# junghoseong/aircombat-selfplay

Hardware: AMD Instinct MI355X
Metric: agent-steps/sec (higher is better)
Workload: dtype f32

## Files before the change

aircombat-selfplay_amd/csrc/aircombat.hip:

```cpp
#include <hip/hip_runtime.h>
#include <stdint.h>
#include <stdio.h>
#include <string.h>
#include <string>
#include <vector>
#include <cmath>
#include <algorithm>
#include <chrono>
#include "../../include/aircombat.h"
#include "../../include/aircombat_buffer.h"
#include "clk_stamps.hpp"
#include "f16_device.hpp"
#include "f16_split.hpp"

using f16::State;
using f16::Derived;
using f16::Tab;
using f16::clampf;

#define AC_F_FIELDS(X)                                                                                           \
  X(vx) X(vy) X(vz) X(q0) X(q1) X(q2) X(q3) X(wp) X(wq) X(wr) X(hv1x) X(hv1y) X(hv1z) X(hv2x) X(hv2y) X(hv2z)   \
  X(ha1x) X(ha1y) X(ha1z) X(wdx) X(wdy) X(wdz) X(aix) X(aiy) X(aiz) X(bax) X(bay) X(baz) X(da) X(de) X(dr)       \
  X(thr) X(pin_r) X(pin_p) X(pin_y) X(pi_r) X(pi_p) X(pi_y) X(tef) X(ail) X(elev) X(sbdeg) X(alpha) X(mach)      \
  X(qc) X(vg) X(ap) X(aq) X(ar) X(npx) X(npy) X(npz) X(n1) X(n2) X(n2norm) X(ff) X(tank0) X(tank1)
#define AC_TF_FIELDS(X) X(bloods) X(pre_posture) X(pre_altitude) X(pre_event) X(pre_shoot)
#define AC_TI_FIELDS(X)                                                                                  \
  X(status) X(die_flag) X(remaining) X(pre_remaining) X(shoot_action) X(last_missile) X(last_shoot_time) \
  X(lock_bits) X(lock_pos) X(cur_step)

enum {
#define X(n) FF_##n,
  AC_F_FIELDS(X) AC_TF_FIELDS(X)
#undef X
  NF
};
enum {
  FI_eng, FI_ticks,
#define X(n) FI_##n,
  AC_TI_FIELDS(X)
#undef X
  NI
};
enum { ND = 3 };
enum : int {
  SW_tef = 0, SW_pin_r, SW_pin_p, SW_pin_y,
  SW_pi_r, SW_pi_p, SW_pi_y, SW_ail,
  SW_elev, SW_sbdeg, SW_n1, SW_n2,
  SW_n2norm, SW_ff, SW_tank0, SW_tank1,
  SW_alpha, SW_mach, SW_qc, SW_vg,
  SW_ap, SW_aq, SW_ar, SW_npy,
  SW_npz, SW_npx, SW_eng, SW_ticks,
  SW_vx, SW_vy, SW_vz, SW_q0,
  SW_q1, SW_q2, SW_q3, SW_wp,
  SW_wq, SW_wr, SW_hv1x, SW_hv1y,
  SW_hv1z, SW_hv2x, SW_hv2y, SW_hv2z,
  SW_ha1x, SW_ha1y, SW_ha1z, SW_wdx,
  SW_wdy, SW_wdz, SW_aix, SW_aiy,
  SW_aiz, SW_bax, SW_bay, SW_baz,
  SW_da, SW_de, SW_dr, SW_thr,
  SW_pre_posture, SW_pre_altitude, SW_pre_event, SW_cur_step,
  SW_bloods, SW_status, SW_die_flag, SW_pre_shoot,
  SW_remaining, SW_pre_remaining, SW_shoot_action, SW_last_missile,
  SW_last_shoot_time, SW_lock_bits, SW_lock_pos, SW_pad,
  NSW
};
enum { NSG = NSW / 4, SG_TASK0 = 15 };
static_assert(NSW == 76 && SW_pre_posture == 4 * SG_TASK0, "19 groups: 15 flight, 4 task");
static const int kSlotF[NF] = {
#define X(n) SW_##n,
    AC_F_FIELDS(X) AC_TF_FIELDS(X)
#undef X
};
static const int kSlotI[NI] = {SW_eng, SW_ticks,
#define X(n) SW_##n,
                               AC_TI_FIELDS(X)
#undef X
};
enum { MF_px, MF_py, MF_pz, MF_vx, MF_vy, MF_vz, MF_theta, MF_psi, MF_t, MF_m, MF_dth, MF_dph, MF_dprev, NMF };
enum { MI_status, MI_recede, MI_order, NMI };
enum { MSL_INACTIVE = -1, MSL_LAUNCHED = 0, MSL_HIT = 1, MSL_MISS = 2 };

static const char* kStateNames[AC_STATE_LEN] = {
    "rx", "ry", "rz",
#define X(n) #n,
    AC_F_FIELDS(X) AC_TF_FIELDS(X) "eng", "ticks", AC_TI_FIELDS(X)
#undef X
    "x_rem_gun", "x_rem_9m", "x_rem_120b", "x_rem_chaff", "x_bits", "x_last_chaff", "x_orphan_hits", "x_mp_prev", "x_ref_set",
    "x_ch_status0", "x_ch_mult0", "x_ch_status1", "x_ch_mult1", "x_n_ch",
    "x_cg_AO", "x_cg_TA", "x_wez0", "x_wez1", "x_wez2", "x_wez3", "x_tail0", "x_tail1", "x_tail2", "x_tail3",
    "x_c0x", "x_c0y", "x_c0z", "x_c0t", "x_c1x", "x_c1y", "x_c1z", "x_c1t",
};

struct Task {
#define X(n) float n;
  AC_TF_FIELDS(X)
#undef X
#define X(n) int n;
  AC_TI_FIELDS(X)
#undef X
};

template <typename R>
struct MslT {
  R px, py, pz, vx, vy, vz, theta, psi, t, m, dth, dph, dprev;
  int status, recede, order;
  int dpos;
  int model;
};
using Msl = MslT<float>;
using MslD = MslT<double>;

struct DevCfg {
  int task, A, n_ego, substeps, max_steps, obs_dim, act_dim, msl_slots;
  int N;
  float altitude_limit, acc_x, acc_y, acc_z;
  float posture_scale, altitude_scale, event_scale, missile_posture_scale, shoot_penalty_scale;
  int posture_pot, altitude_pot, event_pot, shoot_pot;
  float alt_safe, alt_danger, alt_kv;
  float max_attack_angle, max_attack_distance;
  int min_attack_interval, use_artillery, lock_len;
  int rwr;
  int legacy_obs;
  int tobs;
  int num_missiles[AC_MAX_AGENTS];
  double P0x, P0y, P0z, sLat0, cLat0, sLon0, cLon0;
  float rm0, rn0, h0;
  unsigned long long chaff_seed;
};

struct DevPtrs {
  float* F; int* I; double* D;
  float* MF; int* MI;
  double* MD;
  float* H;
  int* man_step; float* man_h0;
  const float* tF; const int* tI; const double* tD;
  const float* tab;
  const float* actions;
  float* obs; float* rew; uint8_t* done; int* info;
  float* obs2; float* rew2; uint8_t* done2; int* info2;
  int* err;
};

__device__ __forceinline__ bool nonfinite_probe(float veci, float pqr, float h_sl_ft, float np_max) {
  return !(fabsf(veci + pqr + h_sl_ft + np_max) < INFINITY);
}
__device__ __forceinline__ float poison_if(bool bad, float reward) { return bad ? __int_as_float(0x7fc00001) : reward; }

#define AC_LANE_INDEX(n) const unsigned un_ = (unsigned)(n), uN_ = (unsigned)N
#define AC_AT(base, f) \
  (*(decltype(base))((char*)(base) + (size_t)((unsigned)(f) * (uN_ * (unsigned)sizeof(*(base))) + un_ * (unsigned)sizeof(*(base)))))
#define AC_GRP(S, g) (*reinterpret_cast<float4*>((char*)(S) + (size_t)((unsigned)(g) * (uN_ * 16u) + un_ * 16u)))
#define AC_WORD(S, w) (*reinterpret_cast<int*>((char*)(S) + (size_t)((unsigned)((w) >> 2) * (uN_ * 16u) + un_ * 16u + 4u * (unsigned)((w) & 3))))
__device__ __forceinline__ int state_word(const float* S, int w, int N, int n) { AC_LANE_INDEX(n); return AC_WORD(S, w); }
#define AC_FLIGHT_GROUPS(G)                                                                                                       \
  G(0, tef, pin_r, pin_p, pin_y) G(1, pi_r, pi_p, pi_y, ail) G(2, elev, sbdeg, n1, n2) G(3, n2norm, ff, tank0, tank1)               \
  G(4, alpha, mach, qc, vg) G(5, ap, aq, ar, npy) G(7, vx, vy, vz, q0) G(8, q1, q2, q3, wp) G(9, wq, wr, hv1x, hv1y)                \
  G(10, hv1z, hv2x, hv2y, hv2z) G(11, ha1x, ha1y, ha1z, wdx) G(12, wdy, wdz, aix, aiy) G(13, aiz, bax, bay, baz) G(14, da, de, dr, thr)
static_assert(SW_alpha == 16 && SW_npz == 24 && SW_vx == 28 && SW_ha1x == 44 && SW_da == 56, "AC_FLIGHT_GROUPS follows the SW_ order");
__device__ __forceinline__ void load_position(const double* D, int N, int n, State& s) {
  const double2 xy = *reinterpret_cast<const double2*>((const char*)D + (size_t)((unsigned)n * 16u));
  s.rx = xy.x; s.ry = xy.y;
  s.rz = D[2 * (size_t)N + n];
}
__device__ __forceinline__ void store_position(double* D, int N, int n, const State& s) {
  *reinterpret_cast<double2*>((char*)D + (size_t)((unsigned)n * 16u)) = make_double2(s.rx, s.ry);
  D[2 * (size_t)N + n] = s.rz;
}
constexpr bool ac_role_reads(int role, int g) {
  return role < 0 || (role == 0 ? g >= 4 : (role == 1 ? g <= 6 : (g >= 6 && g <= 10)));
}
template <int ROLE>
__device__ __forceinline__ void load_flight_role(const float* F, const int* I, const double* D, int N, int n, State& s) {
  (void)I;
  AC_LANE_INDEX(n);
#define G(g, a, b, c, d) if (ac_role_reads(ROLE, g)) { const float4 v = AC_GRP(F, g); s.a = v.x; s.b = v.y; s.c = v.z; s.d = v.w; }
  AC_FLIGHT_GROUPS(G)
#undef G
  if (ac_role_reads(ROLE, 6)) {
    const float4 v = AC_GRP(F, 6);
    s.npz = v.x; s.npx = v.y; s.eng = __float_as_int(v.z); s.ticks = __float_as_int(v.w);
  }
  if (ROLE != 1) load_position(D, N, n, s);
}
__device__ __forceinline__ void load_flight(const float* F, const int* I, const double* D, int N, int n, State& s) { load_flight_role<-1>(F, I, D, N, n, s); }
__device__ __forceinline__ void store_flight(float* F, int* I, double* D, int N, int n, const State& s) {
  (void)I;
  AC_LANE_INDEX(n);
#define G(g, a, b, c, d) AC_GRP(F, g) = make_float4(s.a, s.b, s.c, s.d);
  AC_FLIGHT_GROUPS(G)
#undef G
  AC_GRP(F, 6) = make_float4(s.npz, s.npx, __int_as_float(s.eng), __int_as_float(s.ticks));
  store_position(D, N, n, s);
}
__device__ __forceinline__ void load_task(const float* F, const int* I, int N, int n, Task& t) {
  (void)I;
  AC_LANE_INDEX(n);
  const float4 a = AC_GRP(F, SG_TASK0), b = AC_GRP(F, SG_TASK0 + 1), c = AC_GRP(F, SG_TASK0 + 2), d = AC_GRP(F, SG_TASK0 + 3);
  t.pre_posture = a.x; t.pre_altitude = a.y; t.pre_event = a.z; t.cur_step = __float_as_int(a.w);
  t.bloods = b.x; t.status = __float_as_int(b.y); t.die_flag = __float_as_int(b.z); t.pre_shoot = b.w;
  t.remaining = __float_as_int(c.x); t.pre_remaining = __float_as_int(c.y); t.shoot_action = __float_as_int(c.z); t.last_missile = __float_as_int(c.w);
  t.last_shoot_time = __float_as_int(d.x); t.lock_bits = __float_as_int(d.y); t.lock_pos = __float_as_int(d.z);
}
__device__ __forceinline__ void store_task_group0(float* F, int N, int n, const Task& t) {
  AC_LANE_INDEX(n);
  AC_GRP(F, SG_TASK0) = make_float4(t.pre_posture, t.pre_altitude, t.pre_event, __int_as_float(t.cur_step));
}
__device__ __forceinline__ void store_task_rare(float* F, int N, int n, const Task& t) {
  AC_LANE_INDEX(n);
  AC_GRP(F, SG_TASK0 + 1) = make_float4(t.bloods, __int_as_float(t.status), __int_as_float(t.die_flag), t.pre_shoot);
  AC_GRP(F, SG_TASK0 + 2) = make_float4(__int_as_float(t.remaining), __int_as_float(t.pre_remaining), __int_as_float(t.shoot_action), __int_as_float(t.last_missile));
  AC_GRP(F, SG_TASK0 + 3) = make_float4(__int_as_float(t.last_shoot_time), __int_as_float(t.lock_bits), __int_as_float(t.lock_pos), 0.0f);
}
__device__ __forceinline__ void store_task(float* F, int* I, int N, int n, const Task& t) {
  (void)I;
  store_task_group0(F, N, n, t);
  store_task_rare(F, N, n, t);
}
__device__ __forceinline__ void load_state(const float* F, const int* I, const double* D, int N, int n, State& s, Task& t) {
  load_flight(F, I, D, N, n, s);
  load_task(F, I, N, n, t);
}
__device__ __forceinline__ void store_state(float* F, int* I, double* D, int N, int n, const State& s, const Task& t) {
  store_flight(F, I, D, N, n, s);
  store_task(F, I, N, n, t);
}
template <typename R>
__device__ __forceinline__ void load_msl(const R* MF, const int* MI, int N, int n, int slot, MslT<R>& m) {
  AC_LANE_INDEX(n);
  const R* f = MF + (size_t)slot * NMF * N;
  const int* i = MI + (size_t)slot * NMI * N;
  m.px = AC_AT(f, MF_px); m.py = AC_AT(f, MF_py); m.pz = AC_AT(f, MF_pz);
  m.vx = AC_AT(f, MF_vx); m.vy = AC_AT(f, MF_vy); m.vz = AC_AT(f, MF_vz);
  m.theta = AC_AT(f, MF_theta); m.psi = AC_AT(f, MF_psi); m.t = AC_AT(f, MF_t); m.m = AC_AT(f, MF_m);
  m.dth = AC_AT(f, MF_dth); m.dph = AC_AT(f, MF_dph); m.dprev = AC_AT(f, MF_dprev);
  m.status = AC_AT(i, MI_status); m.order = AC_AT(i, MI_order);
  const int rw = AC_AT(i, MI_recede);
  m.recede = rw & 511; m.model = (rw >> 9) & 1; m.dpos = rw >> 10;
}
template <typename R>
__device__ __forceinline__ void store_msl(R* MF, int* MI, int N, int n, int slot, const MslT<R>& m) {
  AC_LANE_INDEX(n);
  R* f = MF + (size_t)slot * NMF * N;
  int* i = MI + (size_t)slot * NMI * N;
  AC_AT(f, MF_px) = m.px; AC_AT(f, MF_py) = m.py; AC_AT(f, MF_pz) = m.pz;
  AC_AT(f, MF_vx) = m.vx; AC_AT(f, MF_vy) = m.vy; AC_AT(f, MF_vz) = m.vz;
  AC_AT(f, MF_theta) = m.theta; AC_AT(f, MF_psi) = m.psi; AC_AT(f, MF_t) = m.t; AC_AT(f, MF_m) = m.m;
  AC_AT(f, MF_dth) = m.dth; AC_AT(f, MF_dph) = m.dph; AC_AT(f, MF_dprev) = m.dprev;
  AC_AT(i, MI_status) = m.status; AC_AT(i, MI_recede) = (m.dpos << 10) | (m.model << 9) | m.recede; AC_AT(i, MI_order) = m.order;
}

template <typename R>
__device__ __forceinline__ void store_msl_clock(R* MF, int* MI, int N, int n, int slot, const MslT<R>& m) {
  AC_LANE_INDEX(n);
  R* f = MF + (size_t)slot * NMF * N;
  int* i = MI + (size_t)slot * NMI * N;
  AC_AT(f, MF_t) = m.t; AC_AT(f, MF_dprev) = m.dprev;
  AC_AT(i, MI_status) = m.status; AC_AT(i, MI_recede) = (m.dpos << 10) | (m.model << 9) | m.recede;
}
__device__ __forceinline__ void store_task_changed(float* F, int* I, int N, int n, const Task& t, const Task& was) {
  (void)I;
  store_task_group0(F, N, n, t);
  const bool rare = __float_as_int(t.bloods) != __float_as_int(was.bloods) || __float_as_int(t.pre_shoot) != __float_as_int(was.pre_shoot) ||
                    t.status != was.status || t.die_flag != was.die_flag || t.remaining != was.remaining || t.pre_remaining != was.pre_remaining ||
                    t.shoot_action != was.shoot_action || t.last_missile != was.last_missile || t.last_shoot_time != was.last_shoot_time ||
                    t.lock_bits != was.lock_bits || t.lock_pos != was.lock_pos;
  if (rare) store_task_rare(F, N, n, t);
}

__device__ __forceinline__ void zero_controller_state(const DevPtrs& P, int N, int n, bool live) {
  if (P.H && live) {
    for (int k = 0; k < 128; ++k) P.H[(size_t)k * N + n] = 0.0f;
    P.man_step[n] = 0; P.man_h0[n] = 0.0f;
  }
}

struct Props {
  float n, e, u;
  double n64, e64, u64;
  float vn, ve, vd;
  float alt_m;
  float ub, vb, wb, vc;
  float sphi, cphi, stht, ctht;
  float m11, m12;
};
__device__ __forceinline__ float mps(float fps) { return clampf(-700.0f, fps * f16::kFt2M, 700.0f); }

__device__ __forceinline__ void make_pose(const Derived& d, const DevCfg& c, Props& p) {
  p.alt_m = clampf(-500.0f, d.h_sl_ft * f16::kFt2M, 26000.0f);
  p.vn = mps(d.vn); p.ve = mps(d.ve); p.vd = mps(d.vd);
  const double a = 6378137.0, b = 6356752.314245179;
  double sl = d.sLat64, cl = d.cLat64, so = d.sLon64, co = d.cLon64;
  double Nn = a * a * fx::rsqrt(a * a * cl * cl + b * b * sl * sl);
  double h = (double)p.alt_m;
  double x = (Nn + h) * cl * co, y = (Nn + h) * cl * so, z = (Nn * (b / a) * (b / a) + h) * sl;
  double dx = x - c.P0x, dy = y - c.P0y, dz = z - c.P0z;
  double t = c.cLon0 * dx + c.sLon0 * dy;
  p.e64 = -c.sLon0 * dx + c.cLon0 * dy; p.u64 = c.cLat0 * t + c.sLat0 * dz; p.n64 = -c.sLat0 * t + c.cLat0 * dz;
  p.e = (float)p.e64; p.u = (float)p.u64; p.n = (float)p.n64;
}
__device__ __forceinline__ void make_props(const State& s, const Derived& d, const DevCfg& c, Props& p) {
  make_pose(d, c, p);
  p.ub = mps(d.u); p.vb = mps(d.v); p.wb = mps(d.w);
  p.vc = clampf(0.0f, f16::vcas_from_impact_pressure(s.qc) * f16::kFt2M, 1400.0f);
  const float* T = d.T;
  float m13 = T[0] * d.d_eci[0] + T[1] * d.d_eci[1] + T[2] * d.d_eci[2];
  float m23 = T[3] * d.d_eci[0] + T[4] * d.d_eci[1] + T[5] * d.d_eci[2];
  float m33 = T[6] * d.d_eci[0] + T[7] * d.d_eci[1] + T[8] * d.d_eci[2];
  p.m11 = T[0] * d.n_eci[0] + T[1] * d.n_eci[1] + T[2] * d.n_eci[2];
  p.m12 = T[0] * d.e_eci[0] + T[1] * d.e_eci[1] + T[2] * d.e_eci[2];
  p.stht = clampf(-1.0f, -m13, 1.0f);
  float ct = sqrtf(fmaxf(0.0f, 1.0f - p.stht * p.stht));
  p.ctht = ct;
  float ic = (ct > 1e-12f) ? 1.0f / sqrtf(m23 * m23 + m33 * m33) : 0.0f;
  p.sphi = (ct > 1e-12f) ? m23 * ic : 0.0f;
  p.cphi = (ct > 1e-12f) ? m33 * ic : 1.0f;
}

struct Geo { float AO, TA, R, side, cAO, cTA; };
__device__ __forceinline__ float acos_fast(float x) { return f16::atan2_fast(sqrtf((1.0f - x) * (1.0f + x)), x); }
__device__ __forceinline__ float tanh_fast(float x) {
  const float t = __expf(2.0f * clampf(-10.0f, x, 10.0f));
  return (t - 1.0f) / (t + 1.0f);
}
__device__ __forceinline__ float atanh_fast(float x) { return 0.5f * __logf((1.0f + x) / (1.0f - x)); }
template <bool TWO_D>
__device__ __forceinline__ Geo ao_ta_r(float ex, float ey, float ez, float evx, float evy, float evz,
                                       float nx, float ny, float nz, float nvx, float nvy, float nvz) {
  float dx = nx - ex, dy = ny - ey, dz = nz - ez;
  float ev, nv, R, pe, pn;
  if (TWO_D) {
    ev = sqrtf(evx * evx + evy * evy); nv = sqrtf(nvx * nvx + nvy * nvy); R = sqrtf(dx * dx + dy * dy);
    pe = dx * evx + dy * evy; pn = dx * nvx + dy * nvy;
  } else {
    ev = sqrtf(evx * evx + evy * evy + evz * evz); nv = sqrtf(nvx * nvx + nvy * nvy + nvz * nvz);
    R = sqrtf(dx * dx + dy * dy + dz * dz);
    pe = dx * evx + dy * evy + dz * evz; pn = dx * nvx + dy * nvy + dz * nvz;
  }
  Geo g;
  g.cAO = clampf(-1.0f, pe / (R * ev + 1e-8f), 1.0f);
  g.cTA = clampf(-1.0f, pn / (R * nv + 1e-8f), 1.0f);
  g.AO = acos_fast(g.cAO);
  g.TA = acos_fast(g.cTA);
  g.R = R;
  float cr = evx * dy - evy * dx;
  g.side = (cr > 0.0f) ? 1.0f : ((cr < 0.0f) ? -1.0f : 0.0f);
// ... 245 lines not shown
  __builtin_amdgcn_fence(__ATOMIC_RELEASE, "wavefront");
  __builtin_amdgcn_wave_barrier();
  __builtin_amdgcn_fence(__ATOMIC_ACQUIRE, "wavefront");
}
__device__ __forceinline__ void emit_rows(const DevPtrs& P, float* lds , int ow, int lane,
                                          float reward, bool done, int A, int i0, int i1, int i2, int i3);
template <int NOB>
__device__ __forceinline__ void emit_outputs(const DevPtrs& P, float* lds , int ow, int lane, const float (&ob)[NOB],
                                             float reward, bool done, int A, int i0, int i1, int i2, int i3) {
  float* row = lds + lane * ow;
#pragma unroll
  for (int k = 0; k < NOB; ++k) if (k < ow) row[k] = ob[k];
  for (int k = NOB; k < ow; ++k) row[k] = 0.0f;
  emit_rows(P, lds, ow, lane, reward, done, A, i0, i1, i2, i3);
}
__device__ __forceinline__ void emit_obs_rows(const DevPtrs& P, float* lds, int ow, int lane) {
  wave_lds_fence();
  AC_CLK(56);
  const size_t blk = blockIdx.x;
  const int nvec = 16 * ow;
  const float4* l4 = reinterpret_cast<const float4*>(lds);
#pragma unroll
  for (int set = 1; set >= 0; --set) {
    float* obs = set ? P.obs2 : P.obs;
    if (!obs) continue;
    float4* o4 = reinterpret_cast<float4*>(obs + blk * 64 * (size_t)ow);
    int i = lane;
    for (; i + 192 < nvec; i += 256) {
      const float4 v0 = l4[i], v1 = l4[i + 64], v2 = l4[i + 128], v3 = l4[i + 192];
      o4[i] = v0; o4[i + 64] = v1; o4[i + 128] = v2; o4[i + 192] = v3;
    }
    for (; i < nvec; i += 64) o4[i] = l4[i];
  }
  AC_CLK(57);
  wave_lds_fence();
}
__device__ __forceinline__ void emit_scalars(const DevPtrs& P, int lane, float reward, bool done, int A, int i0, int i1, int i2, int i3) {
  const size_t blk = blockIdx.x;
  const unsigned long long dmask = __ballot(done);
  unsigned dword = 0;
#pragma unroll
  for (int b = 0; b < 4; ++b) dword |= (unsigned)((dmask >> (4 * (lane & 15) + b)) & 1ull) << (8 * b);
  const int4 inf = make_int4(i0, i1, i2, i3);
  const int packed = (i0 & 0xFFFF) | ((i1 & 0xFF) << 16) | (min(i2, 127) << 24) | ((i3 & 1) << 31);
  const size_t n = blk * 64 + lane;
  if (!(fabsf(reward) < INFINITY)) {
    const int own = ((__float_as_int(reward) & 0x7fffffff) == 0x7fc00001) ? 1 : 0;
    __hip_atomic_fetch_max(P.err, (own << 30) | (0x3fffffff - (int)n), __ATOMIC_RELAXED, __HIP_MEMORY_SCOPE_SYSTEM);
  }
#pragma unroll
  for (int set = 1; set >= 0; --set) {
    float* rew = set ? P.rew2 : P.rew; uint8_t* dn = set ? P.done2 : P.done; int* info = set ? P.info2 : P.info;
    if (!rew) continue;
    rew[n] = reward;
    if (lane < 16) reinterpret_cast<unsigned*>(dn + blk * 64)[lane] = dword;
    if (set) {
      const int w = __shfl(packed, (lane * A) & 63);
      if (lane < 64 / A) info[blk * (64 / A) + lane] = w;
    } else if (lane % A == 0) *reinterpret_cast<int4*>(info + (n / A) * 4) = inf;
  }
}
__device__ __forceinline__ void emit_rows(const DevPtrs& P, float* lds, int ow, int lane, float reward, bool done, int A, int i0, int i1, int i2, int i3) {
  emit_obs_rows(P, lds, ow, lane);
  emit_scalars(P, lane, reward, done, A, i0, i1, i2, i3);
}
__device__ __forceinline__ float4 load_controls(const float* act, int act_dim) {
  if ((act_dim & 3) == 0) return *reinterpret_cast<const float4*>(act);
  return make_float4(act[0], act[1], act[2], act[3]);
}

struct Enemy { float n, e, u, vn, ve, vd, ub, alt; };
__device__ __forceinline__ Enemy exchange_1v1(const Props& pr) {
  Enemy E;
  E.n = __shfl_xor(pr.n, 1); E.e = __shfl_xor(pr.e, 1); E.u = __shfl_xor(pr.u, 1);
  E.vn = __shfl_xor(pr.vn, 1); E.ve = __shfl_xor(pr.ve, 1); E.vd = __shfl_xor(pr.vd, 1);
  E.ub = __shfl_xor(pr.ub, 1); E.alt = __shfl_xor(pr.alt_m, 1);
  return E;
}
struct Incoming { bool any; float px, py, pz, vx, vy, vz; };
template <int TASK>
__device__ __forceinline__ void observe_1v1(const Props& pr, const Enemy& E, const Incoming& in, float* ob) {
  ob[0] = pr.alt_m / 5000.0f;
  ob[1] = pr.sphi; ob[2] = pr.cphi; ob[3] = pr.stht; ob[4] = pr.ctht;
  ob[5] = pr.ub / 340.0f; ob[6] = pr.vb / 340.0f; ob[7] = pr.wb / 340.0f; ob[8] = pr.vc / 340.0f;
  Geo g = (TASK == AC_TASK_SINGLECOMBAT)
              ? ao_ta_r<true>(pr.n, pr.e, pr.u, pr.vn, pr.ve, pr.vd, E.n, E.e, E.u, E.vn, E.ve, E.vd)
              : ao_ta_r<false>(pr.n, pr.e, pr.u, pr.vn, pr.ve, pr.vd, E.n, E.e, E.u, E.vn, E.ve, E.vd);
  ob[9] = (E.ub - pr.ub) / 340.0f;
  ob[10] = (E.alt - pr.alt_m) / 1000.0f;
  ob[11] = g.AO; ob[12] = g.TA; ob[13] = g.R / 10000.0f; ob[14] = g.side;
  if (TASK == AC_TASK_SINGLECOMBAT) {
#pragma unroll
    for (int k = 0; k < 15; ++k) ob[k] = clampf(-10.0f, ob[k], 10.0f);
  } else {
#pragma unroll
    for (int k = 15; k < 21; ++k) ob[k] = 0.0f;
    if (in.any) {
      Geo gm = ao_ta_r<false>(pr.n, pr.e, pr.u, pr.vn, pr.ve, pr.vd, in.px, in.py, in.pz, in.vx, in.vy, in.vz);
      ob[15] = (sqrtf(in.vx * in.vx + in.vy * in.vy + in.vz * in.vz) - pr.ub) / 340.0f;
      ob[16] = (in.pz - pr.alt_m) / 1000.0f;
      ob[17] = gm.AO; ob[18] = gm.TA; ob[19] = gm.R / 10000.0f; ob[20] = gm.side;
    }
  }
}
__device__ __forceinline__ float posture_raw(const Props& pr, const Enemy& E) {
  Geo g = ao_ta_r<false>(pr.n, pr.e, pr.u, pr.vn, pr.ve, pr.vd, E.n, E.e, E.u, E.vn, E.ve, E.vd);
  return posture_fn(g.AO, g.TA, g.R * 0.001f);
}
__device__ __forceinline__ float altitude_raw(const Props& pr, const DevCfg& c) {
  return altitude_fn(pr.u * 0.001f, pr.vd / 340.0f, c);
}

template <int TASK>
struct TaskTraits {
  static constexpr bool HAS_MSL = (TASK == AC_TASK_SHOOT_MISSILE || TASK == AC_TASK_DODGE_MISSILE);
  static constexpr int MSLOTS = HAS_MSL ? AC_MAX_MISSILES_PER_AGENT : 1;
  static constexpr int OBS = (TASK == AC_TASK_SINGLECOMBAT) ? 15 : 21;
};

#include "split_kernel.hpp"
#include "pair_kernel.hpp"

template <int TASK, int WPE, int FORM = 0>
__global__ __launch_bounds__(FORM == 1 ? 192 : (FORM == 2 ? 128 : (FORM == 3 ? 256 : 64)), WPE) void step_kernel_1v1(DevPtrs P, DevCfg c) {
  static_assert(TASK == AC_TASK_SINGLECOMBAT ? FORM <= 1 : FORM >= 2, "no launch path for this (task, form)");
  using TT = TaskTraits<TASK>;
  constexpr bool SPLIT = FORM == 1, QUAD = FORM == 3, PAIR = FORM == 2 || QUAD;
  constexpr bool HAS_MSL = TT::HAS_MSL;
  constexpr int MSLOTS = TT::MSLOTS;
  constexpr int OBS = TT::OBS;
  AC_CLK(0);
  __shared__ __attribute__((aligned(16))) float lds_tab[F16_PACK_LEN];
  __shared__ __attribute__((aligned(16))) float lds_out[64 * OBS];
  __shared__ __attribute__((aligned(16))) char split_lds[SPLIT ? sizeof(SplitLds) : (QUAD ? sizeof(QuadLds) : (PAIR ? sizeof(PairLds) : 16))];
  SplitLds& L = *reinterpret_cast<SplitLds*>(split_lds);
  QuadLds& LQ = *reinterpret_cast<QuadLds*>(split_lds);
  PairLds& LP = QUAD ? LQ.P : *reinterpret_cast<PairLds*>(split_lds);
  const Tab T{lds_tab};
  const int N = c.N;
  const int l = threadIdx.x & 63;
  const int n = blockIdx.x * 64 + l;
  const bool live = n < N;
  const int nn = live ? n : (N - 2 + (n & 1));
  const int slot = nn & 1;

  State s; Task t; Derived d; Props pr;
  int pre_st[MSLOTS];
#pragma unroll
  for (int k = 0; k < MSLOTS; ++k) pre_st[k] = MSL_INACTIVE;
  const float* act = P.actions + (size_t)nn * c.act_dim;
  float4 a4;
  ActionFetch arow;
  float shoot_raw = 0.0f;
  if (SPLIT) {
    TableCopy<192> tc;
    tc.issue(P.tab);
    AC_CLKW(0, 123);
    const int role = __builtin_amdgcn_readfirstlane(threadIdx.x >> 6);
    s = State{}; t = Task{};
    if (role == 0) { load_flight_role<0>(P.F, P.I, P.D, N, nn, s); AC_CLKW(0, 124); load_task(P.F, P.I, N, nn, t); AC_CLKW(0, 125); }
    else if (role == 1) load_flight_role<1>(P.F, P.I, P.D, N, nn, s);
    else { load_flight_role<2>(P.F, P.I, P.D, N, nn, s); t.status = state_word(P.F, SW_status, N, nn); }
    __builtin_amdgcn_s_barrier();
    tc.write(lds_tab);
    a4 = make_float4(0.f, 0.f, 0.f, 0.f);
    __builtin_amdgcn_s_waitcnt(0x0F70);
    if (role == 1) arow.issue(act, c.act_dim);
    AC_CLKW(0, 120); AC_CLKW(1, 121); AC_CLKW(2, 122);
    __syncthreads();
  } else if (QUAD) {
    const int role = __builtin_amdgcn_readfirstlane(threadIdx.x >> 6);
    TableCopy<256> tc;
    tc.issue(P.tab);
    s = State{}; t = Task{};
    if (role == 0) { load_flight_role<0>(P.F, P.I, P.D, N, nn, s); t.status = state_word(P.F, SW_status, N, nn); }
    else if (role == 1) load_flight_role<1>(P.F, P.I, P.D, N, nn, s);
    else if (role == 2) { load_flight_role<2>(P.F, P.I, P.D, N, nn, s); t.status = state_word(P.F, SW_status, N, nn); }
    else {
      load_task(P.F, P.I, N, nn, t);
      s.ticks = state_word(P.F, SW_ticks, N, nn);
#pragma unroll
      for (int k = 0; k < MSLOTS; ++k) pre_st[k] = P.MI[((size_t)k * NMI + MI_status) * (size_t)N + nn];
    }
    __builtin_amdgcn_s_barrier();
    tc.write(lds_tab);
    a4 = make_float4(0.f, 0.f, 0.f, 0.f);
    __builtin_amdgcn_s_waitcnt(0x0F70);
    if (role == 1) arow.issue(act, c.act_dim);
    __syncthreads();
    if (role == 0) { quad_dynamics_wave(P, c, T, LQ, l, n, live, s, t); return; }
    if (role != 3 && split_helper_wave<true>(s, t, T, LQ.S, l, c.substeps, nullptr, nullptr, &arow)) return;
  } else if (PAIR) {
    const bool flight_role = __builtin_amdgcn_readfirstlane(threadIdx.x >> 6) == 1;
    PairFlightIn fin;
    if (!flight_role) {
      a4 = make_float4(0.f, 0.f, 0.f, 0.f);
      s = State{}; load_task(P.F, P.I, N, nn, t);
#pragma unroll
      for (int k = 0; k < MSLOTS; ++k) pre_st[k] = P.MI[((size_t)k * NMI + MI_status) * (size_t)N + nn];
    }
    stage_tables<128>(lds_tab, P.tab);
    if (flight_role) {
      pair_flight_load(P, c, nn, fin);
      pair_flight_wave<true>(P, c, T, LP, l, n, live, fin);
      return;
    }

  } else {
    TableCopy<64> tc;
    tc.issue(P.tab);
    a4 = load_controls(act, c.act_dim);
    if (TASK == AC_TASK_SHOOT_MISSILE) shoot_raw = act[4];
    load_state(P.F, P.I, P.D, N, nn, s, t);
    tc.commit(lds_tab);
  }
  AC_CLK(1);
  const Task was = t;
  constexpr bool OBS_BY_KIN = SPLIT && TASK == AC_TASK_SINGLECOMBAT;
  if (SPLIT) {
    const int role = __builtin_amdgcn_readfirstlane(threadIdx.x >> 6);
    if (split_helper_wave(s, t, T, L, l, c.substeps, nullptr, nullptr, &arow)) {
      if (OBS_BY_KIN && role == 1) {
        using namespace mail;
        wg_sync();
        Props q;
        q.alt_m = L.M[T_PR][l]; q.ub = L.M[T_PR + 5][l];
        q.n = L.M[T_PR + 9][l]; q.e = L.M[T_PR + 10][l]; q.u = L.M[T_PR + 11][l];
        q.vn = L.M[T_PR + 12][l]; q.ve = L.M[T_PR + 13][l]; q.vd = L.M[T_PR + 14][l];
        const Enemy Eq = exchange_1v1(q);
        L.M[T_RALT][l] = altitude_raw(q, c);
        L.M[T_RPOS][l] = posture_raw(q, Eq);
        wg_sync();
      }
      if (OBS_BY_KIN && role == 2) {
        using namespace mail;
        wg_sync();
        Props q;
        q.alt_m = L.M[T_PR][l]; q.sphi = L.M[T_PR + 1][l]; q.cphi = L.M[T_PR + 2][l]; q.stht = L.M[T_PR + 3][l]; q.ctht = L.M[T_PR + 4][l];
        q.ub = L.M[T_PR + 5][l]; q.vb = L.M[T_PR + 6][l]; q.wb = L.M[T_PR + 7][l]; q.vc = L.M[T_PR + 8][l];
        q.n = L.M[T_PR + 9][l]; q.e = L.M[T_PR + 10][l]; q.u = L.M[T_PR + 11][l];
        q.vn = L.M[T_PR + 12][l]; q.ve = L.M[T_PR + 13][l]; q.vd = L.M[T_PR + 14][l];
        const Enemy Eq = exchange_1v1(q);
        const Incoming none{false, 0, 0, 0, 0, 0, 0};
        float obq[OBS];
        observe_1v1<TASK>(q, Eq, none, obq);
        wg_sync();
        if (L.M[T_DONE][l] != 0.0f) {
          const float* tobs = (const float*)(P.tF + (size_t)NSW * 2) + slot * OBS;
#pragma unroll
          for (int k = 0; k < OBS; ++k) obq[k] = tobs[k];
        }
        float* row = lds_out + l * OBS;
#pragma unroll
        for (int k = 0; k < OBS; ++k) row[k] = obq[k];
        emit_obs_rows(P, lds_out, OBS, l);
      }
      return;
    }
  }
  Msl ms[MSLOTS];
  int nslots = 0, msl_was_active = 0;
  if (HAS_MSL) {
    nslots = min(c.num_missiles[slot], MSLOTS);
#pragma unroll
    for (int k = 0; k < MSLOTS; ++k) {
      const int st = (k < nslots) ? (PAIR ? pre_st[k] : P.MI[((size_t)k * NMI + MI_status) * (size_t)N + nn]) : MSL_INACTIVE;
      if (st != MSL_INACTIVE) { load_msl(P.MF, P.MI, N, nn, k, ms[k]); msl_was_active |= 1 << k; }
      else { ms[k] = Msl{}; ms[k].status = MSL_INACTIVE; }
    }
  }

  t.cur_step += 1;
  if (!SPLIT) {
    s.da = clampf(-1.0f, a4.x / 20.0f - 1.0f, 1.0f);
    s.de = clampf(-1.0f, a4.y / 20.0f - 1.0f, 1.0f);
    s.dr = clampf(-1.0f, a4.z / 20.0f - 1.0f, 1.0f);
    s.thr = clampf(0.0f, a4.w / 58.0f + 0.4f, 0.9f);
  }
  if (TASK == AC_TASK_SHOOT_MISSILE && !PAIR) t.shoot_action = (shoot_raw != 0.0f) ? 1 : 0;

  const MslParam MP = aim9l();
  bool have_pose = false;
  int last_tick = -1;
  bool env_has_missiles = false;
  if (PAIR) {
    bool mine = false;
#pragma unroll
    for (int k = 0; k < MSLOTS; ++k) mine = mine || ms[k].status != MSL_INACTIVE;
    const int other = __shfl_xor((int)mine, 1);
    env_has_missiles = mine || (bool)other;
  }
  int quad_nrun = 0;
  const int quad_ticks0 = s.ticks;
  for (int sub = 0; sub < c.substeps; ++sub) {
    bool fly_munitions = HAS_MSL;
    if (QUAD) {
      quad_substep_begin<true>(t, LQ, l, sub, env_has_missiles, quad_ticks0, quad_nrun, pr, c);
      fly_munitions = env_has_missiles;
    } else if (PAIR) {
      AC_CLK(2 + 8 * sub);
      pair_substep<true>(t, LP, l, sub, env_has_missiles, pr, c);
      AC_CLK(4 + 8 * sub);
      if (!env_has_missiles) continue;
    } else if (SPLIT) {
      if (dynamics_wave_tick(s, t, d, T, L, l, sub)) { have_pose = true; last_tick = sub; }
    } else if (t.status == AC_ALIVE) {
      if (t.bloods <= 0.0f) t.status = AC_SHOTDOWN;
      f16::tick<false>(s, d, T);
      have_pose = true;
    }
    if (HAS_MSL && fly_munitions) {
      if (!PAIR) {
      f16::locate(s, d);
      if (!have_pose) { f16::body_frame(s, d); have_pose = true; }
      make_props(s, d, c, pr);
      }
      float tx = __shfl_xor(pr.n, 1), ty = __shfl_xor(pr.e, 1), tz = __shfl_xor(pr.u, 1);
      float tvx = __shfl_xor(pr.vn, 1), tvy = __shfl_xor(pr.ve, 1), tvz = __shfl_xor(pr.vd, 1);
      bool talive = __shfl_xor(t.status, 1) == AC_ALIVE;
      bool hit_now = false;
#pragma unroll
      for (int k = 0; k < MSLOTS; ++k) {
        if (k < nslots && ms[k].status != MSL_INACTIVE) {
          missile_run(ms[k], MP, tx, ty, tz, tvx, tvy, tvz, talive, c);
          if (ms[k].status == MSL_HIT && talive) { hit_now = true; talive = false; }
        }
      }
      if (__shfl_xor((int)hit_now, 1) && t.status == AC_ALIVE) t.status = AC_SHOTDOWN;
      AC_CLK(5 + 8 * sub);
    }
    if (QUAD) wg_sync();
  }
  const bool split_located = SPLIT && dynamics_wave_finish(s, d, L, l, last_tick, c.substeps);
  if (PAIR) {
    if (QUAD) wg_sync();
    wg_sync();
    pair_read_final(LP, l, s, d, pr);
  } else if (!HAS_MSL || c.substeps == 0) {
    if (!split_located) f16::locate(s, d);
    if (!have_pose) f16::body_frame(s, d);
    make_props(s, d, c, pr);
  }
  AC_CLK(52);
  if (OBS_BY_KIN) {
    using namespace mail;
    L.M[T_PR][l] = pr.alt_m; L.M[T_PR + 1][l] = pr.sphi; L.M[T_PR + 2][l] = pr.cphi; L.M[T_PR + 3][l] = pr.stht; L.M[T_PR + 4][l] = pr.ctht;
    L.M[T_PR + 5][l] = pr.ub; L.M[T_PR + 6][l] = pr.vb; L.M[T_PR + 7][l] = pr.wb; L.M[T_PR + 8][l] = pr.vc;
    L.M[T_PR + 9][l] = pr.n; L.M[T_PR + 10][l] = pr.e; L.M[T_PR + 11][l] = pr.u;
    L.M[T_PR + 12][l] = pr.vn; L.M[T_PR + 13][l] = pr.ve; L.M[T_PR + 14][l] = pr.vd;
    wg_sync();
  }
  Enemy E = exchange_1v1(pr);

  if (c.use_artillery) {
    Geo g = ao_ta_r<false>(pr.n, pr.e, pr.u, pr.vn, pr.ve, pr.vd, E.n, E.e, E.u, E.vn, E.ve, E.vd);
    bool ealive = __shfl_xor(t.status, 1) == AC_ALIVE;
    float of = (g.AO <= 0.5236f) ? 1.0f - g.AO / 0.5236f : 0.0f;
    float Rk = g.R * 0.001f;
    float df = (Rk <= 1.0f) ? 1.0f : ((Rk <= 3.0f) ? (3.0f - Rk) * 0.5f : 0.0f);
    float dmg = ealive ? of * df : 0.0f;
    t.bloods -= __shfl_xor(dmg, 1);
  }
  if (HAS_MSL) {
    bool launch;
    if (TASK == AC_TASK_SHOOT_MISSILE && PAIR) t.shoot_action = ((QUAD ? LQ.S.M[mail::F_BITS][l] : LP.FIN[pair::FIN_BITS][l]) != 0.0f) ? 1 : 0;
    if (TASK == AC_TASK_DODGE_MISSILE) {
      const float dx = E.n - pr.n, dy = E.e - pr.e, dz = E.u - pr.u;
      const float dist = sqrtf(dx * dx + dy * dy + dz * dz);
      const float sp = sqrtf(pr.vn * pr.vn + pr.ve * pr.ve + pr.vd * pr.vd);
      const float ang = 57.29577951f * acosf(clampf(-1.0f, (dx * pr.vn + dy * pr.ve + dz * pr.vd) / (dist * sp + 1e-8f), 1.0f));
      const int len = c.lock_len;
      const unsigned bit = 1u << (unsigned)(t.lock_pos % len);
      t.lock_bits = (ang < c.max_attack_angle) ? (t.lock_bits | (int)bit) : (t.lock_bits & ~(int)bit);
      t.lock_pos += 1;
      const bool locked = __popc((unsigned)t.lock_bits & ((1u << len) - 1u)) >= len;
      launch = t.status == AC_ALIVE && locked && dist <= c.max_attack_distance && t.remaining > 0 &&
               (t.cur_step - t.last_shoot_time) >= c.min_attack_interval;
      if (launch) t.last_shoot_time = t.cur_step;
    } else {
      bool prev_done = t.last_missile < 0;
#pragma unroll
      for (int k = 0; k < MSLOTS; ++k)
        if (k == t.last_missile) prev_done = (ms[k].status == MSL_HIT || ms[k].status == MSL_MISS);
      launch = t.status == AC_ALIVE && t.shoot_action && t.remaining > 0 && prev_done;
    }
    int k = nslots - t.remaining;
    if (launch && k >= 0 && k < nslots) {
      float tht = asinf(pr.stht);
      float psi = atan2f(pr.m12, pr.m11);
      if (psi < 0.0f) psi += 2.0f * f16::kPi;
#pragma unroll
      for (int q = 0; q < MSLOTS; ++q)
        if (q == k) {
          ms[q].px = pr.n; ms[q].py = pr.e; ms[q].pz = pr.u; ms[q].vx = pr.vn; ms[q].vy = pr.ve; ms[q].vz = pr.vd;
          ms[q].theta = tht; ms[q].psi = psi; ms[q].t = 0.0f; ms[q].m = MP.m0; ms[q].dth = 0.0f; ms[q].dph = 0.0f;
          ms[q].dprev = INFINITY; ms[q].recede = 0; ms[q].status = MSL_LAUNCHED; ms[q].order = t.cur_step;
        }
      t.last_missile = k;
      t.remaining -= 1;
    }
  }

  Incoming inc{false, 0, 0, 0, 0, 0, 0};
  int my_hits = 0;
  int inc_slot = -1;
  if (HAS_MSL) {
    int best = 0x7fffffff, mine = -1;
#pragma unroll
    for (int k = 0; k < MSLOTS; ++k) {
      if (k < nslots && ms[k].status == MSL_LAUNCHED && ms[k].order < best) { best = ms[k].order; mine = k; }
      if (k < nslots && ms[k].status == MSL_HIT) my_hits += 1;
    }
    float a0 = 0, a1 = 0, a2 = 0, a3 = 0, a4 = 0, a5 = 0;
#pragma unroll
    for (int k = 0; k < MSLOTS; ++k)
      if (k == mine) { a0 = ms[k].px; a1 = ms[k].py; a2 = ms[k].pz; a3 = ms[k].vx; a4 = ms[k].vy; a5 = ms[k].vz; }
    inc.any = __shfl_xor((int)(mine >= 0), 1);
    inc_slot = __shfl_xor(mine, 1);
    inc.px = __shfl_xor(a0, 1); inc.py = __shfl_xor(a1, 1); inc.pz = __shfl_xor(a2, 1);
    inc.vx = __shfl_xor(a3, 1); inc.vy = __shfl_xor(a4, 1); inc.vz = __shfl_xor(a5, 1);
  }
  float ob[OBS];
  if (!OBS_BY_KIN) observe_1v1<TASK>(pr, E, inc, ob);
  AC_CLK(58);

  const int status_pre = t.status;
  int code = AC_DONE_NONE;
  bool done = false;
  bool nonfinite = false;
  {
    float np_max = fmaxf(fabsf(s.npx), fmaxf(fabsf(s.npy), fabsf(s.npz)));
    float pqr = sqrtf(d.p * d.p + d.q * d.q + d.r * d.r);
    nonfinite = nonfinite_probe(d.veci, pqr, d.h_sl_ft, np_max);
    bool extreme = nonfinite || (d.veci >= 1e10f) || (pqr >= 1000.0f) || (d.h_sl_ft >= 1e10f) || (np_max > 10.0f);
    bool overload = (s.ticks >= kTickOverload) &&
                    (fabsf(s.npx) > c.acc_x || fabsf(s.npy) > c.acc_y || fabsf(s.npz + 1.0f) > c.acc_z);
    if (pr.alt_m <= c.altitude_limit) { t.status = AC_CRASH; code = AC_DONE_LOW_ALTITUDE; done = true; }
    else if (extreme) { t.status = AC_CRASH; code = AC_DONE_EXTREME_STATE; done = true; }
    else if (overload) { t.status = AC_CRASH; code = AC_DONE_OVERLOAD; done = true; }
  }
  {
    int other_pre = __shfl_xor(status_pre, 1), other_post = __shfl_xor(t.status, 1);
    int enemy_status = (slot == 0) ? other_pre : other_post;
    if (!done) {
      if (t.status == AC_SHOTDOWN) { code = AC_DONE_SHOTDOWN; done = true; }
      else if (t.status == AC_CRASH) { code = AC_DONE_CRASHED; done = true; }
      else if (enemy_status != AC_ALIVE && !inc.any) { code = AC_DONE_MISSION_COMPLETE; done = true; }
      else if (t.cur_step >= c.max_steps) { code = AC_DONE_TIMEOUT; done = true; }
    }
  }

  const int other_done = __shfl_xor((int)done, 1);
  const bool all_done = done && (bool)other_done;
  const int other_code = __shfl_xor(code, 1);
  if (OBS_BY_KIN) {
    L.M[mail::T_DONE][l] = all_done ? 1.0f : 0.0f;
    wg_sync();
  } else if (all_done) {
    const float* tobs = (const float*)(P.tF + (size_t)NSW * 2) + slot * OBS;
#pragma unroll
    for (int k = 0; k < OBS; ++k) ob[k] = tobs[k];
  }

  AC_CLK(59);
  float reward = 0.0f;
  const bool evaluates = !t.die_flag;
  if (evaluates) {
    t.die_flag = (t.status != AC_ALIVE) ? 1 : 0;
    float r_alt = potential(OBS_BY_KIN ? L.M[mail::T_RALT][l] : altitude_raw(pr, c), c.altitude_scale, c.altitude_pot, t.pre_altitude);
    float r_pos = potential(OBS_BY_KIN ? L.M[mail::T_RPOS][l] : posture_raw(pr, E), c.posture_scale, c.posture_pot, t.pre_posture);
    float ev = ((t.status != AC_ALIVE) ? -200.0f : 0.0f) + 200.0f * (float)my_hits;
    float r_ev = potential(ev, c.event_scale, c.event_pot, t.pre_event);
    reward = r_alt + r_pos + r_ev;
    if (TASK == AC_TASK_SHOOT_MISSILE) {
      float sp = (t.remaining == t.pre_remaining - 1) ? -30.0f : 0.0f;
      t.pre_remaining = t.remaining;
      reward += potential(sp, c.shoot_penalty_scale, c.shoot_pot, t.pre_shoot);
    }
  }
  if (TASK == AC_TASK_DODGE_MISSILE) {
    float spd[MSLOTS];
#pragma unroll
    for (int k = 0; k < MSLOTS; ++k) spd[k] = sqrtf(ms[k].vx * ms[k].vx + ms[k].vy * ms[k].vy + ms[k].vz * ms[k].vz);
    const int base = (threadIdx.x & 63) - slot;
    const int my_inc_id = inc.any ? 1 + (slot ^ 1) * MSLOTS + inc_slot : 0;
    int prev = t.shoot_action;
    float r_mp = 0.0f;
#pragma unroll
    for (int i = 0; i < 2; ++i) {
      const int ev_i = __shfl((int)evaluates, base + i), id_i = __shfl(my_inc_id, base + i);
      if (!ev_i) continue;
      if (id_i) {
        if (!prev) prev = id_i;
        float v_prev = 0.0f, v_cur = 0.0f;
#pragma unroll
        for (int k = 0; k < MSLOTS; ++k) {
          float a = __shfl(spd[k], base + (prev - 1) / MSLOTS), b = __shfl(spd[k], base + (id_i - 1) / MSLOTS);
          if (k == (prev - 1) % MSLOTS) v_prev = a;
          if (k == (id_i - 1) % MSLOTS) v_cur = b;
        }
        if (slot == i) {
          const float v_dec = (v_prev - v_cur) / 340.0f * c.missile_posture_scale;
          const float va = sqrtf(pr.vn * pr.vn + pr.ve * pr.ve + pr.vd * pr.vd);
          const float ang = (inc.vx * pr.vn + inc.vy * pr.ve + inc.vz * pr.vd) / (v_cur * va);
          r_mp = (ang < 0.0f) ? ang / (fmaxf(v_dec, 0.0f) + 1.0f) : ang * fmaxf(v_dec, 0.0f);
        }
      } else prev = 0;
    }
    t.shoot_action = prev;
    reward += r_mp;
  }

  int step_out = t.cur_step;
  if (all_done) {
    load_state(P.tF, P.tI, P.tD, 2, slot, s, t);
    zero_controller_state(P, N, n, live);
#pragma unroll
    for (int k = 0; k < MSLOTS; ++k) { ms[k] = Msl{}; ms[k].status = MSL_INACTIVE; }
  }
  AC_CLK(53);
  if (live) {
    if (!PAIR) { store_flight(P.F, P.I, P.D, N, n, s); store_task_changed(P.F, P.I, N, n, t, was); }
    else {
      if (all_done) store_flight(P.F, P.I, P.D, N, n, s);
      store_task_changed(P.F, P.I, N, n, t, was);
    }
    if (HAS_MSL) {
#pragma unroll
      for (int k = 0; k < MSLOTS; ++k)
        if (k < nslots && (ms[k].status != MSL_INACTIVE || ((msl_was_active >> k) & 1))) store_msl(P.MF, P.MI, N, n, k, ms[k]);
    }
  }
  AC_CLK(55);
  reward = poison_if(nonfinite, reward);
  if (OBS_BY_KIN) emit_scalars(P, l, reward, done, 2, step_out, other_code ? other_code : code, 0, all_done ? 1 : 0);
  else emit_outputs(P, lds_out, OBS, l, ob, reward, done, 2, step_out, other_code ? other_code : code, 0, all_done ? 1 : 0);
  AC_CLK(54);
}

__device__ __forceinline__ Enemy gather_pose(const Props& pr, int lane) {
  Enemy E;
  E.n = __shfl(pr.n, lane); E.e = __shfl(pr.e, lane); E.u = __shfl(pr.u, lane);
  E.vn = __shfl(pr.vn, lane); E.ve = __shfl(pr.ve, lane); E.vd = __shfl(pr.vd, lane);
  E.ub = __shfl(pr.ub, lane); E.alt = __shfl(pr.alt_m, lane);
  return E;
}
template <int A>
__device__ __forceinline__ float observe_nvn(const Props& pr, int slot, int base_lane, int n_ego, float* ob) {
  auto c10 = [](float v) { return clampf(-10.0f, v, 10.0f); };
  if (ob) {
    ob[0] = c10(pr.alt_m / 5000.0f);
    ob[1] = c10(pr.sphi); ob[2] = c10(pr.cphi); ob[3] = c10(pr.stht); ob[4] = c10(pr.ctht);
    ob[5] = c10(pr.ub / 340.0f); ob[6] = c10(pr.vb / 340.0f); ob[7] = c10(pr.wb / 340.0f); ob[8] = c10(pr.vc / 340.0f);
  }
  const int my_team = slot < n_ego ? 0 : 1;
  const int n_mine = my_team == 0 ? n_ego : A - n_ego;
  float posture = 0.0f;
#pragma unroll
  for (int j = 0; j < A; ++j) {
    Enemy E = gather_pose(pr, base_lane + j);
    const int team_j = j < n_ego ? 0 : 1;
    if (j == slot) continue;
    Geo g = ao_ta_r<false>(pr.n, pr.e, pr.u, pr.vn, pr.ve, pr.vd, E.n, E.e, E.u, E.vn, E.ve, E.vd);
    int idx;
    if (team_j == my_team) {
      int first = my_team == 0 ? 0 : n_ego;
      idx = (j - first) - (j > slot ? 1 : 0);
    } else {
      int first = my_team == 0 ? n_ego : 0;
      idx = (n_mine - 1) + (j - first);
      posture += posture_fn(g.AO, g.TA, g.R * 0.001f);
    }
    if (ob) {
      float* blk = ob + 9 + idx * 6;
      blk[0] = c10((E.ub - pr.ub) / 340.0f); blk[1] = c10((E.alt - pr.alt_m) / 1000.0f);
      blk[2] = c10(g.AO); blk[3] = c10(g.TA); blk[4] = c10(g.R / 10000.0f); blk[5] = c10(g.side);
    }
  }
  return posture;
}

template <int A>
__device__ __forceinline__ void legacy_obs_nvn(const Props& pr, int slot, int base_lane, int n_ego, float* row) {
  const int team = slot < n_ego ? 0 : 1;
  const int paired = (team == 0 ? n_ego : 0) + (slot - (team == 0 ? 0 : n_ego));
  const Enemy E = gather_pose(pr, base_lane + paired);
  const Incoming none{false, 0, 0, 0, 0, 0, 0};
  float o21[21];
  observe_1v1<AC_TASK_SHOOT_MISSILE>(pr, E, none, o21);
#pragma unroll
  for (int k = 0; k < 21; ++k) row[k] = o21[k];
}

template <int A, int WPE, bool SPLIT = false>
__global__ __launch_bounds__(SPLIT ? 192 : 64, WPE) void step_kernel_nvn(DevPtrs P, DevCfg c) {
  constexpr int OBS = 9 + 6 * (A - 1);
  __shared__ __attribute__((aligned(16))) float lds_tab[F16_PACK_LEN];
  __shared__ __attribute__((aligned(16))) float lds_out[64 * OBS];
  __shared__ __attribute__((aligned(16))) char split_lds[SPLIT ? sizeof(SplitLds) : 16];
  SplitLds& L = *reinterpret_cast<SplitLds*>(split_lds);
  const Tab T{lds_tab};
  const int N = c.N;
  const int l = threadIdx.x & 63;
  const int n = blockIdx.x * 64 + l;
  const bool live = n < N;
  const int slot = l % A;
  const int nn = live ? n : (N - A + slot);
  const int base_lane = l - slot;
  const int team = slot < c.n_ego ? 0 : 1;

  State s; Task t; Derived d; Props pr;
  TableCopy<SPLIT ? 192 : 64> tc;
  tc.issue(P.tab);
  const float4 a4 = load_controls(P.actions + (size_t)nn * c.act_dim, c.act_dim);
  load_state(P.F, P.I, P.D, N, nn, s, t);
  const Task was = t;
  tc.commit(lds_tab);
  t.cur_step += 1;
  s.da = clampf(-1.0f, a4.x / 20.0f - 1.0f, 1.0f);
  s.de = clampf(-1.0f, a4.y / 20.0f - 1.0f, 1.0f);
  s.dr = clampf(-1.0f, a4.z / 20.0f - 1.0f, 1.0f);
  s.thr = clampf(0.0f, a4.w / 58.0f + 0.4f, 0.9f);
  if (SPLIT && split_helper_wave(s, t, T, L, l, c.substeps)) return;
  bool have_pose = false;
  int nrun_split = 0;
  const bool split_located = SPLIT && dynamics_wave_ticks(s, t, d, T, L, l, c.substeps, nrun_split);
  for (int sub = 0; sub < c.substeps && !SPLIT; ++sub) {
    if (t.status == AC_ALIVE) {
      if (t.bloods <= 0.0f) t.status = AC_SHOTDOWN;
      f16::tick<false>(s, d, T);
      have_pose = true;
    }
  }
  if (!split_located) {
    f16::locate(s, d);
    if (!have_pose) f16::body_frame(s, d);
  }
  make_props(s, d, c, pr);

  const int ow = c.legacy_obs ? 21 : OBS;
  float* orow = lds_out + l * ow;
  float posture = observe_nvn<A>(pr, slot, base_lane, c.n_ego, c.legacy_obs ? nullptr : orow);
  if (c.legacy_obs) legacy_obs_nvn<A>(pr, slot, base_lane, c.n_ego, orow);

  float own = 0.0f;
  if (t.status == AC_ALIVE) {
    float r_alt = potential(altitude_raw(pr, c), c.altitude_scale, c.altitude_pot, t.pre_altitude);
    float r_pos = potential(posture, c.posture_scale, c.posture_pot, t.pre_posture);
    float r_ev = potential(0.0f, c.event_scale, c.event_pot, t.pre_event);
    own = r_alt + r_pos + r_ev;
  }
  float tsum = 0.0f;
#pragma unroll
  for (int j = 0; j < A; ++j) {
    float rj = __shfl(own, base_lane + j);
    if ((j < c.n_ego ? 0 : 1) == team) tsum += rj;
  }
  const float reward = tsum / (float)(team == 0 ? c.n_ego : A - c.n_ego);

  bool done = false;
  int code = AC_DONE_NONE;
  int last_code = AC_DONE_NONE;
  float np_max = fmaxf(fabsf(s.npx), fmaxf(fabsf(s.npy), fabsf(s.npz)));
  float pqr = sqrtf(d.p * d.p + d.q * d.q + d.r * d.r);
  const bool nonfinite = nonfinite_probe(d.veci, pqr, d.h_sl_ft, np_max);
  const bool extreme = nonfinite || (d.veci >= 1e10f) || (pqr >= 1000.0f) || (d.h_sl_ft >= 1e10f) || (np_max > 10.0f);
  const bool overload = (s.ticks >= kTickOverload) &&
                        (fabsf(s.npx) > c.acc_x || fabsf(s.npy) > c.acc_y || fabsf(s.npz + 1.0f) > c.acc_z);
  const bool low = pr.alt_m <= c.altitude_limit;
  const unsigned long long env_mask = ((A == 64) ? ~0ull : ((1ull << A) - 1ull)) << base_lane;
  const int st0 = t.status;
  const bool crash_cond = extreme || overload || low;
  constexpr unsigned amask = (A >= 32) ? ~0u : ((1u << A) - 1u);
  const unsigned al0 = (unsigned)(__ballot(st0 == AC_ALIVE) >> base_lane) & amask;
  const unsigned ccb = (unsigned)(__ballot(crash_cond) >> base_lane) & amask;
  const unsigned team0 = (1u << c.n_ego) - 1u, team1 = amask & ~team0;
  unsigned alive = al0;
  bool enemies_dead = false, crash_mine = false;
#pragma unroll
  for (int i = 0; i < A; ++i) {
    const bool ed = (alive & (i < c.n_ego ? team1 : team0)) == 0;
    const bool crash_now = ((al0 >> i) & 1u) && !ed && ((ccb >> i) & 1u);
    if (crash_now) alive &= ~(1u << i);
    if (i == slot) { enemies_dead = ed; crash_mine = crash_now; }
  }
  if (crash_mine) t.status = AC_CRASH;
  if (st0 == AC_SHOTDOWN) { code = AC_DONE_SHOTDOWN; done = true; }
  else if (st0 == AC_CRASH) { code = AC_DONE_CRASHED; done = true; }
  else if (enemies_dead) { code = AC_DONE_MISSION_COMPLETE; done = true; }
  else if (extreme) { code = AC_DONE_EXTREME_STATE; done = true; }
  else if (overload) { code = AC_DONE_OVERLOAD; done = true; }
  else if (low) { code = AC_DONE_LOW_ALTITUDE; done = true; }
  else if (t.cur_step >= c.max_steps) { code = AC_DONE_TIMEOUT; done = true; }
  {
    const unsigned long long coded = __ballot(code != AC_DONE_NONE) & env_mask;
    const int last = coded ? 63 - __clzll((long long)coded) : l;
    last_code = __shfl(code, last);
  }
  const bool all_done = ((unsigned)(__ballot(done) >> base_lane) & amask) == amask;
  int step_out = t.cur_step;
  if (all_done) {
    load_state(P.tF, P.tI, P.tD, A, slot, s, t);
    zero_controller_state(P, N, n, live);
    const float* tobs = P.tF + (size_t)NSW * A + slot * OBS;
    for (int k = 0; k < ow; ++k) orow[k] = tobs[k];
  }
  if (live) {
    store_flight(P.F, P.I, P.D, N, n, s);
    store_task_changed(P.F, P.I, N, n, t, was);
  }
  emit_rows(P, lds_out, ow, l, poison_if(nonfinite, reward), done, A, step_out, last_code, 0, all_done ? 1 : 0);
}

struct InitArgs { ac_init_state_t ic[AC_MAX_AGENTS]; };

__device__ double geod_alt_from_asl(double geod_lat, double alt) {
  const double a = f16::kA, b = f16::kB, e2 = 1.0 - b * b / (a * a);
  double cg = cos(geod_lat), sg = sin(geod_lat), Nn = a / sqrt(1 - e2 * sg * sg);
  double n = e2, prev_n = 1.0;
  int iter = 0;
  if (cg > fabs(sg)) {
    double tg = sg / cg, x0 = Nn * e2 * cg, x = 0.0;
    while (fabs(n - prev_n) > 1E-15 && iter < 10) {
      double tl = (1 - n) * tg, c2 = 1. / (1. + tl * tl), slr = b / sqrt(1. - e2 * c2), R = slr + alt;
      x = R * sqrt(c2); prev_n = n; n = x0 / x; iter++;
    }
    return x / cg - Nn;
  }
  double ctg = cg / sg, z0 = Nn * e2 * sg, z = 0.0;
  while (fabs(n - prev_n) > 1E-15 && iter < 10) {
    double ctl = ctg / (1 - n), s2 = 1. / (1. + ctl * ctl), c2 = 1. - s2, slr = b / sqrt(1. - e2 * c2), R = slr + alt;
    z = R * (ctl >= 0 ? 1.0 : -1.0) * sqrt(s2); prev_n = n; n = z0 / (z0 + z); iter++;
  }
  return z / sg - Nn * (1 - e2);
}

__device__ void initial_state(const ac_init_state_t& ic, const Tab& T, State& s, Derived& d) {
  s = State{};
  const double D2R = 3.14159265358979323846 / 180.0;
  double lon = ic.lon_deg * D2R, lat = ic.lat_geod_deg * D2R, psi = ic.psi_deg * D2R;
  double hg = geod_alt_from_asl(lat, ic.h_sl_ft);
  const double ee = 1.0 - (f16::kB / f16::kA) * (f16::kB / f16::kA);
  double sl = sin(lat), cl = cos(lat), so = sin(lon), co = cos(lon);
  double RN = f16::kA / sqrt(1.0 - ee * sl * sl);
  s.rx = (RN + hg) * cl * co; s.ry = (RN + hg) * cl * so; s.rz = ((1 - ee) * RN + hg) * sl;
  double Tl[9] = {-co * sl, -so * sl, cl, -so, co, 0.0, -co * cl, -so * cl, -sl};
  double tr[4] = {1.0 + Tl[0] + Tl[4] + Tl[8], 1.0 + Tl[0] - Tl[4] - Tl[8], 1.0 - Tl[0] + Tl[4] - Tl[8], 1.0 - Tl[0] - Tl[4] + Tl[8]};
  int idx = 0;
  for (int i = 1; i < 4; ++i) if (tr[i] > tr[idx]) idx = i;
  double a4[4];
  double m12 = Tl[1], m21 = Tl[3], m13 = Tl[2], m31 = Tl[6], m23 = Tl[5], m32 = Tl[7];
  if (idx == 0) { a4[0] = 0.5 * sqrt(tr[0]); a4[1] = 0.25 * (m23 - m32) / a4[0]; a4[2] = 0.25 * (m31 - m13) / a4[0]; a4[3] = 0.25 * (m12 - m21) / a4[0]; }
  else if (idx == 1) { a4[1] = 0.5 * sqrt(tr[1]); a4[0] = 0.25 * (m23 - m32) / a4[1]; a4[2] = 0.25 * (m12 + m21) / a4[1]; a4[3] = 0.25 * (m31 + m13) / a4[1]; }
  else if (idx == 2) { a4[2] = 0.5 * sqrt(tr[2]); a4[0] = 0.25 * (m31 - m13) / a4[2]; a4[1] = 0.25 * (m12 + m21) / a4[2]; a4[3] = 0.25 * (m23 + m32) / a4[2]; }
  else { a4[3] = 0.5 * sqrt(tr[3]); a4[0] = 0.25 * (m12 - m21) / a4[3]; a4[1] = 0.25 * (m13 + m31) / a4[3]; a4[2] = 0.25 * (m23 + m32) / a4[3]; }
  double b0 = cos(0.5 * psi), b3 = sin(0.5 * psi);
  double q[4] = {a4[0] * b0 - a4[3] * b3, a4[1] * b0 + a4[2] * b3, a4[2] * b0 - a4[1] * b3, a4[0] * b3 + a4[3] * b0};
  double qn = 1.0 / sqrt(q[0] * q[0] + q[1] * q[1] + q[2] * q[2] + q[3] * q[3]);
  for (int i = 0; i < 4; ++i) q[i] *= qn;
  s.q0 = (float)q[0]; s.q1 = (float)q[1]; s.q2 = (float)q[2]; s.q3 = (float)q[3];
  double Tb[9] = {q[0] * q[0] + q[1] * q[1] - q[2] * q[2] - q[3] * q[3], 2.0 * (q[1] * q[2] + q[0] * q[3]), 2.0 * (q[1] * q[3] - q[0] * q[2]),
                  2.0 * (q[1] * q[2] - q[0] * q[3]), q[0] * q[0] - q[1] * q[1] + q[2] * q[2] - q[3] * q[3], 2.0 * (q[2] * q[3] + q[0] * q[1]),
                  2.0 * (q[1] * q[3] + q[0] * q[2]), 2.0 * (q[2] * q[3] - q[0] * q[1]), q[0] * q[0] - q[1] * q[1] - q[2] * q[2] + q[3] * q[3]};
  s.wp = (float)(ic.p_rad_sec + f16::kOmega * Tb[2]); s.wq = (float)(ic.q_rad_sec + f16::kOmega * Tb[5]); s.wr = (float)(ic.r_rad_sec + f16::kOmega * Tb[8]);
  double vix = Tb[0] * ic.u_fps + Tb[3] * ic.v_fps + Tb[6] * ic.w_fps;
  double viy = Tb[1] * ic.u_fps + Tb[4] * ic.v_fps + Tb[7] * ic.w_fps;
  double viz = Tb[2] * ic.u_fps + Tb[5] * ic.v_fps + Tb[8] * ic.w_fps;
  s.vx = (float)(vix - f16::kOmega * s.ry); s.vy = (float)(viy + f16::kOmega * s.rx); s.vz = (float)viz;
  s.tank0 = (float)F16_TANK0_CONTENTS; s.tank1 = (float)F16_TANK1_CONTENTS;
  s.eng = f16::PH_OFF | f16::ENG_CUTOFF;
  f16::tick<true, true>(s, d, T);
  f16::tick<true>(s, d, T);
  s.hv1x = s.hv2x = s.vx; s.hv1y = s.hv2y = s.vy; s.hv1z = s.hv2z = s.vz;
  s.ha1x = s.aix; s.ha1y = s.aiy; s.ha1z = s.aiz;
  s.n2 = (float)F16_ENG_IDLEN2; s.n1 = (float)F16_ENG_IDLEN1; s.n2norm = 0.0f;
  s.eng = f16::PH_RUN | f16::ENG_RUNNING;
  {
    f16::Atmos A = f16::atmosphere(d.h_sl_ft);
    float idle_f, mil_f, aug_f;
    f16::engine_factors(T, s.mach, d.h_sl_ft, idle_f, mil_f, aug_f);
    float idle = (float)F16_ENG_MILTHRUST * idle_f;
    float tsfc = (float)F16_ENG_TSFC * sqrtf(A.T * (1.0f / 389.7f)) * (0.84f + 1.0f);
    float target = idle * tsfc;
    float ff = (target > 0.0f) ? target : 0.0f;
    s.ff = fmaxf(ff, 757.648518f);
  }
}

template <int TASK>
__global__ __launch_bounds__(64) void init_kernel_1v1(InitArgs ia, DevCfg c, const float* tab, float* tF, int* tI, double* tD) {
  using TT = TaskTraits<TASK>;
  constexpr int OBS = TT::OBS;
  __shared__ __attribute__((aligned(16))) float lds_tab[F16_PACK_LEN];
  stage_tables(lds_tab, tab);
  const Tab T{lds_tab};
  const int slot = threadIdx.x & 1;
  State s; Derived d; Task t{}; Props pr;
  initial_state(ia.ic[slot], T, s, d);
  t.bloods = 100.0f; t.status = AC_ALIVE;
  t.remaining = c.num_missiles[slot]; t.pre_remaining = c.num_missiles[slot];
  t.last_missile = -1; t.last_shoot_time = -c.min_attack_interval;
  f16::locate(s, d);
  make_props(s, d, c, pr);
  Enemy E = exchange_1v1(pr);
  Incoming inc{false, 0, 0, 0, 0, 0, 0};
  float ob[OBS];
  observe_1v1<TASK>(pr, E, inc, ob);
  if (c.altitude_pot) t.pre_altitude = altitude_raw(pr, c) * c.altitude_scale;
  if (c.posture_pot) t.pre_posture = posture_raw(pr, E) * c.posture_scale;
  if (threadIdx.x < 2) {
    store_state(tF, tI, tD, 2, slot, s, t);
    float* tobs = tF + (size_t)NSW * 2 + slot * OBS;
    for (int k = 0; k < OBS; ++k) tobs[k] = ob[k];
  }
}

template <int A>
__global__ __launch_bounds__(64) void init_kernel_nvn(InitArgs ia, DevCfg c, const float* tab, float* tF, int* tI, double* tD) {
  constexpr int OBS = 9 + 6 * (A - 1);
  __shared__ __attribute__((aligned(16))) float lds_tab[F16_PACK_LEN];
  stage_tables(lds_tab, tab);
  const Tab T{lds_tab};
  const int slot = threadIdx.x % A;
  const int base_lane = (threadIdx.x & 63) - slot;
  State s; Derived d; Task t{}; Props pr;
  initial_state(ia.ic[slot], T, s, d);
  t.bloods = 100.0f; t.status = AC_ALIVE;
  t.remaining = c.num_missiles[slot]; t.pre_remaining = c.num_missiles[slot];
  t.last_missile = -1; t.last_shoot_time = -c.min_attack_interval;
  f16::locate(s, d);
  make_props(s, d, c, pr);
  float ob[OBS];
  for (int k = 0; k < OBS; ++k) ob[k] = 0.0f;
  float posture = observe_nvn<A>(pr, slot, base_lane, c.n_ego, ob);
  if (c.legacy_obs) legacy_obs_nvn<A>(pr, slot, base_lane, c.n_ego, ob);
  if (c.altitude_pot) t.pre_altitude = altitude_raw(pr, c) * c.altitude_scale;
  if (c.posture_pot) t.pre_posture = posture * c.posture_scale;
  if (threadIdx.x < A) {
    store_state(tF, tI, tD, A, slot, s, t);
    float* tobs = tF + (size_t)NSW * A + slot * OBS;
    for (int k = 0; k < OBS; ++k) tobs[k] = ob[k];
  }
}

#include "scenario_kernel.hpp"
#include "controller_common.hpp"
#include "controller_pieces.hpp"
#include "controller8_kernel.hpp"
#include "heading_kernel.hpp"

__global__ void reset_all_kernel(DevPtrs P, DevCfg c) {
  const int OBS = c.obs_dim;
  const int N = c.N;
  const int n = blockIdx.x * blockDim.x + threadIdx.x;
  if (n >= N) return;
  const int slot = n % c.A;
  State s; Task t;
  load_state(P.tF, P.tI, P.tD, c.A, slot, s, t);
  store_state(P.F, P.I, P.D, N, n, s, t);
  for (int k = 0; k < c.msl_slots; ++k) {
    if (P.MD) { MslD m{}; m.status = MSL_INACTIVE; store_msl(P.MD, P.MI, N, n, k, m); }
    else { Msl m{}; m.status = MSL_INACTIVE; store_msl(P.MF, P.MI, N, n, k, m); }
  }
  const int TOBS = c.tobs;
  const float* tobs = P.tF + (size_t)NSW * c.A + slot * TOBS;
  for (int k = 0; k < OBS; ++k) P.obs[(size_t)n * OBS + k] = (k < TOBS) ? tobs[k] : 0.0f;
  zero_controller_state(P, N, n, true);
  P.rew[n] = 0.0f; P.done[n] = 0;
  if (slot == 0) { int* inf = P.info + (size_t)(n / c.A) * 4; inf[0] = 0; inf[1] = 0; inf[2] = 0; inf[3] = 0; }
}

static thread_local std::string g_err;
static int fail(const std::string& m) { g_err = m; return -1; }
static uint64_t fnv1a(uint64_t hsh, const void* p, size_t n) {
  const unsigned char* b = (const unsigned char*)p;
  for (size_t i = 0; i < n; ++i) { hsh ^= b[i]; hsh *= 0x100000001B3ULL; }
  return hsh;
}
#define HIP_OK(call)                                                                              \
  do {                                                                                            \
    hipError_t e_ = (call);                                                                       \
    if (e_ != hipSuccess) return fail(std::string(#call) + ": " + hipGetErrorString(e_));        \
  } while (0)

#include "aql_dispatch.hpp"

struct ac_env {
  ac_config_t cfg;
  DevCfg dc;
  DevPtrs dp;
  int E, A, N, obs_dim, act_dim, device;
  hipStream_t stream;
  float* d_actions;
  float* d_tab;
  float* d_tF; int* d_tI; double* d_tD;
  float* d_XF; int* d_XI;
  double* d_state_io;
  float* d_low;
  float* d_ctlWs8;
  int ctl_np;
  int ctl_rows;
  HeadingPtrs hp; HeadingCfg hc;
  int act_low;
  hipEvent_t ev0, ev1;
  hipEvent_t ev_mid;
  bool mark_mid;
  hipEvent_t ev_order;
  struct HostSet { float* act; float* obs; float* rew; uint8_t* done; int* info; } hs[AC_HOST_SETS];
  bool have_hs[AC_HOST_SETS];
  int* err_host;
  int err_sticky;
  int* count_host;
  bool timing;
  bool quad_waves;
  bool split_waves;
  uint64_t tmpl_hash, ctl_hash;
  int32_t* h_idx; int32_t* d_idx;
  int idx_cap;
  void* h_clone_tab; void* d_clone_tab;
  void* d_snap_hdr;
  unsigned char snap_hdr[1024];
  bool snap_hdr_ok;
  AqlState aql;
  bool stream_dirty;
};

static void geodetic2ecef_m(double lat_deg, double lon_deg, double alt, double* x, double* y, double* z) {
  const double a = 6378137.0, b = 6356752.314245179, D2R = M_PI / 180.0;
  double lat = lat_deg * D2R, lon = lon_deg * D2R;
  double Nn = a * a / hypot(a * cos(lat), b * sin(lat));
  *x = (Nn + alt) * cos(lat) * cos(lon);
  *y = (Nn + alt) * cos(lat) * sin(lon);
  *z = (Nn * (b / a) * (b / a) + alt) * sin(lat);
}

static int check_nonfinite(ac_env* h, const char* who) {
  if (h->err_host && *(volatile int*)h->err_host) h->err_sticky = *(volatile int*)h->err_host;
  if (!h->err_sticky) return 0;
  const int n = std::max(0, std::min(0x3fffffff - (h->err_sticky & 0x3fffffff), h->N - 1));
  char msg[192];
  snprintf(msg, sizeof msg, "%s: JSBSim failed. Non-finite state or reward in env %d, agent %d (ac_reset clears the condition)", who, n / h->A, n % h->A);
  return fail(msg);
}
static int ctl_rows_for(int N, int pinned) { return pinned ? pinned : ((N + 31) / 32 > 256 ? 64 : 32); }
static int ctl_rows_pin() {
  const char* cr = getenv("AIRCOMBAT_CTL_ROWS");
  return cr ? (atoi(cr) == 64 ? 64 : 32) : 0;
}
static int step_plan(ac_env* h, const float* d_actions, int host_set, StepPlan* sp) {
  DevPtrs p = h->dp;
  p.actions = d_actions ? d_actions : h->d_actions;
  if (host_set >= 0) {
    const ac_env::HostSet& hs = h->hs[host_set];
    p.actions = hs.act; p.obs2 = hs.obs; p.rew2 = hs.rew; p.done2 = hs.done; p.info2 = hs.info;
  }
  sp->n = 0;
  const dim3 block(64), grid((h->N + 63) / 64);
  auto add = [&](const void* fn, dim3 g, dim3 b) -> KLaunch& {
    KLaunch& k = sp->k[sp->n++];
    k.fn = fn; k.grid = g; k.block = b; k.size = 0; k.argc = 0;
    return k;
  };
  auto pd = [&](const void* fn, dim3 b) { KLaunch& k = add(fn, grid, b); k.arg(p); k.arg(h->dc); };
  auto scen = [&](const void* fn, dim3 b) {
    KLaunch& k = add(fn, grid, b);
    k.arg(p); k.arg(h->dc); k.arg(h->d_XF); k.arg(h->d_XI); k.arg((const float*)nullptr); k.arg((const int*)nullptr);
  };
  auto heading = [&](const void* fn, dim3 b) { KLaunch& k = add(fn, grid, b); k.arg(p); k.arg(h->dc); k.arg(h->hp); k.arg(h->hc); k.arg((int)0); };
#define AC_K(...) reinterpret_cast<const void*>(&__VA_ARGS__)
  if (h->cfg.hierarchical) {
    if (!h->d_ctlWs8) return fail("hierarchical task: ac_load_controller has not been called");
    ctl::Args a{h->d_ctlWs8, p.actions, p.obs, p.H, h->d_low, h->N, h->obs_dim, h->act_dim, h->act_low,
                h->cfg.use_baseline, h->A, h->cfg.n_ego, h->cfg.use_artillery,
                (float)h->cfg.agent_interaction_steps / (float)h->cfg.sim_freq, p.man_step, p.man_h0, p, h->dc};
    {
      const int rows = ctl_rows_for(h->N, h->ctl_rows);
      const dim3 g8((h->N + rows - 1) / rows);
      const void* fn;
      if (h->ctl_np == 3) {
        if (rows == 64) fn = h->cfg.use_baseline ? AC_K(controller8x3_kernel<true, 4>) : AC_K(controller8x3_kernel<false, 4>);
        else fn = h->cfg.use_baseline ? AC_K(controller8x3_kernel<true, 2>) : AC_K(controller8x3_kernel<false, 2>);
      } else if (rows == 64) fn = h->cfg.use_baseline ? AC_K(controller8_kernel<true, 4>) : AC_K(controller8_kernel<false, 4>);
      else fn = h->cfg.use_baseline ? AC_K(controller8_kernel<true, 2>) : AC_K(controller8_kernel<false, 2>);
      add(fn, g8, dim3(512)).arg(a);
    }
    p.actions = h->d_low;
  }
  const bool one_wave_per_simd = grid.x <= 1024;
  const bool pair_wpe1 = grid.x <= 512;
  const bool gun_only = h->cfg.task == AC_TASK_WVR || h->cfg.task == AC_TASK_MANEUVER;
  if (h->cfg.task == AC_TASK_HEADING) {
    if (h->split_waves) heading(AC_K(step_kernel_heading<true>), dim3(192));
    else if (one_wave_per_simd) heading(AC_K(step_kernel_heading<false, 1>), block);
    else heading(AC_K(step_kernel_heading<false, 2>), block);
  } else if (gun_only) {
    if (h->split_waves) scen(AC_K(step_kernel_scenario<2, 1, FORM_SPLIT>), dim3(192));
    else if (pair_wpe1) scen(AC_K(step_kernel_scenario<2, 1, FORM_PAIR>), dim3(128));
    else scen(AC_K(step_kernel_scenario<2, 2, FORM_PAIR>), dim3(128));
  } else if (h->cfg.task == AC_TASK_DODGE_MISSILE && h->A > 2) {
    if (h->A == 4) scen(pair_wpe1 ? AC_K(step_kernel_scenario<4, 1, FORM_PAIR, true>) : AC_K(step_kernel_scenario<4, 2, FORM_PAIR, true>), dim3(128));
    else scen(pair_wpe1 ? AC_K(step_kernel_scenario<8, 1, FORM_PAIR, true>) : AC_K(step_kernel_scenario<8, 2, FORM_PAIR, true>), dim3(128));
  } else if (h->cfg.task == AC_TASK_SCENARIO1 || h->cfg.task == AC_TASK_SCENARIO_NVN) {
    if (h->A == 2 && h->quad_waves) scen(AC_K(step_kernel_scenario<2, 1, FORM_QUAD>), dim3(256));
    else if (h->A == 2) scen(pair_wpe1 ? AC_K(step_kernel_scenario<2, 1, FORM_PAIR>) : AC_K(step_kernel_scenario<2, 2, FORM_PAIR>), dim3(128));
    else if (h->A == 4) scen(pair_wpe1 ? AC_K(step_kernel_scenario<4, 1, FORM_PAIR>) : AC_K(step_kernel_scenario<4, 2, FORM_PAIR>), dim3(128));
    else scen(pair_wpe1 ? AC_K(step_kernel_scenario<8, 1, FORM_PAIR>) : AC_K(step_kernel_scenario<8, 2, FORM_PAIR>), dim3(128));
  } else if (h->cfg.task == AC_TASK_MULTICOMBAT) {
    if (h->split_waves) pd(h->A == 4 ? AC_K(step_kernel_nvn<4, 1, true>) : AC_K(step_kernel_nvn<8, 1, true>), dim3(192));
    else if (h->A == 4) pd(one_wave_per_simd ? AC_K(step_kernel_nvn<4, 1>) : AC_K(step_kernel_nvn<4, 2>), block);
    else pd(one_wave_per_simd ? AC_K(step_kernel_nvn<8, 1>) : AC_K(step_kernel_nvn<8, 2>), block);
  } else if (h->cfg.task == AC_TASK_SINGLECOMBAT) {
    if (h->split_waves) pd(AC_K(step_kernel_1v1<AC_TASK_SINGLECOMBAT, 1, 1>), dim3(192));
    else if (one_wave_per_simd) pd(AC_K(step_kernel_1v1<AC_TASK_SINGLECOMBAT, 1, 0>), block);
    else pd(AC_K(step_kernel_1v1<AC_TASK_SINGLECOMBAT, 2, 0>), block);
  } else if (h->cfg.task == AC_TASK_DODGE_MISSILE) {
    if (h->quad_waves) pd(AC_K(step_kernel_1v1<AC_TASK_DODGE_MISSILE, 1, 3>), dim3(256));
    else if (pair_wpe1) pd(AC_K(step_kernel_1v1<AC_TASK_DODGE_MISSILE, 1, 2>), dim3(128));
    else pd(AC_K(step_kernel_1v1<AC_TASK_DODGE_MISSILE, 2, 2>), dim3(128));
  } else {
    if (h->quad_waves) pd(AC_K(step_kernel_1v1<AC_TASK_SHOOT_MISSILE, 1, 3>), dim3(256));
    else if (pair_wpe1) pd(AC_K(step_kernel_1v1<AC_TASK_SHOOT_MISSILE, 1, 2>), dim3(128));
    else pd(AC_K(step_kernel_1v1<AC_TASK_SHOOT_MISSILE, 2, 2>), dim3(128));
  }
#undef AC_K
  for (int i = 0; i < sp->n; ++i)
    if (sp->k[i].size > KLaunch::kCap) return fail("step_plan: kernel arguments larger than the kernarg block");
  return 0;
}
static int launch_plan(ac_env* h, const StepPlan& sp) {
  h->stream_dirty = true;
  for (int i = 0; i < sp.n; ++i) {
    const KLaunch& k = sp.k[i];
    HIP_OK(hipLaunchKernel(k.fn, k.grid, k.block, const_cast<void**>(k.argv), 0, h->stream));
    if (i + 1 < sp.n && h->mark_mid) HIP_OK(hipEventRecord(h->ev_mid, h->stream));
  }
  return 0;
}
static int launch_step(ac_env* h, const float* d_actions, int host_set = -1) {
  StepPlan sp;
  if (step_plan(h, d_actions, host_set, &sp)) return -1;
  return launch_plan(h, sp);
}
static int aql_fault(ac_env* h, const std::string& e) {
  h->aql.set_hip("fallback: " + e);
  return fail(e);
}
static int aql_settle(ac_env* h) {
  if (!h->aql.in_flight) return 0;
  const std::string e = aql_wait(&h->aql);
  return e.empty() ? 0 : aql_fault(h, e);
}
static int stream_settle(ac_env* h) {
  if (!h->stream_dirty) return 0;
  HIP_OK(hipStreamSynchronize(h->stream));
  h->stream_dirty = false;
  return 0;
}
static int host_entry(ac_env* h) {
  if (aql_settle(h)) return -1;
  h->stream_dirty = true;
  return 0;
}
static int host_step(ac_env* h, int set) {
  if (aql_settle(h)) return -1;
  StepPlan sp;
  if (step_plan(h, nullptr, set, &sp)) return -1;
  AqlState& a = h->aql;
  bool aql = a.mode == AqlState::READY && !h->timing && sp.n == a.nkern;
  for (int i = 0; aql && i < sp.n; ++i) aql = sp.k[i].fn == a.kern[i].fn;
  if (aql) {
    if (stream_settle(h)) return -1;
    const std::string e = aql_dispatch(&a, sp, set);
    return e.empty() ? 0 : aql_fault(h, e);
  }
  if (launch_plan(h, sp)) return -1;
  if (a.mode == AqlState::PENDING && !h->timing) {
    const std::string e = aql_setup(&a, h->device, sp);
    if (e.empty()) a.mode = AqlState::READY;
    else { aql_release(&a); a.set_hip("fallback: " + e); }
  }
  return 0;
}
static int launch_reset(ac_env* h) {
  dim3 block(64), grid((h->N + 63) / 64);
  if (h->cfg.task == AC_TASK_HEADING) {
    hipLaunchKernelGGL((step_kernel_heading<false, 1>), grid, block, 0, h->stream, h->dp, h->dc, h->hp, h->hc, 1);
    HIP_OK(hipGetLastError());
    return 0;
  }
  hipLaunchKernelGGL(reset_all_kernel, grid, block, 0, h->stream, h->dp, h->dc);
  HIP_OK(hipGetLastError());
  if (h->d_XF) {
    hipLaunchKernelGGL(reset_ext_kernel, grid, block, 0, h->stream, h->dc, h->d_XF, h->d_XI);
    HIP_OK(hipGetLastError());
  }
  return 0;
}

extern "C" {

const char* ac_last_error(void) { return g_err.c_str(); }
const char* ac_version(void) { return "aircombat-hip 0.1 (gfx950)"; }
const char* ac_state_field_name(int i) { return (i >= 0 && i < AC_STATE_LEN && kStateNames[i]) ? kStateNames[i] : ""; }

int ac_create(const ac_config_t* cfg, int32_t n_envs, int32_t device_id, uint64_t seed, ac_env_t** out) {
  if (!cfg || !out) return fail("ac_create: null argument");
  const bool nvn_dodge = cfg->task == AC_TASK_DODGE_MISSILE && cfg->n_agents > 2;
  const bool scenario = cfg->task == AC_TASK_SCENARIO1 || cfg->task == AC_TASK_SCENARIO_NVN || cfg->task == AC_TASK_WVR || cfg->task == AC_TASK_MANEUVER || nvn_dodge;
  const bool heading = cfg->task == AC_TASK_HEADING;
  if (cfg->task != AC_TASK_SINGLECOMBAT && cfg->task != AC_TASK_SHOOT_MISSILE && cfg->task != AC_TASK_DODGE_MISSILE &&
      cfg->task != AC_TASK_MULTICOMBAT && !scenario && !heading)
    return fail("ac_create: unknown task (supported: AC_TASK_HEADING, AC_TASK_SINGLECOMBAT, AC_TASK_DODGE_MISSILE, AC_TASK_SHOOT_MISSILE, AC_TASK_MULTICOMBAT, AC_TASK_SCENARIO1, AC_TASK_SCENARIO_NVN)");
  if (heading && (cfg->n_agents != 1 || cfg->n_ego != 1 || cfg->hierarchical))
    return fail("ac_create: AC_TASK_HEADING is a single-aircraft task with control-index actions (n_agents == n_ego == 1)");
  if (cfg->task == AC_TASK_DODGE_MISSILE && (cfg->sim_freq / cfg->agent_interaction_steps < 1 || cfg->sim_freq / cfg->agent_interaction_steps > 31))
    return fail("ac_create: AC_TASK_DODGE_MISSILE keeps its lock window in 31 bits (needs 1 <= sim_freq / agent_interaction_steps <= 31)");
  if (cfg->task == AC_TASK_SCENARIO_NVN || nvn_dodge) {
    if ((cfg->n_agents != 4 && cfg->n_agents != 8) || cfg->n_ego * 2 != cfg->n_agents)
      return fail("ac_create: AC_TASK_SCENARIO_NVN (and AC_TASK_DODGE_MISSILE with more than two aircraft) needs n_agents in {4, 8} split into two equal teams");
    if (nvn_dodge && cfg->rwr) return fail("ac_create: multiplecombat_dodge_missile has no rwr variant");
  }
  const bool gun_only = cfg->task == AC_TASK_WVR || cfg->task == AC_TASK_MANEUVER;
  if (scenario && !gun_only)
    for (int i = 0; i < cfg->n_agents; ++i)
      if (cfg->num_missiles[i] != 2) return fail("ac_create: the scenario tasks are built for 'missile: 2' (two munition uids per aircraft), as every shipped YAML has");
  if (cfg->task == AC_TASK_SCENARIO_NVN || nvn_dodge) {
  } else if (cfg->task == AC_TASK_MULTICOMBAT) {
    if ((cfg->n_agents != 4 && cfg->n_agents != 8) || cfg->n_ego <= 0 || cfg->n_ego >= cfg->n_agents)
      return fail("ac_create: AC_TASK_MULTICOMBAT needs n_agents in {4, 8} and 0 < n_ego < n_agents");
  } else if (!heading && (cfg->n_agents != 2 || cfg->n_ego != 1)) return fail("ac_create: 1v1 tasks need n_agents == 2 and n_ego == 1");
  if (cfg->controller_precision != AC_CTL_FAST && cfg->controller_precision != AC_CTL_FP32)
    return fail("ac_create: unknown controller_precision (AC_CTL_FAST = 0, AC_CTL_FP32 = 1)");
  if (cfg->controller_precision != AC_CTL_FAST && !cfg->hierarchical)
    return fail("ac_create: controller_precision selects the form of the low-level controller; it needs cfg.hierarchical");
  int ctl_prec = cfg->controller_precision;
  if (const char* pe = getenv("AIRCOMBAT_CTL_PRECISION")) {
    if (!strcmp(pe, "fast")) ctl_prec = AC_CTL_FAST;
    else if (!strcmp(pe, "fp32")) ctl_prec = AC_CTL_FP32;
    else return fail("ac_create: AIRCOMBAT_CTL_PRECISION must be 'fast' or 'fp32'");
  }
  if (cfg->use_baseline && (!cfg->hierarchical || cfg->use_baseline < 0 || cfg->use_baseline > 2 || cfg->n_ego * 2 != cfg->n_agents))
    return fail("ac_create: use_baseline (1 pursue, 2 maneuver) needs the hierarchical form and equal teams (enemy k is flown by scripted agent k)");
  if ((cfg->task == AC_TASK_WVR || cfg->task == AC_TASK_MANEUVER) && (cfg->n_agents != 2 || cfg->n_ego != 1 || cfg->rwr))
    return fail("ac_create: AC_TASK_WVR / AC_TASK_MANEUVER are 1v1 tasks");
  if (cfg->legacy_obs && ((cfg->task != AC_TASK_SCENARIO_NVN && cfg->task != AC_TASK_MULTICOMBAT && !nvn_dodge) || cfg->rwr))
    return fail("ac_create: legacy_obs is the observation of Scenario2 / Scenario3 (AC_TASK_SCENARIO_NVN without rwr) and of "
                "multiplecombat_shoot / hierarchical_multiplecombat_shoot (AC_TASK_MULTICOMBAT)");
  if (cfg->rwr && !scenario) return fail("ac_create: rwr is a variant of the scenario tasks (Scenario1_RWR, Scenario2_RWR, Scenario3_RWR)");
  if (n_envs <= 0) return fail("ac_create: n_envs must be positive");
  if (cfg->max_steps > 65535) return fail("ac_create: max_steps above 65535 (the host-boundary info word carries current_step in 16 bits)");
  if ((long long)n_envs * cfg->n_agents > (1 << 23))
    return fail("ac_create: more than 2^23 aircraft in one handle; shard the envs over handles / GPUs");
  if (cfg->sim_freq != 60) return fail("ac_create: sim_freq must be 60 (the FDM tick is compiled for 1/60 s)");
  for (int i = 0; i < cfg->n_agents; ++i)
    if (cfg->num_missiles[i] < 0 || cfg->num_missiles[i] > AC_MAX_MISSILES_PER_AGENT) return fail("ac_create: num_missiles out of range");
  int ndev = 0;
  HIP_OK(hipGetDeviceCount(&ndev));
  if (device_id < 0 || device_id >= ndev) return fail("ac_create: no such HIP device");
  HIP_OK(hipSetDevice(device_id));
  ac_env* h = new ac_env();
  memset(h, 0, sizeof *h);
  h->cfg = *cfg; h->E = n_envs; h->A = cfg->n_agents; h->N = n_envs * cfg->n_agents; h->device = device_id;
  {
    const char* d = getenv("AIRCOMBAT_DISPATCH");
    if (d && !strcmp(d, "hip")) h->aql.set_hip("AIRCOMBAT_DISPATCH=hip");
  }
  h->cfg.controller_precision = cfg->hierarchical ? ctl_prec : AC_CTL_FAST;
  h->ctl_np = h->cfg.controller_precision == AC_CTL_FP32 ? 3 : 2;
  {
    const char* e = getenv("AIRCOMBAT_SPLIT");
    const int wgs = (h->N + 63) / 64;
    const bool ticks_only = cfg->task == AC_TASK_SINGLECOMBAT || cfg->task == AC_TASK_MULTICOMBAT || cfg->task == AC_TASK_HEADING ||
                            cfg->task == AC_TASK_WVR || cfg->task == AC_TASK_MANEUVER;
    h->split_waves = ticks_only && (e ? (e[0] == '1') : (wgs <= 512));
    h->ctl_rows = ctl_rows_pin();
    const char* qe = getenv("AIRCOMBAT_QUAD");
    const bool munitions_1v1 = cfg->task == AC_TASK_SHOOT_MISSILE || (cfg->task == AC_TASK_DODGE_MISSILE && !nvn_dodge) || cfg->task == AC_TASK_SCENARIO1;
    h->quad_waves = munitions_1v1 && (qe ? (qe[0] == '1') : (wgs <= 256));
  }
  h->obs_dim = heading ? 12 : (cfg->task == AC_TASK_SINGLECOMBAT) ? 15 : (cfg->task == AC_TASK_MULTICOMBAT ? 9 + 6 * (cfg->n_agents - 1) : 21);
  if (cfg->task == AC_TASK_SCENARIO_NVN || nvn_dodge) h->obs_dim = 9 + 6 * cfg->n_agents + 6;
  const int tmpl_obs = h->obs_dim;
  if (gun_only) h->obs_dim = 15;
  if (((cfg->task == AC_TASK_SCENARIO_NVN || cfg->task == AC_TASK_MULTICOMBAT) && cfg->legacy_obs) || nvn_dodge) h->obs_dim = 21;
  if (cfg->rwr) h->obs_dim += 2;
  const bool weapon_bits = scenario && !gun_only && !nvn_dodge;
  h->act_low = weapon_bits ? 8 : ((cfg->task == AC_TASK_SHOOT_MISSILE) ? 5 : 4);
  if (!cfg->hierarchical && cfg->task == AC_TASK_MULTICOMBAT && cfg->legacy_obs) h->act_low = 5;
  h->act_dim = cfg->hierarchical ? (weapon_bits ? 7 : (cfg->task == AC_TASK_SHOOT_MISSILE ? 4 : 3)) : h->act_low;
  if (cfg->hierarchical && cfg->task == AC_TASK_MULTICOMBAT && cfg->legacy_obs) h->act_dim = 4;
  DevCfg& c = h->dc;
  memset(&c, 0, sizeof c);
  c.task = cfg->task; c.A = h->A; c.n_ego = cfg->n_ego; c.substeps = cfg->agent_interaction_steps; c.max_steps = cfg->max_steps;
  c.obs_dim = h->obs_dim; c.act_dim = h->act_low; c.N = h->N;
  c.msl_slots = scenario ? 2 : ((cfg->task == AC_TASK_SHOOT_MISSILE || cfg->task == AC_TASK_DODGE_MISSILE) ? AC_MAX_MISSILES_PER_AGENT : 0);
  c.chaff_seed = seed;
  c.rwr = cfg->rwr ? 1 : 0;
  c.tobs = tmpl_obs;
  c.legacy_obs = (((cfg->task == AC_TASK_SCENARIO_NVN || cfg->task == AC_TASK_MULTICOMBAT) && cfg->legacy_obs) || nvn_dodge) ? 1 : 0;
  c.altitude_limit = (float)cfg->altitude_limit; c.acc_x = (float)cfg->acc_limit_x; c.acc_y = (float)cfg->acc_limit_y; c.acc_z = (float)cfg->acc_limit_z;
  c.posture_scale = (float)cfg->posture_scale; c.altitude_scale = (float)cfg->altitude_scale; c.event_scale = (float)cfg->event_scale;
  c.missile_posture_scale = (float)cfg->missile_posture_scale; c.shoot_penalty_scale = (float)cfg->shoot_penalty_scale;
  c.posture_pot = cfg->posture_potential; c.altitude_pot = cfg->altitude_potential; c.event_pot = cfg->event_potential; c.shoot_pot = cfg->shoot_penalty_potential;
  c.alt_safe = (float)cfg->alt_safe; c.alt_danger = (float)cfg->alt_danger; c.alt_kv = (float)cfg->alt_kv;
  c.max_attack_angle = (float)cfg->max_attack_angle; c.max_attack_distance = (float)cfg->max_attack_distance;
  c.min_attack_interval = cfg->min_attack_interval; c.use_artillery = cfg->use_artillery;
  c.lock_len = (int)(1.0 / ((double)cfg->agent_interaction_steps / cfg->sim_freq));
  for (int i = 0; i < AC_MAX_AGENTS; ++i) c.num_missiles[i] = cfg->num_missiles[i];
  geodetic2ecef_m(cfg->center_lat, cfg->center_lon, cfg->center_alt, &c.P0x, &c.P0y, &c.P0z);
  c.sLat0 = sin(cfg->center_lat * M_PI / 180.0); c.cLat0 = cos(cfg->center_lat * M_PI / 180.0);
  {
    const double a = 6378137.0, f = 1.0 / 298.257223563, e2 = f * (2.0 - f), w2 = 1.0 - e2 * c.sLat0 * c.sLat0;
    c.rn0 = (float)(a / sqrt(w2) + cfg->center_alt);
    c.rm0 = (float)(a * (1.0 - e2) / (w2 * sqrt(w2)) + cfg->center_alt);
    c.h0 = (float)cfg->center_alt;
  }
  c.sLon0 = sin(cfg->center_lon * M_PI / 180.0); c.cLon0 = cos(cfg->center_lon * M_PI / 180.0);

  HIP_OK(hipStreamCreateWithFlags(&h->stream, hipStreamNonBlocking));
  HIP_OK(hipEventCreate(&h->ev0));
  HIP_OK(hipEventCreate(&h->ev1));
  HIP_OK(hipEventCreateWithFlags(&h->ev_order, hipEventDisableTiming));
  HIP_OK(hipEventCreate(&h->ev_mid));
  HIP_OK(hipHostMalloc((void**)&h->err_host, sizeof(int), hipHostMallocDefault));
  *h->err_host = 0; h->err_sticky = 0;
  h->dp.err = h->err_host;
  HIP_OK(hipHostMalloc((void**)&h->count_host, sizeof(int), hipHostMallocDefault));
  const size_t N = (size_t)h->N;
  DevPtrs& p = h->dp;
  HIP_OK(hipMalloc(&p.F, sizeof(float) * NSW * N));
  p.I = reinterpret_cast<int*>(p.F);
  HIP_OK(hipMalloc(&p.D, sizeof(double) * ND * N));
  const size_t ms = c.msl_slots > 0 ? (size_t)c.msl_slots : 1;
  HIP_OK(hipMalloc(&p.MF, sizeof(float) * ms * NMF * N));
  p.MD = nullptr;
  if (scenario) HIP_OK(hipMalloc(&p.MD, sizeof(double) * ms * NMF * N));
  HIP_OK(hipMalloc(&p.MI, sizeof(int) * ms * NMI * N));
  const size_t Npad = (N + 63) / 64 * 64;
  HIP_OK(hipMalloc(&p.obs, sizeof(float) * Npad * h->obs_dim));
  HIP_OK(hipMalloc(&p.rew, sizeof(float) * Npad));
  HIP_OK(hipMalloc(&p.done, Npad));
  HIP_OK(hipMalloc(&p.info, sizeof(int) * 4 * (Npad / h->A)));
  p.obs2 = nullptr; p.rew2 = nullptr; p.done2 = nullptr; p.info2 = nullptr;
  HIP_OK(hipMemset(p.F, 0, sizeof(float) * NSW * N));
  HIP_OK(hipMemset(p.D, 0, sizeof(double) * ND * N));
  HIP_OK(hipMemset(p.MF, 0, sizeof(float) * ms * NMF * N));
  if (p.MD) HIP_OK(hipMemset(p.MD, 0, sizeof(double) * ms * NMF * N));
  HIP_OK(hipMemset(p.MI, 0, sizeof(int) * ms * NMI * N));
  HIP_OK(hipMemset(p.obs, 0, sizeof(float) * Npad * h->obs_dim));
  HIP_OK(hipMemset(p.rew, 0, sizeof(float) * Npad));
  HIP_OK(hipMemset(p.done, 0, Npad));
  HIP_OK(hipMemset(p.info, 0, sizeof(int) * 4 * (Npad / h->A)));
  HIP_OK(hipMalloc(&h->d_actions, sizeof(float) * N * h->act_dim));
  HIP_OK(hipMemset(h->d_actions, 0, sizeof(float) * N * h->act_dim));
  std::vector<float> tab(F16_PACK_LEN);
  for (int i = 0; i < F16_PACK_LEN; ++i) tab[i] = (float)F16_PACK[i];
  HIP_OK(hipMalloc(&h->d_tab, sizeof(float) * F16_PACK_LEN));
  HIP_OK(hipMemcpy(h->d_tab, tab.data(), sizeof(float) * F16_PACK_LEN, hipMemcpyHostToDevice));
  HIP_OK(hipMalloc(&h->d_tF, sizeof(float) * ((size_t)NSW * h->A + (size_t)h->A * tmpl_obs)));
  h->d_tI = reinterpret_cast<int*>(h->d_tF);
  HIP_OK(hipMalloc(&h->d_tD, sizeof(double) * ND * h->A));
  HIP_OK(hipMalloc(&h->d_state_io, sizeof(double) * 256));
  if (scenario) {
    HIP_OK(hipMalloc(&h->d_XF, sizeof(float) * NXF * N));
    HIP_OK(hipMalloc(&h->d_XI, sizeof(int) * NXI * N));
    HIP_OK(hipMemset(h->d_XF, 0, sizeof(float) * NXF * N));
    HIP_OK(hipMemset(h->d_XI, 0, sizeof(int) * NXI * N));
  }
  if (heading) {
    HIP_OK(hipMalloc(&h->hp.HD, sizeof(double) * NHD * N));
    HIP_OK(hipMalloc(&h->hp.HF, sizeof(float) * NHF * N));
    HIP_OK(hipMalloc(&h->hp.HI, sizeof(int) * N));
    HIP_OK(hipMalloc(&h->hp.HR, sizeof(unsigned long long) * 4 * N));
    HIP_OK(hipMemset(h->hp.HD, 0, sizeof(double) * NHD * N));
    HIP_OK(hipMemset(h->hp.HF, 0, sizeof(float) * NHF * N));
    HIP_OK(hipMemset(h->hp.HI, 0, sizeof(int) * N));
    std::vector<unsigned long long> r(4 * N);
    unsigned long long z = seed;
    auto sm = [&z]() { z += 0x9E3779B97F4A7C15ULL; unsigned long long v = z; v = (v ^ (v >> 30)) * 0xBF58476D1CE4E5B9ULL; v = (v ^ (v >> 27)) * 0x94D049BB133111EBULL; return v ^ (v >> 31); };
    for (size_t e = 0; e < N; ++e) { r[0 * N + e] = sm(); r[1 * N + e] = sm(); r[2 * N + e] = sm(); r[3 * N + e] = sm() | 1ULL; }
    HIP_OK(hipMemcpy(h->hp.HR, r.data(), sizeof(unsigned long long) * 4 * N, hipMemcpyHostToDevice));
    h->hc.ic = cfg->init[0];
    h->hc.max_heading_increment = cfg->max_heading_increment; h->hc.max_altitude_increment = cfg->max_altitude_increment;
    h->hc.max_velocities_u_increment = cfg->max_velocities_u_increment; h->hc.check_interval = cfg->check_interval;
    h->hc.heading_scale = (float)cfg->heading_scale; h->hc.heading_pot = cfg->heading_potential;
    h->hc.approach = cfg->approach ? 1 : 0;
  }
  p.H = nullptr; p.man_step = nullptr; p.man_h0 = nullptr;
  if (cfg->hierarchical) {
    HIP_OK(hipMalloc(&p.H, sizeof(float) * 128 * N));
    HIP_OK(hipMemset(p.H, 0, sizeof(float) * 128 * N));
    HIP_OK(hipMalloc(&h->d_low, sizeof(float) * N * h->act_low));
    HIP_OK(hipMemset(h->d_low, 0, sizeof(float) * N * h->act_low));
    HIP_OK(hipMalloc(&p.man_step, sizeof(int) * N));
    HIP_OK(hipMemset(p.man_step, 0, sizeof(int) * N));
    HIP_OK(hipMalloc(&p.man_h0, sizeof(float) * N));
    HIP_OK(hipMemset(p.man_h0, 0, sizeof(float) * N));
  }
  p.tF = h->d_tF; p.tI = h->d_tI; p.tD = h->d_tD; p.tab = h->d_tab; p.actions = h->d_actions;
  InitArgs ia;
  for (int i = 0; i < AC_MAX_AGENTS; ++i) ia.ic[i] = cfg->init[i];
  if (heading) {
  } else if (scenario && h->A == 2)
    hipLaunchKernelGGL(init_kernel_scenario<2>, dim3(1), dim3(64), 0, h->stream, ia, h->dc, h->d_tab, h->d_tF, h->d_tI, h->d_tD);
  else if (scenario && h->A == 4)
    hipLaunchKernelGGL(init_kernel_scenario<4>, dim3(1), dim3(64), 0, h->stream, ia, h->dc, h->d_tab, h->d_tF, h->d_tI, h->d_tD);
  else if (scenario)
    hipLaunchKernelGGL(init_kernel_scenario<8>, dim3(1), dim3(64), 0, h->stream, ia, h->dc, h->d_tab, h->d_tF, h->d_tI, h->d_tD);
  else if (cfg->task == AC_TASK_MULTICOMBAT && h->A == 4)
    hipLaunchKernelGGL(init_kernel_nvn<4>, dim3(1), dim3(64), 0, h->stream, ia, h->dc, h->d_tab, h->d_tF, h->d_tI, h->d_tD);
  else if (cfg->task == AC_TASK_MULTICOMBAT)
    hipLaunchKernelGGL(init_kernel_nvn<8>, dim3(1), dim3(64), 0, h->stream, ia, h->dc, h->d_tab, h->d_tF, h->d_tI, h->d_tD);
  else if (cfg->task == AC_TASK_SINGLECOMBAT)
    hipLaunchKernelGGL(init_kernel_1v1<AC_TASK_SINGLECOMBAT>, dim3(1), dim3(64), 0, h->stream, ia, h->dc, h->d_tab, h->d_tF, h->d_tI, h->d_tD);
  else
    hipLaunchKernelGGL(init_kernel_1v1<AC_TASK_SHOOT_MISSILE>, dim3(1), dim3(64), 0, h->stream, ia, h->dc, h->d_tab, h->d_tF, h->d_tI, h->d_tD);
  HIP_OK(hipGetLastError());
  if (launch_reset(h)) return -1;
  HIP_OK(hipStreamSynchronize(h->stream));
  *out = h;
  return 0;
}

int ac_destroy(ac_env_t* h) {
  if (!h) return 0;
  (void)hipSetDevice(h->device);
  (void)aql_settle(h);
  aql_release(&h->aql);
  (void)hipStreamSynchronize(h->stream);
  void* bufs[] = {h->dp.F, h->dp.D, h->dp.MF, h->dp.MD, h->dp.MI, h->dp.obs, h->dp.rew, h->dp.done, h->dp.info,
                  h->d_actions, h->d_tab, h->d_tF, h->d_tD, h->d_state_io, h->d_XF, h->d_XI, h->dp.H, h->dp.man_step, h->dp.man_h0, h->d_ctlWs8, h->d_low, h->hp.HD, h->hp.HF, h->hp.HI, h->hp.HR,
                  h->d_idx, h->d_clone_tab, h->d_snap_hdr};
  for (void* b : bufs) (void)hipFree(b);
  for (int k = 0; k < AC_HOST_SETS; ++k)
    if (h->have_hs[k]) ac_host_set_free(h->hs[k].act, h->hs[k].obs, h->hs[k].rew, h->hs[k].done, h->hs[k].info);
  if (h->err_host) (void)hipHostFree(h->err_host);
  if (h->count_host) (void)hipHostFree(h->count_host);
  if (h->h_idx) (void)hipHostFree(h->h_idx);
  if (h->h_clone_tab) (void)hipHostFree(h->h_clone_tab);
  (void)hipEventDestroy(h->ev0); (void)hipEventDestroy(h->ev1); (void)hipEventDestroy(h->ev_order); (void)hipEventDestroy(h->ev_mid);
  (void)hipStreamDestroy(h->stream);
  delete h;
  return 0;
}
int ac_obs_dim(const ac_env_t* h) { return h ? h->obs_dim : -1; }
int ac_act_dim(const ac_env_t* h) { return h ? h->act_dim : -1; }
int ac_num_envs(const ac_env_t* h) { return h ? h->E : -1; }
int ac_num_agents(const ac_env_t* h) { return h ? h->A : -1; }

int ac_reset(ac_env_t* h, float* obs) {
  if (!h) return fail("ac_reset: null handle");
  if (host_entry(h)) return -1;
  HIP_OK(hipSetDevice(h->device));
  HIP_OK(hipStreamSynchronize(h->stream));
  *h->err_host = 0; h->err_sticky = 0;
  if (launch_reset(h)) return -1;
  if (obs) HIP_OK(hipMemcpyAsync(obs, h->dp.obs, sizeof(float) * (size_t)h->N * h->obs_dim, hipMemcpyDeviceToHost, h->stream));
  HIP_OK(hipStreamSynchronize(h->stream));
  return 0;
}

int ac_step(ac_env_t* h, const float* actions, float* obs, float* rewards, uint8_t* dones, int32_t* info) {
  if (!h || !actions) return fail("ac_step: null argument");
  if (host_entry(h)) return -1;
  HIP_OK(hipSetDevice(h->device));
  const size_t N = (size_t)h->N;
  HIP_OK(hipMemcpyAsync(h->d_actions, actions, sizeof(float) * N * h->act_dim, hipMemcpyHostToDevice, h->stream));
  if (launch_step(h, nullptr)) return -1;
  if (obs) HIP_OK(hipMemcpyAsync(obs, h->dp.obs, sizeof(float) * N * h->obs_dim, hipMemcpyDeviceToHost, h->stream));
  if (rewards) HIP_OK(hipMemcpyAsync(rewards, h->dp.rew, sizeof(float) * N, hipMemcpyDeviceToHost, h->stream));
  if (dones) HIP_OK(hipMemcpyAsync(dones, h->dp.done, N, hipMemcpyDeviceToHost, h->stream));
  if (info) HIP_OK(hipMemcpyAsync(info, h->dp.info, sizeof(int) * 4 * h->E, hipMemcpyDeviceToHost, h->stream));
  HIP_OK(hipStreamSynchronize(h->stream));
  return check_nonfinite(h, "ac_step");
}

int ac_host_buffers(ac_env_t* h, int32_t set, float** actions, float** obs, float** rewards, uint8_t** dones, int32_t** info) {
  if (!h || set < 0 || set >= AC_HOST_SETS) return fail("ac_host_buffers: bad argument (sets 0 .. AC_HOST_SETS - 1)");
  HIP_OK(hipSetDevice(h->device));
  ac_env::HostSet& hs = h->hs[set];
  if (!h->have_hs[set]) {
    const size_t Npad = ((size_t)h->N + 63) / 64 * 64;
    HIP_OK(hipHostMalloc((void**)&hs.act, sizeof(float) * Npad * h->act_dim, hipHostMallocDefault));
    HIP_OK(hipHostMalloc((void**)&hs.obs, sizeof(float) * Npad * h->obs_dim, hipHostMallocDefault));
    HIP_OK(hipHostMalloc((void**)&hs.rew, sizeof(float) * Npad, hipHostMallocDefault));
    HIP_OK(hipHostMalloc((void**)&hs.done, Npad, hipHostMallocDefault));
    HIP_OK(hipHostMalloc((void**)&hs.info, sizeof(int) * (Npad / h->A), hipHostMallocDefault));
    memset(hs.act, 0, sizeof(float) * Npad * h->act_dim); memset(hs.obs, 0, sizeof(float) * Npad * h->obs_dim);
    memset(hs.rew, 0, sizeof(float) * Npad); memset(hs.done, 0, Npad); memset(hs.info, 0, sizeof(int) * (Npad / h->A));
    h->have_hs[set] = true;
  }
  if (actions) *actions = hs.act;
  if (obs) *obs = hs.obs;
  if (rewards) *rewards = hs.rew;
  if (dones) *dones = hs.done;
  if (info) *info = hs.info;
  return 0;
}
int ac_host_set_detach(ac_env_t* h, int32_t set) {
  if (!h || set < 0 || set >= AC_HOST_SETS || !h->have_hs[set]) return fail("ac_host_set_detach: no such set");
  if (host_entry(h)) return -1;
  HIP_OK(hipSetDevice(h->device));
  HIP_OK(hipStreamSynchronize(h->stream));
  h->have_hs[set] = false;
  memset(&h->hs[set], 0, sizeof h->hs[set]);
  return 0;
}
void ac_host_set_free(void* actions, void* obs, void* rewards, void* dones, void* info) {
  (void)hipHostFree(actions); (void)hipHostFree(obs); (void)hipHostFree(rewards); (void)hipHostFree(dones); (void)hipHostFree(info);
}
int ac_step_host_async(ac_env_t* h, int32_t set) {
  if (!h || set < 0 || set >= AC_HOST_SETS) return fail("ac_step_host_async: bad argument");
  if (!h->have_hs[set]) return fail("ac_step_host_async: call ac_host_buffers for this set first");
  HIP_OK(hipSetDevice(h->device));
  return host_step(h, set);
}
int ac_step_host_wait(ac_env_t* h) {
  if (!h) return fail("ac_step_host_wait: null handle");
  if (h->aql.in_flight) {
    if (aql_settle(h)) return -1;
  } else {
    HIP_OK(hipStreamSynchronize(h->stream));
    h->stream_dirty = false;
  }
  return check_nonfinite(h, "ac_step_host_wait");
}
int ac_step_host(ac_env_t* h, int32_t set) {
  if (ac_step_host_async(h, set)) return -1;
  return ac_step_host_wait(h);
}

int ac_order_after(ac_env_t* h, void* producer_stream) {
  if (!h) return fail("ac_order_after: null handle");
  if (host_entry(h)) return -1;
  HIP_OK(hipSetDevice(h->device));
  HIP_OK(hipEventRecord(h->ev_order, (hipStream_t)producer_stream));
  HIP_OK(hipStreamWaitEvent(h->stream, h->ev_order, 0));
  return 0;
}
int ac_order_before(ac_env_t* h, void* consumer_stream) {
  if (!h) return fail("ac_order_before: null handle");
  if (host_entry(h)) return -1;
  HIP_OK(hipSetDevice(h->device));
  HIP_OK(hipEventRecord(h->ev_order, h->stream));
  HIP_OK(hipStreamWaitEvent((hipStream_t)consumer_stream, h->ev_order, 0));
  return 0;
}

int ac_step_async_device(ac_env_t* h, const float* d_actions) {
  if (!h) return fail("ac_step_async_device: null handle");
  if (host_entry(h)) return -1;
  HIP_OK(hipSetDevice(h->device));
  return launch_step(h, d_actions);
}
int ac_device_buffers(ac_env_t* h, float** d_actions, float** d_obs, float** d_rewards, uint8_t** d_dones, int32_t** d_info) {
  if (!h) return fail("ac_device_buffers: null handle");
  if (d_actions) *d_actions = h->d_actions;
  if (d_obs) *d_obs = h->dp.obs;
  if (d_rewards) *d_rewards = h->dp.rew;
  if (d_dones) *d_dones = h->dp.done;
  if (d_info) *d_info = h->dp.info;
  return 0;
}
void* ac_stream(ac_env_t* h) {
  if (!h) return nullptr;
  (void)host_entry(h);
  return (void*)h->stream;
}
const char* ac_dispatch_path(ac_env_t* h) {
  if (!h) return "";
  switch (h->aql.mode) {
    case AqlState::READY: return "aql";
    case AqlState::PENDING: return "pending";
    default: return h->aql.why;
  }
}
int ac_sync(ac_env_t* h) {
  if (!h) return fail("ac_sync: null handle");
  if (host_entry(h)) return -1;
  HIP_OK(hipSetDevice(h->device));
  HIP_OK(hipStreamSynchronize(h->stream));
  h->stream_dirty = false;
  return check_nonfinite(h, "ac_sync");
}
int ac_timing_begin(ac_env_t* h) {
  if (!h) return fail("ac_timing_begin: null handle");
  if (host_entry(h)) return -1;
  HIP_OK(hipEventRecord(h->ev0, h->stream));
  h->timing = true;
  return 0;
}
int ac_timing_end(ac_env_t* h, float* total_ms) {
  if (!h || !total_ms) return fail("ac_timing_end: null argument");
  if (host_entry(h)) return -1;
  h->timing = false;
  HIP_OK(hipEventRecord(h->ev1, h->stream));
  HIP_OK(hipEventSynchronize(h->ev1));
  HIP_OK(hipEventElapsedTime(total_ms, h->ev0, h->ev1));
  return 0;
}

int ac_step_timed_device(ac_env_t* h, const float* d_actions, float* controller_ms, float* step_ms) {
  if (!h || !controller_ms || !step_ms) return fail("ac_step_timed_device: null argument");
  if (host_entry(h)) return -1;
  HIP_OK(hipSetDevice(h->device));
  HIP_OK(hipEventRecord(h->ev0, h->stream));
  h->mark_mid = h->cfg.hierarchical != 0;
  const int rc = launch_step(h, d_actions);
  h->mark_mid = false;
  if (rc) return rc;
  HIP_OK(hipEventRecord(h->ev1, h->stream));
  HIP_OK(hipEventSynchronize(h->ev1));
  *controller_ms = 0.0f;
  if (h->cfg.hierarchical) {
    HIP_OK(hipEventElapsedTime(controller_ms, h->ev0, h->ev_mid));
    HIP_OK(hipEventElapsedTime(step_ms, h->ev_mid, h->ev1));
  } else HIP_OK(hipEventElapsedTime(step_ms, h->ev0, h->ev1));
  return check_nonfinite(h, "ac_step_timed_device");
}

static float* storage_word(float* S, int w, size_t N, size_t n) { return S + (((size_t)(w >> 2) * N + n) * 4 + (size_t)(w & 3)); }
static double* position_word(double* D, int f, size_t N, size_t n) { return f < 2 ? D + 2 * n + f : D + 2 * N + n; }
static int check_idx(ac_env_t* h, int env, int agent) {
  if (!h) return fail("null handle");
  if (env < 0 || env >= h->E || agent < 0 || agent >= h->A) return fail("env/agent index out of range");
  return 0;
}
struct SlotMap { int f[NF]; int i[NI]; };
constexpr int kStateIoWords = ND + NF + NI + NXI + NXF;
static_assert(kStateIoWords <= 256, "state_io_kernel: one thread per word of a 256-thread block");
__global__ void state_io_kernel(float* F, double* D, const float* XF, const int* XI, size_t N, size_t n, double* io, int write, SlotMap m) {
  const int t = threadIdx.x;
  if (t < ND) {
    double* w = t < 2 ? D + 2 * n + t : D + 2 * N + n;
    if (write) *w = io[t]; else io[t] = *w;
  } else if (t < ND + NF) {
    const int sw = m.f[t - ND];
    float* w = F + (((size_t)(sw >> 2) * N + n) * 4 + (size_t)(sw & 3));
    if (write) *w = (float)io[t]; else io[t] = (double)*w;
  } else if (t < ND + NF + NI) {
    const int sw = m.i[t - ND - NF];
    int* w = reinterpret_cast<int*>(F + (((size_t)(sw >> 2) * N + n) * 4 + (size_t)(sw & 3)));
    if (write) *w = (int)llround(io[t]); else io[t] = (double)*w;
  } else if (!write && t < kStateIoWords) {
    const int q = t - (ND + NF + NI);
    if (q < NXI) io[t] = XI ? (double)XI[(size_t)q * N + n] : 0.0;
    else io[t] = XF ? (double)XF[(size_t)(q - NXI) * N + n] : 0.0;
  }
}
static SlotMap slot_map() {
  SlotMap m;
  for (int f = 0; f < NF; ++f) m.f[f] = kSlotF[f];
  for (int f = 0; f < NI; ++f) m.i[f] = kSlotI[f];
  return m;
}
int ac_get_state(ac_env_t* h, int32_t env, int32_t agent, double* out) {
  if (check_idx(h, env, agent) || !out) return fail("ac_get_state: bad argument");
  if (host_entry(h)) return -1;
  HIP_OK(hipSetDevice(h->device));
  const size_t N = h->N, n = (size_t)env * h->A + agent;
  double io[kStateIoWords];
  hipLaunchKernelGGL(state_io_kernel, dim3(1), dim3(256), 0, h->stream, h->dp.F, h->dp.D, h->d_XF, h->d_XI, N, n, h->d_state_io, 0, slot_map());
  HIP_OK(hipGetLastError());
  HIP_OK(hipMemcpyAsync(io, h->d_state_io, sizeof io, hipMemcpyDeviceToHost, h->stream));
  HIP_OK(hipStreamSynchronize(h->stream));
  int k = 0;
  for (int f = 0; f < ND + NF + NI; ++f) out[k++] = io[f];
  if (h->d_XF) {
    {
      const double* w = io + ND + NF + NI;
      Ext x{};
      ext_unpack((int)w[XI_w0], (int)w[XI_w1], x);
      const int v[NXI_UNPACKED] = {x.rem_gun, x.rem_9m, x.rem_120b, x.rem_chaff, x.bits, x.last_chaff, x.orphan_hits, x.mp_prev, x.ref_set,
                                   x.ch_status[0], x.ch_mult[0], x.ch_status[1], x.ch_mult[1], x.n_ch};
      for (int f = 0; f < NXI_UNPACKED; ++f) out[k++] = v[f];
    }
    for (int f = 0; f < NXF; ++f) out[k++] = io[ND + NF + NI + NXI + f];
  }
  for (; k < AC_STATE_LEN; ++k) out[k] = 0.0;
  return 0;
}
int ac_set_state(ac_env_t* h, int32_t env, int32_t agent, const double* in) {
  if (check_idx(h, env, agent) || !in) return fail("ac_set_state: bad argument");
  if (host_entry(h)) return -1;
  HIP_OK(hipSetDevice(h->device));
  const size_t N = h->N, n = (size_t)env * h->A + agent;
  HIP_OK(hipMemcpyAsync(h->d_state_io, in, sizeof(double) * (ND + NF + NI), hipMemcpyHostToDevice, h->stream));
  hipLaunchKernelGGL(state_io_kernel, dim3(1), dim3(256), 0, h->stream, h->dp.F, h->dp.D, h->d_XF, h->d_XI, N, n, h->d_state_io, 1, slot_map());
  HIP_OK(hipGetLastError());
  HIP_OK(hipStreamSynchronize(h->stream));
  return 0;
}
int ac_set_status(ac_env_t* h, int32_t env, int32_t agent, int32_t status) {
  if (check_idx(h, env, agent)) return -1;
  if (host_entry(h)) return -1;
  if (status < AC_ALIVE || status > AC_SHOTDOWN) return fail("ac_set_status: bad status");
  HIP_OK(hipSetDevice(h->device));
  HIP_OK(hipStreamSynchronize(h->stream));
  const size_t N = h->N, n = (size_t)env * h->A + agent;
  int v = status;
  HIP_OK(hipMemcpy(storage_word(h->dp.F, SW_status, N, n), &v, sizeof v, hipMemcpyHostToDevice));
  return 0;
}

__global__ void entity_kernel(DevPtrs P, DevCfg c, int n, double* out) {
  if (threadIdx.x != 0 || blockIdx.x != 0) return;
  State s; Task t; Derived d; Props pr;
  load_state(P.F, P.I, P.D, c.N, n, s, t);
  f16::locate(s, d); f16::body_frame(s, d);
  make_props(s, d, c, pr);
  const double R2D = 180.0 / 3.14159265358979323846;
  out[0] = atan2(d.sLon64, d.cLon64) * R2D; out[1] = atan2(d.sLat64, d.cLat64) * R2D; out[2] = pr.alt_m;
  out[3] = atan2f(pr.sphi, pr.cphi); out[4] = asinf(pr.stht);
  float psi = atan2f(pr.m12, pr.m11); if (psi < 0.0f) psi += 2.0f * f16::kPi;
  out[5] = psi; out[6] = pr.vn; out[7] = pr.ve; out[8] = pr.vd; out[9] = pr.n; out[10] = pr.e; out[11] = pr.u;
}
int ac_get_entity(ac_env_t* h, int32_t env, int32_t agent, double out[12]) {
  if (check_idx(h, env, agent) || !out) return fail("ac_get_entity: bad argument");
  if (host_entry(h)) return -1;
  HIP_OK(hipSetDevice(h->device));
  double* d_out = h->d_state_io;
  hipLaunchKernelGGL(entity_kernel, dim3(1), dim3(64), 0, h->stream, h->dp, h->dc, env * h->A + agent, d_out);
  HIP_OK(hipGetLastError());
  HIP_OK(hipMemcpyAsync(out, d_out, sizeof(double) * 12, hipMemcpyDeviceToHost, h->stream));
  HIP_OK(hipStreamSynchronize(h->stream));
  return 0;
}
__global__ void state_checksum_kernel(DevPtrs P, DevCfg c, unsigned long long* out) {
  const int N = c.N;
  const int n = blockIdx.x * blockDim.x + threadIdx.x;
  unsigned long long acc = 0;
  if (n < N) {
    auto mix = [](unsigned long long v, unsigned f) {
      unsigned long long z = v + 0x9E3779B97F4A7C15ULL * (unsigned long long)(f + 1);
      z ^= z >> 30; z *= 0xBF58476D1CE4E5B9ULL; z ^= z >> 27; z *= 0x94D049BB133111EBULL; z ^= z >> 31;
      return z;
    };
    for (int g = 0; g < NSG; ++g) {
      const float4 v = reinterpret_cast<const float4*>(P.F)[(size_t)g * N + n];
      acc += mix((unsigned long long)__float_as_uint(v.x), 4 * g) + mix((unsigned long long)__float_as_uint(v.y), 4 * g + 1) +
             mix((unsigned long long)__float_as_uint(v.z), 4 * g + 2) + mix((unsigned long long)__float_as_uint(v.w), 4 * g + 3);
    }
    {
      const double2 xy = reinterpret_cast<const double2*>(P.D)[n];
      acc += mix((unsigned long long)__double_as_longlong(xy.x), NSW) + mix((unsigned long long)__double_as_longlong(xy.y), NSW + 1) +
             mix((unsigned long long)__double_as_longlong(P.D[2 * (size_t)N + n]), NSW + 2);
    }
  }
#pragma unroll
  for (int o = 32; o > 0; o >>= 1) acc += __shfl_xor(acc, o);
  if ((threadIdx.x & 63) == 0) atomicAdd(out, acc);
}
int ac_state_checksum(ac_env_t* h, uint64_t* out) {
  if (!h || !out) return fail("ac_state_checksum: null argument");
  if (host_entry(h)) return -1;
  HIP_OK(hipSetDevice(h->device));
  unsigned long long* d_out;
  HIP_OK(hipMalloc(&d_out, sizeof(unsigned long long)));
  HIP_OK(hipMemsetAsync(d_out, 0, sizeof(unsigned long long), h->stream));
  dim3 block(64), grid((h->N + 63) / 64);
  hipLaunchKernelGGL(state_checksum_kernel, grid, block, 0, h->stream, h->dp, h->dc, d_out);
  HIP_OK(hipGetLastError());
  HIP_OK(hipStreamSynchronize(h->stream));
  unsigned long long v = 0;
  HIP_OK(hipMemcpy(&v, d_out, sizeof v, hipMemcpyDeviceToHost));
  HIP_OK(hipFree(d_out));
  *out = (uint64_t)v;
  return 0;
}
__global__ void munitions_in_flight_kernel(DevPtrs P, DevCfg c, int* out) {
  const int N = c.N;
  const int n = blockIdx.x * blockDim.x + threadIdx.x;
  int cnt = 0;
  if (n < N)
    for (int k = 0; k < c.msl_slots; ++k) cnt += P.MI[((size_t)k * NMI + MI_status) * (size_t)N + n] == MSL_LAUNCHED;
#pragma unroll
  for (int o = 32; o > 0; o >>= 1) cnt += __shfl_xor(cnt, o);
  if ((threadIdx.x & 63) == 0 && cnt) __hip_atomic_fetch_add(out, cnt, __ATOMIC_RELAXED, __HIP_MEMORY_SCOPE_SYSTEM);
}
int ac_munitions_in_flight(ac_env_t* h, int32_t* count) {
  if (!h || !count) return fail("ac_munitions_in_flight: null argument");
  if (host_entry(h)) return -1;
  *count = 0;
  if (!h->dc.msl_slots || !h->dp.MI) return 0;
  HIP_OK(hipSetDevice(h->device));
  HIP_OK(hipStreamSynchronize(h->stream));
  *(volatile int*)h->count_host = 0;
  hipLaunchKernelGGL(munitions_in_flight_kernel, dim3((h->N + 63) / 64), dim3(64), 0, h->stream, h->dp, h->dc, h->count_host);
  HIP_OK(hipGetLastError());
  HIP_OK(hipStreamSynchronize(h->stream));
  *count = *(volatile int*)h->count_host;
  return 0;
}
int ac_seed_envs(ac_env_t* h, const uint64_t* states) {
  if (!h || !states) return fail("ac_seed_envs: null argument");
  if (host_entry(h)) return -1;
  if (h->cfg.task != AC_TASK_HEADING) return fail("ac_seed_envs: only AC_TASK_HEADING draws from env.np_random");
  HIP_OK(hipSetDevice(h->device));
  HIP_OK(hipStreamSynchronize(h->stream));
  const size_t N = h->N;
  std::vector<unsigned long long> r(4 * N);
  for (size_t e = 0; e < N; ++e)
    for (int k = 0; k < 4; ++k) r[k * N + e] = states[e * 4 + k];
  HIP_OK(hipMemcpy(h->hp.HR, r.data(), sizeof(unsigned long long) * 4 * N, hipMemcpyHostToDevice));
  return 0;
}
int ac_get_heading_state(ac_env_t* h, int32_t env, double out[8]) {
  if (check_idx(h, env, 0) || !out) return fail("ac_get_heading_state: bad argument");
  if (host_entry(h)) return -1;
  if (h->cfg.task != AC_TASK_HEADING) return fail("ac_get_heading_state: not an AC_TASK_HEADING handle");
  HIP_OK(hipSetDevice(h->device));
  HIP_OK(hipStreamSynchronize(h->stream));
  const size_t N = h->N, n = env;
  for (int f = 0; f < NHD; ++f) HIP_OK(hipMemcpy(&out[f], h->hp.HD + f * N + n, sizeof(double), hipMemcpyDeviceToHost));
  int tc; HIP_OK(hipMemcpy(&tc, h->hp.HI + n, sizeof tc, hipMemcpyDeviceToHost));
  out[5] = tc;
  float lp, lq;
  HIP_OK(hipMemcpy(&lp, h->hp.HF + HF_last_p * N + n, sizeof lp, hipMemcpyDeviceToHost));
  HIP_OK(hipMemcpy(&lq, h->hp.HF + HF_last_q * N + n, sizeof lq, hipMemcpyDeviceToHost));
  out[6] = lp; out[7] = lq;
  return 0;
}
int ac_pin_host_buffer(ac_env_t* h, void* ptr, int64_t bytes) {
  if (!h || !ptr || bytes <= 0) return fail("ac_pin_host_buffer: bad argument");
  HIP_OK(hipSetDevice(h->device));
  HIP_OK(hipHostRegister(ptr, (size_t)bytes, hipHostRegisterDefault));
  return 0;
}
int ac_unpin_host_buffer(ac_env_t* h, void* ptr) {
  if (!h || !ptr) return fail("ac_unpin_host_buffer: bad argument");
  HIP_OK(hipSetDevice(h->device));
  HIP_OK(hipHostUnregister(ptr));
  return 0;
}
}

template <int NP>
static std::vector<float> controller_blob(const float* weights) {
  using namespace ctl;
  using L = ctl8::Lay<NP>;
  std::vector<float> e(L::C_END, 0.0f);
// ... 195 lines not shown
```

aircombat-selfplay_amd/csrc/snapshot.hpp:

```cpp

enum { AC_SNAP_MAGIC = 0x4e534341u , AC_SNAP_FORMAT = 1, AC_SNAP_HDR = 1024, AC_SNAP_MAX_SECTIONS = 32, AC_SNAP_ALIGN = 256 };

struct AcSnapHeader {
  uint32_t magic, format;
  char version[64];
  int32_t task, E, A, msl_slots, obs_dim, act_dim, act_low, ctl_precision, hierarchical, n_sections, reserved0, reserved1;
  uint64_t config_hash;
  uint64_t total_bytes;
  uint64_t offset[AC_SNAP_MAX_SECTIONS], bytes[AC_SNAP_MAX_SECTIONS];
  uint8_t pad[AC_SNAP_HDR - 136 - 16 * AC_SNAP_MAX_SECTIONS];
};
static_assert(sizeof(AcSnapHeader) == AC_SNAP_HDR, "snapshot header is 1024 bytes");

struct SnapSection {
  char* dev;
  size_t bytes;
  uint32_t rows, row_stride, chunk;
};

static std::vector<SnapSection> snap_sections(const ac_env* h) {
  const uint32_t N = (uint32_t)h->N, A = (uint32_t)h->A, E = (uint32_t)h->E;
  const uint32_t ms = h->dc.msl_slots > 0 ? (uint32_t)h->dc.msl_slots : 1;
  std::vector<SnapSection> s;
  auto rows = [&](void* p, uint32_t n_rows, uint32_t elem) {
    if (p) s.push_back({(char*)p, (size_t)n_rows * N * elem, n_rows, N * elem, A * elem});
  };
  auto per_env = [&](void* p, uint32_t chunk) { s.push_back({(char*)p, (size_t)E * chunk, 1, E * chunk, chunk}); };
  rows(h->dp.F, NSG, 16);
  rows(h->dp.D, 1, 16);
  rows((char*)h->dp.D + (size_t)16 * N, 1, 8);
  rows(h->dp.MF, ms * NMF, 4);
  rows(h->dp.MI, ms * NMI, 4);
  rows(h->dp.MD, ms * NMF, 8);
  rows(h->d_XF, NXF, 4);
  rows(h->d_XI, NXI, 4);
  rows(h->hp.HD, NHD, 8);
  rows(h->hp.HF, NHF, 4);
  rows(h->hp.HI, 1, 4);
  rows(h->hp.HR, 4, 8);
  rows(h->dp.H, 128, 4);
  if (h->d_low) per_env(h->d_low, A * (uint32_t)h->act_low * 4);
  rows(h->dp.man_step, 1, 4);
  rows(h->dp.man_h0, 1, 4);
  per_env(h->dp.obs, A * (uint32_t)h->obs_dim * 4);
  rows(h->dp.rew, 1, 4);
  rows(h->dp.done, 1, 1);
  per_env(h->dp.info, 16);
  return s;
}

static int snap_config_hash(ac_env* h, uint64_t* out) {
  if (!h->tmpl_hash) {
    const int A = h->A;
    std::vector<float> tf((size_t)NSW * A + (size_t)A * h->dc.tobs);
    std::vector<double> td((size_t)ND * A);
    HIP_OK(hipStreamSynchronize(h->stream));
    if (h->cfg.task != AC_TASK_HEADING) {
      HIP_OK(hipMemcpy(tf.data(), h->d_tF, sizeof(float) * tf.size(), hipMemcpyDeviceToHost));
      HIP_OK(hipMemcpy(td.data(), h->d_tD, sizeof(double) * td.size(), hipMemcpyDeviceToHost));
    }
    uint64_t t = fnv1a(0xCBF29CE484222325ULL, tf.data(), sizeof(float) * tf.size());
    h->tmpl_hash = fnv1a(t, td.data(), sizeof(double) * td.size()) | 1ULL;
  }
  DevCfg c = h->dc;
  if (!h->d_XF) c.chaff_seed = 0;
  uint64_t x = fnv1a(0xCBF29CE484222325ULL, &c, sizeof c);
  if (h->cfg.task == AC_TASK_HEADING) x = fnv1a(x, &h->hc, sizeof h->hc);
  const int32_t form[10] = {h->cfg.hierarchical, h->cfg.use_baseline, h->cfg.controller_precision, h->act_dim, h->act_low, h->obs_dim,
                            (int32_t)h->split_waves, (int32_t)h->quad_waves, h->ctl_rows, h->E};
  x = fnv1a(x, form, sizeof form);
  x = fnv1a(x, &h->tmpl_hash, sizeof h->tmpl_hash);
  x = fnv1a(x, &h->ctl_hash, sizeof h->ctl_hash);
  *out = x;
  return 0;
}

static int snap_header(ac_env* h, AcSnapHeader* hd) {
  memset(hd, 0, sizeof *hd);
  hd->magic = AC_SNAP_MAGIC; hd->format = AC_SNAP_FORMAT;
  strncpy(hd->version, ac_version(), sizeof hd->version - 1);
  hd->task = h->cfg.task; hd->E = h->E; hd->A = h->A; hd->msl_slots = h->dc.msl_slots; hd->obs_dim = h->obs_dim; hd->act_dim = h->act_dim;
  hd->act_low = h->act_low; hd->ctl_precision = h->cfg.controller_precision; hd->hierarchical = h->cfg.hierarchical;
  if (snap_config_hash(h, &hd->config_hash)) return -1;
  const std::vector<SnapSection> s = snap_sections(h);
  if (s.size() > AC_SNAP_MAX_SECTIONS) return fail("snapshot: too many sections");
  hd->n_sections = (int32_t)s.size();
  uint64_t off = AC_SNAP_HDR;
  for (size_t k = 0; k < s.size(); ++k) {
    hd->offset[k] = off; hd->bytes[k] = s[k].bytes;
    off = (off + s[k].bytes + AC_SNAP_ALIGN - 1) / AC_SNAP_ALIGN * AC_SNAP_ALIGN;
  }
  hd->total_bytes = off;
  return 0;
}

static int snap_check(ac_env* h, const AcSnapHeader& got, const char* who) {
  AcSnapHeader want;
  if (snap_header(h, &want)) return -1;
  char msg[256];
  auto bad = [&](const char* what, long long a, long long b) {
    snprintf(msg, sizeof msg, "%s: snapshot %s is %lld, this handle's is %lld", who, what, a, b);
    return fail(msg);
  };
  if (got.magic != AC_SNAP_MAGIC) return fail(std::string(who) + ": not an env snapshot (bad magic word)");
  if (got.format != AC_SNAP_FORMAT) return bad("format version", got.format, want.format);
  if (strncmp(got.version, want.version, sizeof want.version))
    return fail(std::string(who) + ": snapshot written by '" + std::string(got.version, strnlen(got.version, sizeof got.version)) + "', this library is '" + want.version + "'");
  if (got.task != want.task) return bad("task", got.task, want.task);
  if (got.E != want.E) return bad("number of envs", got.E, want.E);
  if (got.A != want.A) return bad("number of agents", got.A, want.A);
  if (got.msl_slots != want.msl_slots) return bad("munition slot count", got.msl_slots, want.msl_slots);
  if (got.obs_dim != want.obs_dim) return bad("obs_dim", got.obs_dim, want.obs_dim);
  if (got.act_dim != want.act_dim) return bad("act_dim", got.act_dim, want.act_dim);
  if (got.hierarchical != want.hierarchical) return bad("hierarchical flag", got.hierarchical, want.hierarchical);
  if (got.ctl_precision != want.ctl_precision) return bad("controller precision", got.ctl_precision, want.ctl_precision);
  if (got.config_hash != want.config_hash)
    return fail(std::string(who) + ": snapshot config digest differs (config, reset template, seed, controller weights or kernel form)");
  if (got.n_sections != want.n_sections || got.total_bytes != want.total_bytes ||
      memcmp(got.offset, want.offset, sizeof want.offset) || memcmp(got.bytes, want.bytes, sizeof want.bytes))
    return fail(std::string(who) + ": snapshot section layout differs");
  return 0;
}

struct CloneSeg { char* dst; const char* src; uint32_t row_stride, chunk, row0, shift; };
struct CloneTable { CloneSeg s[AC_SNAP_MAX_SECTIONS]; int32_t nseg; };

typedef int clone_v4 __attribute__((ext_vector_type(4)));
template <typename T>
__device__ __forceinline__ void clone_piece(char* d, const char* s) {
#if defined(__HIP_DEVICE_COMPILE__)
  typedef __attribute__((address_space(1))) T GT;
  *(GT*)d = *(const GT*)s;
#endif
}

__global__ void __launch_bounds__(256) clone_envs_kernel(const CloneTable* __restrict__ T, const int32_t* __restrict__ src_env,
                                                         const int32_t* __restrict__ dst_env, int32_t n) {
  const uint32_t y = blockIdx.y;
  int k = 0;
  while (k + 1 < T->nseg && y >= T->s[k + 1].row0) ++k;
  const char* src = T->s[k].src;
  char* dst = T->s[k].dst;
  const uint32_t shift = T->s[k].shift, chunk = T->s[k].chunk;
  const size_t row = (size_t)(y - T->s[k].row0) * T->s[k].row_stride;
  const uint32_t pieces = chunk >> shift;
  const uint32_t t = blockIdx.x * blockDim.x + threadIdx.x;
  if (t >= (uint32_t)n * pieces) return;
  const uint32_t p = t / pieces, v = (t - p * pieces) << shift;
  const char* s = src + row + (size_t)src_env[p] * chunk + v;
  char* d = dst + row + (size_t)dst_env[p] * chunk + v;
  switch (shift) {
    case 4: clone_piece<clone_v4>(d, s); break;
    case 3: clone_piece<long long>(d, s); break;
    case 2: clone_piece<int>(d, s); break;
    default: clone_piece<char>(d, s); break;
  }
}

__global__ void snapshot_checksum_kernel(const uint32_t* __restrict__ w, size_t nw, uint32_t section, unsigned long long* out) {
  unsigned long long acc = 0;
  for (size_t i = blockIdx.x * (size_t)blockDim.x + threadIdx.x; i < nw; i += (size_t)gridDim.x * blockDim.x) {
    unsigned long long z = ((unsigned long long)w[i] | ((unsigned long long)section << 32)) + 0x9E3779B97F4A7C15ULL * (i + 1);
    z ^= z >> 30; z *= 0xBF58476D1CE4E5B9ULL; z ^= z >> 27; z *= 0x94D049BB133111EBULL; z ^= z >> 31;
    acc += z;
  }
#pragma unroll
  for (int o = 32; o > 0; o >>= 1) acc += __shfl_xor(acc, o);
  if ((threadIdx.x & 63) == 0) atomicAdd(out, acc);
}

static int snap_scratch(ac_env* h, int32_t n) {
  if (n <= h->idx_cap) return 0;
  if (h->h_idx) HIP_OK(hipHostFree(h->h_idx));
  if (h->d_idx) HIP_OK(hipFree(h->d_idx));
  h->h_idx = nullptr; h->d_idx = nullptr; h->idx_cap = 0;
  HIP_OK(hipHostMalloc((void**)&h->h_idx, sizeof(int32_t) * 2 * (size_t)n, hipHostMallocDefault));
  HIP_OK(hipMalloc(&h->d_idx, sizeof(int32_t) * 2 * (size_t)n));
  h->idx_cap = n;
  return 0;
}

static int snap_stage_indices(ac_env* h, const int32_t* src, const int32_t* dst, int32_t n, const char* who) {
  if (n <= 0 || !dst) return fail(std::string(who) + ": need n > 0 env indices");
  if (n > h->E) return fail(std::string(who) + ": more destination envs than the handle has (a destination may appear once)");
  if (snap_scratch(h, n)) return -1;
  HIP_OK(hipStreamSynchronize(h->stream));
  int32_t* hs = h->h_idx; int32_t* hd = h->h_idx + n;
  auto fetch = [&](int32_t* to, const int32_t* from) -> int {
    hipPointerAttribute_t a;
    const bool on_device = hipPointerGetAttributes(&a, from) == hipSuccess && a.type == hipMemoryTypeDevice;
    (void)hipGetLastError();
    if (!on_device) { memcpy(to, from, sizeof(int32_t) * n); return 0; }
    HIP_OK(hipMemcpyAsync(to, from, sizeof(int32_t) * n, hipMemcpyDeviceToHost, h->stream));
    return 0;
  };
  if (fetch(hd, dst) || (src && fetch(hs, src))) return -1;
  HIP_OK(hipStreamSynchronize(h->stream));
  if (!src) memcpy(hs, hd, sizeof(int32_t) * n);
  std::vector<uint8_t> seen(h->E, 0);
  char msg[192];
  for (int32_t k = 0; k < n; ++k) {
    if (hs[k] < 0 || hs[k] >= h->E || hd[k] < 0 || hd[k] >= h->E) {
      snprintf(msg, sizeof msg, "%s: env index out of range at position %d (src %d, dst %d; the handle has %d envs)", who, k, hs[k], hd[k], h->E);
      return fail(msg);
    }
    if (seen[hd[k]]++) {
      snprintf(msg, sizeof msg, "%s: destination env %d appears twice", who, hd[k]);
      return fail(msg);
    }
  }
  if (src) {
    std::vector<int32_t> writer(h->E, -1);
    for (int32_t k = 0; k < n; ++k) writer[hd[k]] = hs[k];
    for (int32_t k = 0; k < n; ++k)
      if (writer[hs[k]] >= 0 && writer[hs[k]] != hs[k]) {
        snprintf(msg, sizeof msg, "%s: env %d is both a source (position %d) and a destination of the same call; clone in two calls", who, hs[k], k);
        return fail(msg);
      }
  }
  HIP_OK(hipMemcpyAsync(h->d_idx, h->h_idx, sizeof(int32_t) * 2 * (size_t)n, hipMemcpyHostToDevice, h->stream));
  return 0;
}
// ... 187 lines not shown
```

aircombat-selfplay_amd/csrc/split_kernel.hpp:

```cpp
#pragma once

namespace mail {
enum { RUNF,
       CTH, VB,
       MACH, QBAR, RHO, TEMP, HSL, ALPHA, BETA, QC, VG, NPY, NPZ, AP, AQ, AR,
       S_AIL, S_FLAP, S_ELEV, S_RUD, S_LEF, S_SB,
       THRUST,
       LK_CLB, LK_CNB, LK_G7,
       MASS0 = LK_G7 + 4, MASS_N = 18,
       F_TEF = MASS0 + MASS_N, F_PINR, F_PINP, F_PINY, F_PIR, F_PIP, F_PIY, F_AIL, F_ELEV, F_SBDEG, F_N1, F_N2, F_N2NORM, F_FF, F_TANK0, F_TANK1,
       F_ENG, F_DA, F_DE, F_DR, F_THR,
       F_BITS,
       K_W, K_V = K_W + 3,
       K_OUT = K_V + 3, K_OUT_N = 27,
       G_Q = K_OUT + K_OUT_N,
       G_H = G_Q + 8, G_NED = G_H + 1,
       QP_F = G_NED + 8, QP_F_N = 9,
       T_PR = QP_F + 2 * QP_F_N, T_PR_N = 15,
       T_DONE = T_PR + T_PR_N,
       T_RALT = T_DONE + 1, T_RPOS,
       ROWS = T_RPOS + 1 };
enum { GD_R, GD_X = GD_R + 6, GD_LAT = GD_X + 3, GD_QP = GD_LAT + 4, DROWS = GD_QP + 6 };
}
__device__ __forceinline__ void post_kin(float (*M)[64], int l, const f16::KinOut& o) {
  const float v[mail::K_OUT_N] = {o.T[0], o.T[1], o.T[2], o.T[3], o.T[4], o.T[5], o.T[6], o.T[7], o.T[8], o.h_sl_ft, o.n_eci[0], o.n_eci[1], o.n_eci[2],
                                  o.e_eci[0], o.e_eci[1], o.d_eci[0], o.d_eci[1], o.d_eci[2], o.gx, o.gy, o.gz, o.rxf, o.ryf, o.A.T, o.A.P, o.A.rho, o.A.a};
#pragma unroll
  for (int i = 0; i < mail::K_OUT_N; ++i) M[mail::K_OUT + i][l] = v[i];
}
__device__ __forceinline__ void fetch_kin(float (*M)[64], int l, f16::KinOut& o) {
  float v[mail::K_OUT_N];
#pragma unroll
  for (int i = 0; i < mail::K_OUT_N; ++i) v[i] = M[mail::K_OUT + i][l];
#pragma unroll
  for (int i = 0; i < 9; ++i) o.T[i] = v[i];
  o.h_sl_ft = v[9]; o.n_eci[0] = v[10]; o.n_eci[1] = v[11]; o.n_eci[2] = v[12]; o.e_eci[0] = v[13]; o.e_eci[1] = v[14];
  o.d_eci[0] = v[15]; o.d_eci[1] = v[16]; o.d_eci[2] = v[17]; o.gx = v[18]; o.gy = v[19]; o.gz = v[20]; o.rxf = v[21]; o.ryf = v[22];
  o.A.T = v[23]; o.A.P = v[24]; o.A.rho = v[25]; o.A.a = v[26];
}
__device__ __forceinline__ void post_mass(float (*M)[64], int l, const f16::DynVars& k) {
  const float v[mail::MASS_N] = {k.mass, k.cgx, k.cgy, k.cgz, k.Jxx, k.Jyy, k.Jzz, k.Jxy, k.Jxz, k.Jyz, k.c00, k.c01, k.c02, k.c11, k.c12, k.c22, k.idet, k.im_};
#pragma unroll
  for (int i = 0; i < mail::MASS_N; ++i) M[mail::MASS0 + i][l] = v[i];
}
__device__ __forceinline__ void fetch_mass(float (*M)[64], int l, f16::DynVars& k) {
  float v[mail::MASS_N];
#pragma unroll
  for (int i = 0; i < mail::MASS_N; ++i) v[i] = M[mail::MASS0 + i][l];
  k.mass = v[0]; k.cgx = v[1]; k.cgy = v[2]; k.cgz = v[3]; k.Jxx = v[4]; k.Jyy = v[5]; k.Jzz = v[6]; k.Jxy = v[7]; k.Jxz = v[8]; k.Jyz = v[9];
  k.c00 = v[10]; k.c01 = v[11]; k.c02 = v[12]; k.c11 = v[13]; k.c12 = v[14]; k.c22 = v[15]; k.idet = v[16]; k.im_ = v[17];
}
__device__ __forceinline__ void wg_sync() {
  __builtin_amdgcn_fence(__ATOMIC_RELEASE, "workgroup");
  __builtin_amdgcn_s_barrier();
  __builtin_amdgcn_fence(__ATOMIC_ACQUIRE, "workgroup");
}
typedef float f32x4 __attribute__((ext_vector_type(4)));
struct ActionRow {
  f32x4 v;
  __device__ __forceinline__ void issue(const float* p) { asm volatile("global_load_dwordx4 %0, %1, off" : "=&v"(v) : "v"(p) : "memory"); }
  __device__ __forceinline__ void take() { asm volatile("s_waitcnt vmcnt(0)" : "+v"(v) : : "memory"); }
};
struct ActionWord {
  float v;
  __device__ __forceinline__ void issue(const float* p) { asm volatile("global_load_dword %0, %1, off" : "=&v"(v) : "v"(p) : "memory"); }
  __device__ __forceinline__ void take() { asm volatile("s_waitcnt vmcnt(0)" : "+v"(v) : : "memory"); }
};
struct ActionFetch {
  ActionRow idx, bits;
  ActionWord bit;
  int extra;
  __device__ __forceinline__ void issue(const float* act, int act_dim) {
    extra = act_dim == 8 ? 4 : (act_dim == 5 ? 1 : 0);
    idx.issue(act);
    if (extra == 4) bits.issue(act + 4);
    if (extra == 1) bit.issue(act + 4);
  }
  __device__ __forceinline__ void take() { idx.take(); if (extra == 4) bits.take(); if (extra == 1) bit.take(); }
  __device__ __forceinline__ float packed() const {
    if (extra == 4) return (float)((bits.v.x != 0.0f ? 1 : 0) | (bits.v.y != 0.0f ? 2 : 0) | (bits.v.z != 0.0f ? 4 : 0) | (bits.v.w != 0.0f ? 8 : 0));
    if (extra == 1) return bit.v != 0.0f ? 1.0f : 0.0f;
    return 0.0f;
  }
};
__device__ __forceinline__ void systems_wave(f16::State& s, Task& t, const f16::Tab& T, float (*M)[64], int l, int substeps, const float4* raw = nullptr,
                                             ActionFetch* row = nullptr) {
  using namespace mail;
  f16::DynVars km{};
  f16::sys_mass(s, km);
  post_mass(M, l, km);
  (void)t;
  for (int sub = 0; sub < substeps; ++sub) {
    f16::Surf sf{};
    AC_CLKW(1, 64 + sub * 8);
    wg_sync();
    if (row && sub == 0) {
      row->take();
      s.da = f16::clampf(-1.0f, row->idx.v.x / 20.0f - 1.0f, 1.0f);
      s.de = f16::clampf(-1.0f, row->idx.v.y / 20.0f - 1.0f, 1.0f);
      s.dr = f16::clampf(-1.0f, row->idx.v.z / 20.0f - 1.0f, 1.0f);
      s.thr = f16::clampf(0.0f, row->idx.v.w / 58.0f + 0.4f, 0.9f);
    } else if (raw && sub == 0) {
      s.da = f16::clampf(-1.0f, raw->x / 20.0f - 1.0f, 1.0f);
      s.de = f16::clampf(-1.0f, raw->y / 20.0f - 1.0f, 1.0f);
      s.dr = f16::clampf(-1.0f, raw->z / 20.0f - 1.0f, 1.0f);
      s.thr = f16::clampf(0.0f, raw->w / 58.0f + 0.4f, 0.9f);
    }
    const bool run = M[RUNF][l] != 0.0f;
    if (run) {
      f16::sys_fcs(s, M[CTH][l], M[VB][l], sf);
      M[S_AIL][l] = sf.aileron_rad; M[S_FLAP][l] = sf.flaperon_rad; M[S_ELEV][l] = sf.elevator_rad;
      M[S_RUD][l] = sf.rudder_rad;  M[S_LEF][l] = sf.lef_rad;       M[S_SB][l] = sf.sb_rad;
    }
    AC_CLKW(1, 65 + sub * 8);
    wg_sync();
    if (run) {
      f16::Atmos A{};
      A.rho = M[RHO][l]; A.T = M[TEMP][l];
      const float mach = M[MACH][l], alpha = M[ALPHA][l], h_sl = M[HSL][l];
      float thrust;
      f16::sys_engine(s, T, mach, M[QBAR][l], A, h_sl, sf.throttle_pos, thrust);
      M[THRUST][l] = thrust;
    }
    AC_CLKW(1, 66 + sub * 8);
    wg_sync();
    if (run) {
      s.alpha = M[ALPHA][l]; s.mach = M[MACH][l]; s.qc = M[QC][l]; s.vg = M[VG][l];
      s.npy = M[NPY][l]; s.npz = M[NPZ][l]; s.ap = M[AP][l]; s.aq = M[AQ][l]; s.ar = M[AR][l];
      f16::sys_mass(s, km);
      post_mass(M, l, km);
    }
  }
  if (substeps == 0 && (row || raw)) {
    f32x4 v;
    if (row) { row->take(); v = row->idx.v; } else { v.x = raw->x; v.y = raw->y; v.z = raw->z; v.w = raw->w; }
    s.da = f16::clampf(-1.0f, v.x / 20.0f - 1.0f, 1.0f); s.de = f16::clampf(-1.0f, v.y / 20.0f - 1.0f, 1.0f);
    s.dr = f16::clampf(-1.0f, v.z / 20.0f - 1.0f, 1.0f); s.thr = f16::clampf(0.0f, v.w / 58.0f + 0.4f, 0.9f);
  }
  M[F_TEF][l] = s.tef; M[F_PINR][l] = s.pin_r; M[F_PINP][l] = s.pin_p; M[F_PINY][l] = s.pin_y;
  M[F_PIR][l] = s.pi_r; M[F_PIP][l] = s.pi_p; M[F_PIY][l] = s.pi_y; M[F_AIL][l] = s.ail; M[F_ELEV][l] = s.elev; M[F_SBDEG][l] = s.sbdeg;
  M[F_N1][l] = s.n1; M[F_N2][l] = s.n2; M[F_N2NORM][l] = s.n2norm; M[F_FF][l] = s.ff; M[F_TANK0][l] = s.tank0; M[F_TANK1][l] = s.tank1;
  M[F_ENG][l] = __int_as_float(s.eng);
  M[F_DA][l] = s.da; M[F_DE][l] = s.de; M[F_DR][l] = s.dr; M[F_THR][l] = s.thr;
  M[F_BITS][l] = row ? row->packed() : 0.0f;
  wg_sync();
}
__device__ __forceinline__ void post_quad_pose(float (*M)[64], double (*MD)[64], int l, int pb, const f16::State& s, int ticks, const DevCfg& c) {
  using namespace mail;
  f16::State sp{};
  sp.rx = s.rx; sp.ry = s.ry; sp.rz = s.rz; sp.ticks = ticks;
  f16::Derived dp;
  f16::locate(sp, dp);
  dp.vn = 0.0f; dp.ve = 0.0f; dp.vd = 0.0f;
  Props pp;
  make_pose(dp, c, pp);
  MD[GD_QP + 3 * pb][l] = pp.n64; MD[GD_QP + 3 * pb + 1][l] = pp.e64; MD[GD_QP + 3 * pb + 2][l] = pp.u64;
  const int r = QP_F + QP_F_N * pb;
  M[r][l] = pp.alt_m;
  M[r + 1][l] = dp.n_eci[0]; M[r + 2][l] = dp.n_eci[1]; M[r + 3][l] = dp.n_eci[2];
  M[r + 4][l] = dp.e_eci[0]; M[r + 5][l] = dp.e_eci[1];
  M[r + 6][l] = dp.d_eci[0]; M[r + 7][l] = dp.d_eci[1]; M[r + 8][l] = dp.d_eci[2];
}
template <bool QUAD = false, bool POSE = false>
__device__ __forceinline__ void kinematics_wave(f16::State& s, Task& t, const f16::Tab& T, float (*M)[64], double (*MD)[64], int l, int substeps,
                                                const DevCfg* cfg = nullptr) {
  using namespace mail;
  f16::KinOut o;
  const int ticks0 = s.ticks;
  const bool alive0 = t.status == AC_ALIVE && substeps > 0;
  if (alive0) { f16::kin_position(s, o); f16::kin_attitude(s, o); }
  if (QUAD) { MD[GD_R][l] = s.rx; MD[GD_R + 1][l] = s.ry; MD[GD_R + 2][l] = s.rz; }
  if (POSE) post_quad_pose(M, MD, l, 0, s, ticks0 + (alive0 ? 1 : 0), *cfg);
  for (int sub = 0; sub < substeps; ++sub) {
    AC_CLKW(2, 68 + sub * 8);
    wg_sync();
    const bool run = M[RUNF][l] != 0.0f;
    const bool last = sub + 1 == substeps;
    if (run) {
      const int pb = sub & 1;
      if (!QUAD) { MD[GD_R + 3 * pb][l] = s.rx; MD[GD_R + 3 * pb + 1][l] = s.ry; MD[GD_R + 3 * pb + 2][l] = s.rz; }
      M[G_Q + 4 * pb][l] = s.q0; M[G_Q + 4 * pb + 1][l] = s.q1; M[G_Q + 4 * pb + 2][l] = s.q2; M[G_Q + 4 * pb + 3][l] = s.q3;
    }
    if (run && !last) {
      s.wp = M[K_W][l]; s.wq = M[K_W + 1][l]; s.wr = M[K_W + 2][l];
      s.vx = M[K_V][l]; s.vy = M[K_V + 1][l]; s.vz = M[K_V + 2][l];
      f16::kin_position(s, o);
      if (QUAD) { const int nb = (sub + 1) & 1; MD[GD_R + 3 * nb][l] = s.rx; MD[GD_R + 3 * nb + 1][l] = s.ry; MD[GD_R + 3 * nb + 2][l] = s.rz; }
    } else if (run) {
      f16::Derived d;
      s.ticks += substeps;
      f16::locate(s, d);
      M[G_H][l] = d.h_sl_ft;
      M[G_NED][l] = d.n_eci[0]; M[G_NED + 1][l] = d.n_eci[1]; M[G_NED + 2][l] = d.n_eci[2];
      M[G_NED + 3][l] = d.e_eci[0]; M[G_NED + 4][l] = d.e_eci[1];
      M[G_NED + 5][l] = d.d_eci[0]; M[G_NED + 6][l] = d.d_eci[1]; M[G_NED + 7][l] = d.d_eci[2];
      MD[GD_X][l] = d.X; MD[GD_X + 1][l] = d.Y; MD[GD_X + 2][l] = d.Z;
      MD[GD_LAT][l] = d.sLat64; MD[GD_LAT + 1][l] = d.cLat64; MD[GD_LAT + 2][l] = d.sLon64; MD[GD_LAT + 3][l] = d.cLon64;
    }
    AC_CLKW(2, 69 + sub * 8);
    wg_sync();
    if (run) {
      f16::DynVars kl{};
      f16::Derived dd{};
      dd.h_sl_ft = 1e6f;
      kl.alpha = M[ALPHA][l]; kl.beta = M[BETA][l]; kl.mach = M[MACH][l]; kl.vt = 1.0f;
      f16::dyn_p3(dd, T, kl, f16::Surf{});
      M[LK_CLB][l] = kl.clb; M[LK_CNB][l] = kl.cnb;
      M[LK_G7][l] = kl.g7.x; M[LK_G7 + 1][l] = kl.g7.y; M[LK_G7 + 2][l] = kl.g7.z; M[LK_G7 + 3][l] = kl.g7.w;
    }
    if (run && !last) {
      f16::kin_attitude(s, o);
      post_kin(M, l, o);
    }
    AC_CLKW(2, 70 + sub * 8);
    wg_sync();
    if (POSE && run && !last) post_quad_pose(M, MD, l, (sub + 1) & 1, s, ticks0 + sub + 2, *cfg);
  }
  wg_sync();
}
struct SplitLds {
  float M[mail::ROWS][64];
  double MD[mail::DROWS][64];
};
template <bool QUAD = false, bool POSE = false>
__device__ __forceinline__ bool split_helper_wave(f16::State& s, Task& t, const f16::Tab& T, SplitLds& L, int l, int substeps, const float4* raw = nullptr,
                                                  const DevCfg* cfg = nullptr, ActionFetch* row = nullptr) {
  const int role = __builtin_amdgcn_readfirstlane(threadIdx.x >> 6);
  if (role == 2) { kinematics_wave<QUAD, POSE>(s, t, T, L.M, L.MD, l, substeps, cfg); return true; }
  if (role == 1) { systems_wave(s, t, T, L.M, l, substeps, raw, row); return true; }
  return false;
}
template <bool QUAD = false>
__device__ __forceinline__ bool dynamics_wave_tick(f16::State& s, Task& t, f16::Derived& d, const f16::Tab& T, SplitLds& L, int l, int sub, bool* d_stale = nullptr) {
  using namespace mail;
  float (*M)[64] = L.M;
  double (*MD)[64] = L.MD;
  bool run = t.status == AC_ALIVE;
  if (!QUAD && run && t.bloods <= 0.0f) t.status = AC_SHOTDOWN;
  f16::DynVars k;
  AC_CLK(2 + sub * 8);
  if (!QUAD) M[RUNF][l] = run ? 1.0f : 0.0f;
  const float b_wp = s.wp, b_wq = s.wq, b_wr = s.wr, b_vx = s.vx, b_vy = s.vy, b_vz = s.vz, b_ax = s.ha1x, b_ay = s.ha1y, b_az = s.ha1z;
  const float b_h1x = s.hv1x, b_h1y = s.hv1y, b_h1z = s.hv1z, b_h2x = s.hv2x, b_h2y = s.hv2y, b_h2z = s.hv2z;
  const int b_ticks = s.ticks;
  if (QUAD && !run) { M[K_V][l] = s.vx; M[K_V + 1][l] = s.vy; M[K_V + 2][l] = s.vz; }
  if (run) {
    if (sub == 0) f16::dyn_p1(s, d, k);
    else {
      f16::KinOut o;
      fetch_kin(M, l, o);
      f16::dyn_p1_lite(s, d, k, o);
    }
    M[K_W][l] = s.wp; M[K_W + 1][l] = s.wq; M[K_W + 2][l] = s.wr;
    M[K_V][l] = s.vx; M[K_V + 1][l] = s.vy; M[K_V + 2][l] = s.vz;
    M[CTH][l] = d.T[6] * d.d_eci[0] + d.T[7] * d.d_eci[1] + d.T[8] * d.d_eci[2];
    M[VB][l] = d.v;
  }
  AC_CLK(3 + sub * 8);
  wg_sync();
  AC_CLK(4 + sub * 8);
  if (QUAD && run && M[RUNF][l] == 0.0f) {
    s.wp = b_wp; s.wq = b_wq; s.wr = b_wr; s.vx = b_vx; s.vy = b_vy; s.vz = b_vz; s.ha1x = b_ax; s.ha1y = b_ay; s.ha1z = b_az; s.ticks = b_ticks;
    s.hv1x = b_h1x; s.hv1y = b_h1y; s.hv1z = b_h1z; s.hv2x = b_h2x; s.hv2y = b_h2y; s.hv2z = b_h2z;
    t.status = AC_SHOTDOWN;
    run = false;
    if (d_stale) *d_stale = true;
  }
  if (run) {
    fetch_mass(M, l, k);
    if (sub == 0) f16::dyn_p2<false>(s, d, k);
    else f16::dyn_p2<true>(s, d, k);
    M[BETA][l] = k.beta;
    M[MACH][l] = k.mach; M[QBAR][l] = k.qbar; M[RHO][l] = k.A.rho; M[TEMP][l] = k.A.T; M[HSL][l] = d.h_sl_ft;
    M[ALPHA][l] = k.alpha; M[QC][l] = k.qc; M[VG][l] = k.vg; M[NPY][l] = k.npy; M[NPZ][l] = k.npz;
    M[AP][l] = d.p; M[AQ][l] = d.q; M[AR][l] = d.r;
  }
  AC_CLK(5 + sub * 8);
  wg_sync();
  AC_CLK(6 + sub * 8);
  f16::Surf sf{};
  if (run) {
    sf = f16::Surf{M[S_AIL][l], M[S_FLAP][l], M[S_ELEV][l], M[S_RUD][l], M[S_LEF][l], M[S_SB][l], 0.0f};
    f16::dyn_p3(d, T, k, sf);
  }
  AC_CLK(7 + sub * 8);
  wg_sync();
  AC_CLK(8 + sub * 8);
  if (run) {
    k.clb = M[LK_CLB][l]; k.cnb = M[LK_CNB][l];
    k.g7 = make_float4(M[LK_G7][l], M[LK_G7 + 1][l], M[LK_G7 + 2][l], M[LK_G7 + 3][l]);
    f16::dyn_p4(s, d, k, sf, M[THRUST][l]);
    if (sub > 0) {
      const int pb = sub & 1;
      s.rx = MD[GD_R + 3 * pb][l]; s.ry = MD[GD_R + 3 * pb + 1][l]; s.rz = MD[GD_R + 3 * pb + 2][l];
    }
  }
  return run;
}
__device__ __forceinline__ bool dynamics_wave_finish(f16::State& s, f16::Derived& d, SplitLds& L, int l, int last_tick, int substeps) {
  using namespace mail;
  float (*M)[64] = L.M;
  double (*MD)[64] = L.MD;
  AC_CLK(50);
  wg_sync();
  AC_CLK(51);
  s.tef = M[F_TEF][l]; s.pin_r = M[F_PINR][l]; s.pin_p = M[F_PINP][l]; s.pin_y = M[F_PINY][l];
  s.pi_r = M[F_PIR][l]; s.pi_p = M[F_PIP][l]; s.pi_y = M[F_PIY][l]; s.ail = M[F_AIL][l]; s.elev = M[F_ELEV][l]; s.sbdeg = M[F_SBDEG][l];
  s.n1 = M[F_N1][l]; s.n2 = M[F_N2][l]; s.n2norm = M[F_N2NORM][l]; s.ff = M[F_FF][l]; s.tank0 = M[F_TANK0][l]; s.tank1 = M[F_TANK1][l];
  s.eng = __float_as_int(M[F_ENG][l]);
  s.da = M[F_DA][l]; s.de = M[F_DE][l]; s.dr = M[F_DR][l]; s.thr = M[F_THR][l];
  if (last_tick >= 1) {
    const int pb = last_tick & 1;
    s.q0 = M[G_Q + 4 * pb][l]; s.q1 = M[G_Q + 4 * pb + 1][l]; s.q2 = M[G_Q + 4 * pb + 2][l]; s.q3 = M[G_Q + 4 * pb + 3][l];
  }
  if (last_tick < 0 || last_tick != substeps - 1) return false;
  d.X = MD[GD_X][l]; d.Y = MD[GD_X + 1][l]; d.Z = MD[GD_X + 2][l];
  d.sLat64 = MD[GD_LAT][l]; d.cLat64 = MD[GD_LAT + 1][l]; d.sLon64 = MD[GD_LAT + 2][l]; d.cLon64 = MD[GD_LAT + 3][l];
  d.h_sl_ft = M[G_H][l];
  d.n_eci[0] = M[G_NED][l]; d.n_eci[1] = M[G_NED + 1][l]; d.n_eci[2] = M[G_NED + 2][l];
  d.e_eci[0] = M[G_NED + 3][l]; d.e_eci[1] = M[G_NED + 4][l]; d.e_eci[2] = 0.0f;
  d.d_eci[0] = M[G_NED + 5][l]; d.d_eci[1] = M[G_NED + 6][l]; d.d_eci[2] = M[G_NED + 7][l];
  return true;
}
__device__ __forceinline__ bool dynamics_wave_ticks(f16::State& s, Task& t, f16::Derived& d, const f16::Tab& T, SplitLds& L, int l, int substeps,
                                                    int& nrun) {
  int last_tick = -1;
  nrun = 0;
  for (int sub = 0; sub < substeps; ++sub)
    if (dynamics_wave_tick(s, t, d, T, L, l, sub)) { last_tick = sub; nrun += 1; }
  const bool located = dynamics_wave_finish(s, d, L, l, last_tick, substeps);
  if (last_tick >= 0 && !located) { f16::locate(s, d); return true; }
  return located;
}
```

Baseline: 236.6 million.

## Carry kinematics look-ahead across steps and let helper waves store their own state

Adds a persistent per-agent look-ahead buffer holding the kinematics outputs (position, attitude, atmosphere) computed after the last substep. The next step reuses it so the dynamics wave can skip dyn_p1 and the full dyn_p2 at substep 0. The systems wave now writes its own flight-state groups straight to global memory, and the dynamics wave stores only its own groups. This cuts LDS mailbox traffic and serialized global stores. In exchange it adds extra global memory per agent, extra barriers, an invalidation path on state writes and resets, and more complex correctness coupling between the waves.

```diff
diff --git a/aircombat-selfplay_amd/csrc/aircombat.hip b/aircombat-selfplay_amd/csrc/aircombat.hip
--- a/aircombat-selfplay_amd/csrc/aircombat.hip
+++ b/aircombat-selfplay_amd/csrc/aircombat.hip
@@ -130,6 +130,7 @@
 
 struct DevPtrs {
   float* F; int* I; double* D;
+  float* LA;
   float* MF; int* MI;
   double* MD;
   float* H;
@@ -184,14 +185,21 @@
   if (ROLE != 1) load_position(D, N, n, s);
 }
 __device__ __forceinline__ void load_flight(const float* F, const int* I, const double* D, int N, int n, State& s) { load_flight_role<-1>(F, I, D, N, n, s); }
+constexpr bool ac_role_stores(int role, int g) {
+  return role < 0 || (role == 1 ? (g <= 5 || g == 14) : (g >= 6 && g <= 13));
+}
+template <int ROLE>
+__device__ __forceinline__ void store_flight_role(float* F, double* D, int N, int n, const State& s) {
+  AC_LANE_INDEX(n);
+#define G(g, a, b, c, d) if (ac_role_stores(ROLE, g)) AC_GRP(F, g) = make_float4(s.a, s.b, s.c, s.d);
+  AC_FLIGHT_GROUPS(G)
+#undef G
+  if (ac_role_stores(ROLE, 6)) AC_GRP(F, 6) = make_float4(s.npz, s.npx, __int_as_float(s.eng), __int_as_float(s.ticks));
+  if (ROLE != 1) store_position(D, N, n, s);
+}
 __device__ __forceinline__ void store_flight(float* F, int* I, double* D, int N, int n, const State& s) {
   (void)I;
-  AC_LANE_INDEX(n);
-#define G(g, a, b, c, d) AC_GRP(F, g) = make_float4(s.a, s.b, s.c, s.d);
-  AC_FLIGHT_GROUPS(G)
-#undef G
-  AC_GRP(F, 6) = make_float4(s.npz, s.npx, __int_as_float(s.eng), __int_as_float(s.ticks));
-  store_position(D, N, n, s);
+  store_flight_role<-1>(F, D, N, n, s);
 }
 __device__ __forceinline__ void load_task(const float* F, const int* I, int N, int n, Task& t) {
   (void)I;
@@ -743,6 +751,8 @@
   float4 a4;
   ActionFetch arow;
   float shoot_raw = 0.0f;
+  LookAhead lab;
+  lab.valid = 0;
   if (SPLIT) {
     TableCopy<192> tc;
     tc.issue(P.tab);
@@ -751,7 +761,10 @@
     s = State{}; t = Task{};
     if (role == 0) { load_flight_role<0>(P.F, P.I, P.D, N, nn, s); AC_CLKW(0, 124); load_task(P.F, P.I, N, nn, t); AC_CLKW(0, 125); }
     else if (role == 1) load_flight_role<1>(P.F, P.I, P.D, N, nn, s);
-    else { load_flight_role<2>(P.F, P.I, P.D, N, nn, s); t.status = state_word(P.F, SW_status, N, nn); }
+    else {
+      load_flight_role<2>(P.F, P.I, P.D, N, nn, s); t.status = state_word(P.F, SW_status, N, nn);
+      if (P.LA) la_load(P.LA, N, nn, lab);
+    }
     __builtin_amdgcn_s_barrier();
     tc.write(lds_tab);
     a4 = make_float4(0.f, 0.f, 0.f, 0.f);
@@ -810,7 +823,8 @@
   constexpr bool OBS_BY_KIN = SPLIT && TASK == AC_TASK_SINGLECOMBAT;
   if (SPLIT) {
     const int role = __builtin_amdgcn_readfirstlane(threadIdx.x >> 6);
-    if (split_helper_wave(s, t, T, L, l, c.substeps, nullptr, nullptr, &arow)) {
+    const OwnStore own{P.F, N, n, live};
+    if (split_helper_wave<false, false, true>(s, t, T, L, l, c.substeps, nullptr, nullptr, &arow, &lab, &own)) {
       if (OBS_BY_KIN && role == 1) {
         using namespace mail;
         wg_sync();
@@ -821,6 +835,7 @@
         const Enemy Eq = exchange_1v1(q);
         L.M[T_RALT][l] = altitude_raw(q, c);
         L.M[T_RPOS][l] = posture_raw(q, Eq);
+        __builtin_amdgcn_s_waitcnt(0x0F70);
         wg_sync();
       }
       if (OBS_BY_KIN && role == 2) {
@@ -844,7 +859,12 @@
         float* row = lds_out + l * OBS;
 #pragma unroll
         for (int k = 0; k < OBS; ++k) row[k] = obq[k];
+        const bool ended = L.M[T_DONE][l] != 0.0f;
         emit_obs_rows(P, lds_out, OBS, l);
+        if (P.LA && live) {
+          if (ended) la_copy(P.LA, N, n, P.LA + (size_t)LA_GROUPS * 4 * N, 2, slot);
+          else la_store(P.LA, N, n, lab);
+        }
       }
       return;
     }
@@ -881,6 +901,7 @@
     const int other = __shfl_xor((int)mine, 1);
     env_has_missiles = mine || (bool)other;
   }
+  if (SPLIT) wg_sync();
   int quad_nrun = 0;
   const int quad_ticks0 = s.ticks;
   for (int sub = 0; sub < c.substeps; ++sub) {
@@ -894,7 +915,7 @@
       AC_CLK(4 + 8 * sub);
       if (!env_has_missiles) continue;
     } else if (SPLIT) {
-      if (dynamics_wave_tick(s, t, d, T, L, l, sub)) { have_pose = true; last_tick = sub; }
+      if (dynamics_wave_tick<false, true>(s, t, d, T, L, l, sub)) { have_pose = true; last_tick = sub; }
     } else if (t.status == AC_ALIVE) {
       if (t.bloods <= 0.0f) t.status = AC_SHOTDOWN;
       f16::tick<false>(s, d, T);
@@ -922,7 +943,8 @@
     }
     if (QUAD) wg_sync();
   }
-  const bool split_located = SPLIT && dynamics_wave_finish(s, d, L, l, last_tick, c.substeps);
+  bool sys_ok = true;
+  const bool split_located = SPLIT && dynamics_wave_finish<true>(s, d, L, l, last_tick, c.substeps, &sys_ok);
   if (PAIR) {
     if (QUAD) wg_sync();
     wg_sync();
@@ -1022,7 +1044,7 @@
   {
     float np_max = fmaxf(fabsf(s.npx), fmaxf(fabsf(s.npy), fabsf(s.npz)));
     float pqr = sqrtf(d.p * d.p + d.q * d.q + d.r * d.r);
-    nonfinite = nonfinite_probe(d.veci, pqr, d.h_sl_ft, np_max);
+    nonfinite = nonfinite_probe(d.veci, pqr, d.h_sl_ft, np_max) || !sys_ok;
     bool extreme = nonfinite || (d.veci >= 1e10f) || (pqr >= 1000.0f) || (d.h_sl_ft >= 1e10f) || (np_max > 10.0f);
     bool overload = (s.ticks >= kTickOverload) &&
                     (fabsf(s.npx) > c.acc_x || fabsf(s.npy) > c.acc_y || fabsf(s.npz + 1.0f) > c.acc_z);
@@ -1111,7 +1133,11 @@
   }
   AC_CLK(53);
   if (live) {
-    if (!PAIR) { store_flight(P.F, P.I, P.D, N, n, s); store_task_changed(P.F, P.I, N, n, t, was); }
+    if (SPLIT) {
+      if (all_done) store_flight(P.F, P.I, P.D, N, n, s);
+      else store_flight_role<0>(P.F, P.D, N, n, s);
+      store_task_changed(P.F, P.I, N, n, t, was);
+    } else if (!PAIR) { store_flight(P.F, P.I, P.D, N, n, s); store_task_changed(P.F, P.I, N, n, t, was); }
     else {
       if (all_done) store_flight(P.F, P.I, P.D, N, n, s);
       store_task_changed(P.F, P.I, N, n, t, was);
@@ -1379,7 +1405,7 @@
 }
 
 template <int TASK>
-__global__ __launch_bounds__(64) void init_kernel_1v1(InitArgs ia, DevCfg c, const float* tab, float* tF, int* tI, double* tD) {
+__global__ __launch_bounds__(64) void init_kernel_1v1(InitArgs ia, DevCfg c, const float* tab, float* tF, int* tI, double* tD, float* tLA) {
   using TT = TaskTraits<TASK>;
   constexpr int OBS = TT::OBS;
   __shared__ __attribute__((aligned(16))) float lds_tab[F16_PACK_LEN];
@@ -1403,6 +1429,12 @@
     store_state(tF, tI, tD, 2, slot, s, t);
     float* tobs = tF + (size_t)NSW * 2 + slot * OBS;
     for (int k = 0; k < OBS; ++k) tobs[k] = ob[k];
+    if (tLA) {
+      LookAhead b;
+      la_compute(s, b);
+      b.valid = 1;
+      la_store(tLA, 2, slot, b);
+    }
   }
 }
 
@@ -1449,6 +1481,7 @@
   State s; Task t;
   load_state(P.tF, P.tI, P.tD, c.A, slot, s, t);
   store_state(P.F, P.I, P.D, N, n, s, t);
+  if (P.LA) la_copy(P.LA, N, n, P.LA + (size_t)LA_GROUPS * 4 * N, c.A, slot);
   for (int k = 0; k < c.msl_slots; ++k) {
     if (P.MD) { MslD m{}; m.status = MSL_INACTIVE; store_msl(P.MD, P.MI, N, n, k, m); }
     else { Msl m{}; m.status = MSL_INACTIVE; store_msl(P.MF, P.MI, N, n, k, m); }
@@ -1504,6 +1537,7 @@
   int* count_host;
   bool timing;
   bool quad_waves;
+  bool lookahead;
   bool split_waves;
   uint64_t tmpl_hash, ctl_hash;
   int32_t* h_idx; int32_t* d_idx;
@@ -1691,7 +1725,7 @@
 extern "C" {
 
 const char* ac_last_error(void) { return g_err.c_str(); }
-const char* ac_version(void) { return "aircombat-hip 0.1 (gfx950)"; }
+const char* ac_version(void) { return "aircombat-hip 0.2 (gfx950)"; }
 const char* ac_state_field_name(int i) { return (i >= 0 && i < AC_STATE_LEN && kStateNames[i]) ? kStateNames[i] : ""; }
 
 int ac_create(const ac_config_t* cfg, int32_t n_envs, int32_t device_id, uint64_t seed, ac_env_t** out) {
@@ -1765,6 +1799,8 @@
                             cfg->task == AC_TASK_WVR || cfg->task == AC_TASK_MANEUVER;
     h->split_waves = ticks_only && (e ? (e[0] == '1') : (wgs <= 512));
     h->ctl_rows = ctl_rows_pin();
+    const char* le = getenv("AIRCOMBAT_LOOKAHEAD");
+    h->lookahead = h->split_waves && cfg->task == AC_TASK_SINGLECOMBAT && !(le && le[0] == '0');
     const char* qe = getenv("AIRCOMBAT_QUAD");
     const bool munitions_1v1 = cfg->task == AC_TASK_SHOOT_MISSILE || (cfg->task == AC_TASK_DODGE_MISSILE && !nvn_dodge) || cfg->task == AC_TASK_SCENARIO1;
     h->quad_waves = munitions_1v1 && (qe ? (qe[0] == '1') : (wgs <= 256));
@@ -1835,6 +1871,11 @@
   p.obs2 = nullptr; p.rew2 = nullptr; p.done2 = nullptr; p.info2 = nullptr;
   HIP_OK(hipMemset(p.F, 0, sizeof(float) * NSW * N));
   HIP_OK(hipMemset(p.D, 0, sizeof(double) * ND * N));
+  p.LA = nullptr;
+  if (h->lookahead) {
+    HIP_OK(hipMalloc(&p.LA, (size_t)16 * LA_GROUPS * (N + h->A)));
+    HIP_OK(hipMemset(p.LA, 0, (size_t)16 * LA_GROUPS * (N + h->A)));
+  }
   HIP_OK(hipMemset(p.MF, 0, sizeof(float) * ms * NMF * N));
   if (p.MD) HIP_OK(hipMemset(p.MD, 0, sizeof(double) * ms * NMF * N));
   HIP_OK(hipMemset(p.MI, 0, sizeof(int) * ms * NMI * N));
@@ -1903,9 +1944,10 @@
   else if (cfg->task == AC_TASK_MULTICOMBAT)
     hipLaunchKernelGGL(init_kernel_nvn<8>, dim3(1), dim3(64), 0, h->stream, ia, h->dc, h->d_tab, h->d_tF, h->d_tI, h->d_tD);
   else if (cfg->task == AC_TASK_SINGLECOMBAT)
-    hipLaunchKernelGGL(init_kernel_1v1<AC_TASK_SINGLECOMBAT>, dim3(1), dim3(64), 0, h->stream, ia, h->dc, h->d_tab, h->d_tF, h->d_tI, h->d_tD);
+    hipLaunchKernelGGL(init_kernel_1v1<AC_TASK_SINGLECOMBAT>, dim3(1), dim3(64), 0, h->stream, ia, h->dc, h->d_tab, h->d_tF, h->d_tI, h->d_tD,
+                       p.LA ? p.LA + (size_t)LA_GROUPS * 4 * N : (float*)nullptr);
   else
-    hipLaunchKernelGGL(init_kernel_1v1<AC_TASK_SHOOT_MISSILE>, dim3(1), dim3(64), 0, h->stream, ia, h->dc, h->d_tab, h->d_tF, h->d_tI, h->d_tD);
+    hipLaunchKernelGGL(init_kernel_1v1<AC_TASK_SHOOT_MISSILE>, dim3(1), dim3(64), 0, h->stream, ia, h->dc, h->d_tab, h->d_tF, h->d_tI, h->d_tD, (float*)nullptr);
   HIP_OK(hipGetLastError());
   if (launch_reset(h)) return -1;
   HIP_OK(hipStreamSynchronize(h->stream));
@@ -1919,7 +1961,7 @@
   (void)aql_settle(h);
   aql_release(&h->aql);
   (void)hipStreamSynchronize(h->stream);
-  void* bufs[] = {h->dp.F, h->dp.D, h->dp.MF, h->dp.MD, h->dp.MI, h->dp.obs, h->dp.rew, h->dp.done, h->dp.info,
+  void* bufs[] = {h->dp.F, h->dp.D, h->dp.LA, h->dp.MF, h->dp.MD, h->dp.MI, h->dp.obs, h->dp.rew, h->dp.done, h->dp.info,
                   h->d_actions, h->d_tab, h->d_tF, h->d_tD, h->d_state_io, h->d_XF, h->d_XI, h->dp.H, h->dp.man_step, h->dp.man_h0, h->d_ctlWs8, h->d_low, h->hp.HD, h->hp.HF, h->hp.HI, h->hp.HR,
                   h->d_idx, h->d_clone_tab, h->d_snap_hdr};
   for (void* b : bufs) (void)hipFree(b);
@@ -2120,8 +2162,9 @@
 struct SlotMap { int f[NF]; int i[NI]; };
 constexpr int kStateIoWords = ND + NF + NI + NXI + NXF;
 static_assert(kStateIoWords <= 256, "state_io_kernel: one thread per word of a 256-thread block");
-__global__ void state_io_kernel(float* F, double* D, const float* XF, const int* XI, size_t N, size_t n, double* io, int write, SlotMap m) {
+__global__ void state_io_kernel(float* F, double* D, float* LA, const float* XF, const int* XI, size_t N, size_t n, double* io, int write, SlotMap m) {
   const int t = threadIdx.x;
+  if (write && LA && t == 255) reinterpret_cast<int*>(LA)[((size_t)(LA_VALID_WORD >> 2) * N + n) * 4 + (LA_VALID_WORD & 3)] = 0;
   if (t < ND) {
     double* w = t < 2 ? D + 2 * n + t : D + 2 * N + n;
     if (write) *w = io[t]; else io[t] = *w;
@@ -2151,7 +2194,7 @@
   HIP_OK(hipSetDevice(h->device));
   const size_t N = h->N, n = (size_t)env * h->A + agent;
   double io[kStateIoWords];
-  hipLaunchKernelGGL(state_io_kernel, dim3(1), dim3(256), 0, h->stream, h->dp.F, h->dp.D, h->d_XF, h->d_XI, N, n, h->d_state_io, 0, slot_map());
+  hipLaunchKernelGGL(state_io_kernel, dim3(1), dim3(256), 0, h->stream, h->dp.F, h->dp.D, h->dp.LA, h->d_XF, h->d_XI, N, n, h->d_state_io, 0, slot_map());
   HIP_OK(hipGetLastError());
   HIP_OK(hipMemcpyAsync(io, h->d_state_io, sizeof io, hipMemcpyDeviceToHost, h->stream));
   HIP_OK(hipStreamSynchronize(h->stream));
@@ -2177,7 +2220,7 @@
   HIP_OK(hipSetDevice(h->device));
   const size_t N = h->N, n = (size_t)env * h->A + agent;
   HIP_OK(hipMemcpyAsync(h->d_state_io, in, sizeof(double) * (ND + NF + NI), hipMemcpyHostToDevice, h->stream));
-  hipLaunchKernelGGL(state_io_kernel, dim3(1), dim3(256), 0, h->stream, h->dp.F, h->dp.D, h->d_XF, h->d_XI, N, n, h->d_state_io, 1, slot_map());
+  hipLaunchKernelGGL(state_io_kernel, dim3(1), dim3(256), 0, h->stream, h->dp.F, h->dp.D, h->dp.LA, h->d_XF, h->d_XI, N, n, h->d_state_io, 1, slot_map());
   HIP_OK(hipGetLastError());
   HIP_OK(hipStreamSynchronize(h->stream));
   return 0;
diff --git a/aircombat-selfplay_amd/csrc/snapshot.hpp b/aircombat-selfplay_amd/csrc/snapshot.hpp
--- a/aircombat-selfplay_amd/csrc/snapshot.hpp
+++ b/aircombat-selfplay_amd/csrc/snapshot.hpp
@@ -29,6 +29,7 @@
   rows(h->dp.F, NSG, 16);
   rows(h->dp.D, 1, 16);
   rows((char*)h->dp.D + (size_t)16 * N, 1, 8);
+  rows(h->dp.LA, LA_GROUPS, 16);
   rows(h->dp.MF, ms * NMF, 4);
   rows(h->dp.MI, ms * NMI, 4);
   rows(h->dp.MD, ms * NMF, 8);
@@ -66,8 +67,8 @@
   if (!h->d_XF) c.chaff_seed = 0;
   uint64_t x = fnv1a(0xCBF29CE484222325ULL, &c, sizeof c);
   if (h->cfg.task == AC_TASK_HEADING) x = fnv1a(x, &h->hc, sizeof h->hc);
-  const int32_t form[10] = {h->cfg.hierarchical, h->cfg.use_baseline, h->cfg.controller_precision, h->act_dim, h->act_low, h->obs_dim,
-                            (int32_t)h->split_waves, (int32_t)h->quad_waves, h->ctl_rows, h->E};
+  const int32_t form[11] = {h->cfg.hierarchical, h->cfg.use_baseline, h->cfg.controller_precision, h->act_dim, h->act_low, h->obs_dim,
+                            (int32_t)h->split_waves, (int32_t)h->quad_waves, h->ctl_rows, h->E, (int32_t)h->lookahead};
   x = fnv1a(x, form, sizeof form);
   x = fnv1a(x, &h->tmpl_hash, sizeof h->tmpl_hash);
   x = fnv1a(x, &h->ctl_hash, sizeof h->ctl_hash);
diff --git a/aircombat-selfplay_amd/csrc/split_kernel.hpp b/aircombat-selfplay_amd/csrc/split_kernel.hpp
--- a/aircombat-selfplay_amd/csrc/split_kernel.hpp
+++ b/aircombat-selfplay_amd/csrc/split_kernel.hpp
@@ -11,7 +11,8 @@
        F_TEF = MASS0 + MASS_N, F_PINR, F_PINP, F_PINY, F_PIR, F_PIP, F_PIY, F_AIL, F_ELEV, F_SBDEG, F_N1, F_N2, F_N2NORM, F_FF, F_TANK0, F_TANK1,
        F_ENG, F_DA, F_DE, F_DR, F_THR,
        F_BITS,
-       K_W, K_V = K_W + 3,
+       F_OK = F_TEF,
+       K_W = F_BITS + 1, K_V = K_W + 3,
        K_OUT = K_V + 3, K_OUT_N = 27,
        G_Q = K_OUT + K_OUT_N,
        G_H = G_Q + 8, G_NED = G_H + 1,
@@ -37,6 +38,59 @@
   o.h_sl_ft = v[9]; o.n_eci[0] = v[10]; o.n_eci[1] = v[11]; o.n_eci[2] = v[12]; o.e_eci[0] = v[13]; o.e_eci[1] = v[14];
   o.d_eci[0] = v[15]; o.d_eci[1] = v[16]; o.d_eci[2] = v[17]; o.gx = v[18]; o.gy = v[19]; o.gz = v[20]; o.rxf = v[21]; o.ryf = v[22];
   o.A.T = v[23]; o.A.P = v[24]; o.A.rho = v[25]; o.A.a = v[26];
+}
+enum { LA_GROUPS = 10, LA_VALID_WORD = 27 };
+struct LookAhead {
+  f16::KinOut o;
+  double rx, ry, rz;
+  float q0, q1, q2, q3;
+  int valid;
+};
+__device__ __forceinline__ void la_load(const float* K, int N, int n, LookAhead& b) {
+  AC_LANE_INDEX(n);
+  float v[28];
+#pragma unroll
+  for (int g = 0; g < 7; ++g) { const float4 x = AC_GRP(K, g); v[4 * g] = x.x; v[4 * g + 1] = x.y; v[4 * g + 2] = x.z; v[4 * g + 3] = x.w; }
+  const double2 xy = *reinterpret_cast<const double2*>(&AC_GRP(K, 7));
+  const double2 z = *reinterpret_cast<const double2*>(&AC_GRP(K, 8));
+  const float4 q = AC_GRP(K, 9);
+  f16::KinOut& o = b.o;
+#pragma unroll
+  for (int i = 0; i < 9; ++i) o.T[i] = v[i];
+  o.h_sl_ft = v[9]; o.n_eci[0] = v[10]; o.n_eci[1] = v[11]; o.n_eci[2] = v[12]; o.e_eci[0] = v[13]; o.e_eci[1] = v[14];
+  o.d_eci[0] = v[15]; o.d_eci[1] = v[16]; o.d_eci[2] = v[17]; o.gx = v[18]; o.gy = v[19]; o.gz = v[20]; o.rxf = v[21]; o.ryf = v[22];
+  o.A.T = v[23]; o.A.P = v[24]; o.A.rho = v[25]; o.A.a = v[26];
+  b.valid = __float_as_int(v[LA_VALID_WORD]);
+  b.rx = xy.x; b.ry = xy.y; b.rz = z.x;
+  b.q0 = q.x; b.q1 = q.y; b.q2 = q.z; b.q3 = q.w;
+}
+__device__ __forceinline__ void la_store(float* K, int N, int n, const LookAhead& b) {
+  AC_LANE_INDEX(n);
+  const f16::KinOut& o = b.o;
+  AC_GRP(K, 0) = make_float4(o.T[0], o.T[1], o.T[2], o.T[3]);
+  AC_GRP(K, 1) = make_float4(o.T[4], o.T[5], o.T[6], o.T[7]);
+  AC_GRP(K, 2) = make_float4(o.T[8], o.h_sl_ft, o.n_eci[0], o.n_eci[1]);
+  AC_GRP(K, 3) = make_float4(o.n_eci[2], o.e_eci[0], o.e_eci[1], o.d_eci[0]);
+  AC_GRP(K, 4) = make_float4(o.d_eci[1], o.d_eci[2], o.gx, o.gy);
+  AC_GRP(K, 5) = make_float4(o.gz, o.rxf, o.ryf, o.A.T);
+  AC_GRP(K, 6) = make_float4(o.A.P, o.A.rho, o.A.a, __int_as_float(b.valid));
+  *reinterpret_cast<double2*>(&AC_GRP(K, 7)) = make_double2(b.rx, b.ry);
+  *reinterpret_cast<double2*>(&AC_GRP(K, 8)) = make_double2(b.rz, 0.0);
+  AC_GRP(K, 9) = make_float4(b.q0, b.q1, b.q2, b.q3);
+}
+__device__ __forceinline__ void la_copy(float* K, int N, int n, const float* from, int A, int slot) {
+  const unsigned sN = (unsigned)A * 16u, so = (unsigned)slot * 16u, dN = (unsigned)N * 16u, dn = (unsigned)n * 16u;
+#pragma unroll
+  for (unsigned g = 0; g < LA_GROUPS; ++g) {
+    const float4 v = *reinterpret_cast<const float4*>((const char*)from + (size_t)(g * sN + so));
+    *reinterpret_cast<float4*>((char*)K + (size_t)(g * dN + dn)) = v;
+  }
+}
+__device__ __forceinline__ void la_compute(f16::State& s, LookAhead& b) {
+  f16::kin_position(s, b.o);
+  f16::kin_attitude(s, b.o);
+  b.rx = s.rx; b.ry = s.ry; b.rz = s.rz;
+  b.q0 = s.q0; b.q1 = s.q1; b.q2 = s.q2; b.q3 = s.q3;
 }
 __device__ __forceinline__ void post_mass(float (*M)[64], int l, const f16::DynVars& k) {
   const float v[mail::MASS_N] = {k.mass, k.cgx, k.cgy, k.cgz, k.Jxx, k.Jyy, k.Jzz, k.Jxy, k.Jxz, k.Jyz, k.c00, k.c01, k.c02, k.c11, k.c12, k.c22, k.idet, k.im_};
@@ -83,13 +137,16 @@
     return 0.0f;
   }
 };
+struct OwnStore { float* F; int N, n; bool live; };
+template <bool OWN = false>
 __device__ __forceinline__ void systems_wave(f16::State& s, Task& t, const f16::Tab& T, float (*M)[64], int l, int substeps, const float4* raw = nullptr,
-                                             ActionFetch* row = nullptr) {
+                                             ActionFetch* row = nullptr, const OwnStore* own = nullptr) {
   using namespace mail;
   f16::DynVars km{};
   f16::sys_mass(s, km);
   post_mass(M, l, km);
   (void)t;
+  if (OWN) wg_sync();
   for (int sub = 0; sub < substeps; ++sub) {
     f16::Surf sf{};
     AC_CLKW(1, 64 + sub * 8);
@@ -136,6 +193,15 @@
     if (row) { row->take(); v = row->idx.v; } else { v.x = raw->x; v.y = raw->y; v.z = raw->z; v.w = raw->w; }
     s.da = f16::clampf(-1.0f, v.x / 20.0f - 1.0f, 1.0f); s.de = f16::clampf(-1.0f, v.y / 20.0f - 1.0f, 1.0f);
     s.dr = f16::clampf(-1.0f, v.z / 20.0f - 1.0f, 1.0f); s.thr = f16::clampf(0.0f, v.w / 58.0f + 0.4f, 0.9f);
+  }
+  if (OWN) {
+    if (own->live) store_flight_role<1>(own->F, nullptr, own->N, own->n, s);
+    M[F_ENG][l] = __int_as_float(s.eng);
+    const float sum = s.tef + s.pin_r + s.pin_p + s.pin_y + s.pi_r + s.pi_p + s.pi_y + s.ail + s.elev + s.sbdeg + s.n1 + s.n2 + s.n2norm + s.ff +
+                      s.tank0 + s.tank1 + s.da + s.de + s.dr + s.thr;
+    M[F_OK][l] = fabsf(sum) < INFINITY ? 1.0f : 0.0f;
+    wg_sync();
+    return;
   }
   M[F_TEF][l] = s.tef; M[F_PINR][l] = s.pin_r; M[F_PINP][l] = s.pin_p; M[F_PINY][l] = s.pin_y;
   M[F_PIR][l] = s.pi_r; M[F_PIP][l] = s.pi_p; M[F_PIY][l] = s.pi_y; M[F_AIL][l] = s.ail; M[F_ELEV][l] = s.elev; M[F_SBDEG][l] = s.sbdeg;
@@ -161,14 +227,27 @@
   M[r + 4][l] = dp.e_eci[0]; M[r + 5][l] = dp.e_eci[1];
   M[r + 6][l] = dp.d_eci[0]; M[r + 7][l] = dp.d_eci[1]; M[r + 8][l] = dp.d_eci[2];
 }
-template <bool QUAD = false, bool POSE = false>
+template <bool QUAD = false, bool POSE = false, bool LA = false>
 __device__ __forceinline__ void kinematics_wave(f16::State& s, Task& t, const f16::Tab& T, float (*M)[64], double (*MD)[64], int l, int substeps,
-                                                const DevCfg* cfg = nullptr) {
+                                                const DevCfg* cfg = nullptr, LookAhead* la = nullptr) {
   using namespace mail;
   f16::KinOut o;
   const int ticks0 = s.ticks;
   const bool alive0 = t.status == AC_ALIVE && substeps > 0;
-  if (alive0) { f16::kin_position(s, o); f16::kin_attitude(s, o); }
+  bool flew_last = false;
+  if (LA) {
+    if (alive0) {
+      if (la->valid) {
+        s.hv2x = s.hv1x; s.hv2y = s.hv1y; s.hv2z = s.hv1z;
+        s.hv1x = s.vx; s.hv1y = s.vy; s.hv1z = s.vz;
+        s.rx = la->rx; s.ry = la->ry; s.rz = la->rz;
+        s.q0 = la->q0; s.q1 = la->q1; s.q2 = la->q2; s.q3 = la->q3;
+      } else la_compute(s, *la);
+      post_kin(M, l, la->o);
+    }
+    *la = LookAhead{};
+    wg_sync();
+  } else if (alive0) { f16::kin_position(s, o); f16::kin_attitude(s, o); }
   if (QUAD) { MD[GD_R][l] = s.rx; MD[GD_R + 1][l] = s.ry; MD[GD_R + 2][l] = s.rz; }
   if (POSE) post_quad_pose(M, MD, l, 0, s, ticks0 + (alive0 ? 1 : 0), *cfg);
   for (int sub = 0; sub < substeps; ++sub) {
@@ -214,7 +293,14 @@
     }
     AC_CLKW(2, 70 + sub * 8);
     wg_sync();
+    if (LA && last) flew_last = run;
     if (POSE && run && !last) post_quad_pose(M, MD, l, (sub + 1) & 1, s, ticks0 + sub + 2, *cfg);
+  }
+  if (LA && flew_last) {
+    s.wp = M[K_W][l]; s.wq = M[K_W + 1][l]; s.wr = M[K_W + 2][l];
+    s.vx = M[K_V][l]; s.vy = M[K_V + 1][l]; s.vz = M[K_V + 2][l];
+    la_compute(s, *la);
+    la->valid = 1;
   }
   wg_sync();
 }
@@ -222,15 +308,16 @@
   float M[mail::ROWS][64];
   double MD[mail::DROWS][64];
 };
-template <bool QUAD = false, bool POSE = false>
+template <bool QUAD = false, bool POSE = false, bool LA = false>
 __device__ __forceinline__ bool split_helper_wave(f16::State& s, Task& t, const f16::Tab& T, SplitLds& L, int l, int substeps, const float4* raw = nullptr,
-                                                  const DevCfg* cfg = nullptr, ActionFetch* row = nullptr) {
+                                                  const DevCfg* cfg = nullptr, ActionFetch* row = nullptr, LookAhead* la = nullptr,
+                                                  const OwnStore* own = nullptr) {
   const int role = __builtin_amdgcn_readfirstlane(threadIdx.x >> 6);
-  if (role == 2) { kinematics_wave<QUAD, POSE>(s, t, T, L.M, L.MD, l, substeps, cfg); return true; }
-  if (role == 1) { systems_wave(s, t, T, L.M, l, substeps, raw, row); return true; }
+  if (role == 2) { kinematics_wave<QUAD, POSE, LA>(s, t, T, L.M, L.MD, l, substeps, cfg, la); return true; }
+  if (role == 1) { systems_wave<LA>(s, t, T, L.M, l, substeps, raw, row, own); return true; }
   return false;
 }
-template <bool QUAD = false>
+template <bool QUAD = false, bool LA = false>
 __device__ __forceinline__ bool dynamics_wave_tick(f16::State& s, Task& t, f16::Derived& d, const f16::Tab& T, SplitLds& L, int l, int sub, bool* d_stale = nullptr) {
   using namespace mail;
   float (*M)[64] = L.M;
@@ -245,7 +332,7 @@
   const int b_ticks = s.ticks;
   if (QUAD && !run) { M[K_V][l] = s.vx; M[K_V + 1][l] = s.vy; M[K_V + 2][l] = s.vz; }
   if (run) {
-    if (sub == 0) f16::dyn_p1(s, d, k);
+    if (!LA && sub == 0) f16::dyn_p1(s, d, k);
     else {
       f16::KinOut o;
       fetch_kin(M, l, o);
@@ -268,7 +355,7 @@
   }
   if (run) {
     fetch_mass(M, l, k);
-    if (sub == 0) f16::dyn_p2<false>(s, d, k);
+    if (!LA && sub == 0) f16::dyn_p2<false>(s, d, k);
     else f16::dyn_p2<true>(s, d, k);
     M[BETA][l] = k.beta;
     M[MACH][l] = k.mach; M[QBAR][l] = k.qbar; M[RHO][l] = k.A.rho; M[TEMP][l] = k.A.T; M[HSL][l] = d.h_sl_ft;
@@ -290,26 +377,32 @@
     k.clb = M[LK_CLB][l]; k.cnb = M[LK_CNB][l];
     k.g7 = make_float4(M[LK_G7][l], M[LK_G7 + 1][l], M[LK_G7 + 2][l], M[LK_G7 + 3][l]);
     f16::dyn_p4(s, d, k, sf, M[THRUST][l]);
-    if (sub > 0) {
+    if (LA || sub > 0) {
       const int pb = sub & 1;
       s.rx = MD[GD_R + 3 * pb][l]; s.ry = MD[GD_R + 3 * pb + 1][l]; s.rz = MD[GD_R + 3 * pb + 2][l];
     }
   }
   return run;
 }
-__device__ __forceinline__ bool dynamics_wave_finish(f16::State& s, f16::Derived& d, SplitLds& L, int l, int last_tick, int substeps) {
+template <bool LA = false>
+__device__ __forceinline__ bool dynamics_wave_finish(f16::State& s, f16::Derived& d, SplitLds& L, int l, int last_tick, int substeps, bool* sys_ok = nullptr) {
   using namespace mail;
   float (*M)[64] = L.M;
   double (*MD)[64] = L.MD;
   AC_CLK(50);
   wg_sync();
   AC_CLK(51);
+  if (LA) {
+    s.eng = __float_as_int(M[F_ENG][l]);
+    *sys_ok = M[F_OK][l] != 0.0f;
+  } else {
   s.tef = M[F_TEF][l]; s.pin_r = M[F_PINR][l]; s.pin_p = M[F_PINP][l]; s.pin_y = M[F_PINY][l];
   s.pi_r = M[F_PIR][l]; s.pi_p = M[F_PIP][l]; s.pi_y = M[F_PIY][l]; s.ail = M[F_AIL][l]; s.elev = M[F_ELEV][l]; s.sbdeg = M[F_SBDEG][l];
   s.n1 = M[F_N1][l]; s.n2 = M[F_N2][l]; s.n2norm = M[F_N2NORM][l]; s.ff = M[F_FF][l]; s.tank0 = M[F_TANK0][l]; s.tank1 = M[F_TANK1][l];
   s.eng = __float_as_int(M[F_ENG][l]);
   s.da = M[F_DA][l]; s.de = M[F_DE][l]; s.dr = M[F_DR][l]; s.thr = M[F_THR][l];
-  if (last_tick >= 1) {
+  }
+  if (last_tick >= (LA ? 0 : 1)) {
     const int pb = last_tick & 1;
     s.q0 = M[G_Q + 4 * pb][l]; s.q1 = M[G_Q + 4 * pb + 1][l]; s.q2 = M[G_Q + 4 * pb + 2][l]; s.q3 = M[G_Q + 4 * pb + 3][l];
   }
```

New measurement: 224.0 million. -5.3%, worse.
